# qinzheng93/GeoTransformer

Measured on NVIDIA H100. Metric: point-cloud pairs/sec (3DMatch-shape synth), higher is better.
Workload: dtype f32

## Files before the change

geotransformer_b200/_lib.py:

```python
import ctypes
import os
import threading

import torch

_HERE = os.path.dirname(os.path.abspath(__file__))
LIB_PATH = os.path.join(_HERE, 'libgeob200.so')
_lib = None

c_void_p, c_int64, c_int32, c_float, c_double, c_size_t, c_int = (
    ctypes.c_void_p, ctypes.c_int64, ctypes.c_int32, ctypes.c_float, ctypes.c_double, ctypes.c_size_t, ctypes.c_int)

SIGNATURES = {}


def _sig(name, restype, *argtypes):
    SIGNATURES[name] = (restype, list(argtypes))


P, I64, I32, F, D, SZ = c_void_p, c_int64, c_int32, c_float, c_double, c_size_t
_sig('geob200_last_error', ctypes.c_char_p)
_sig('geob200_launch_count', ctypes.c_uint64)
_sig('geob200_grid_subsample_workspace_bytes', SZ, I64, I64)
_sig('geob200_grid_subsample', c_int, P, I64, P, I64, F, P, P, P, SZ, P)
_sig('geob200_radius_search_workspace_bytes', SZ, I64, I64, I64)
_sig('geob200_radius_search', c_int, P, I64, P, I64, P, P, I64, F, I64, P, P, P, P, SZ, P)

_sig('geob200_neighbor_histogram', c_int, P, I64, I64, I64, I64, P, P)
_sig('geob200_kpconv_workspace_bytes', SZ, I64)
_sig('geob200_kpconv', c_int, P, P, P, P, I64, I64, I64, P, I64, P, P, I64, I64, F, P, P, SZ, P)
_sig('geob200_kpconv_tc_workspace_bytes', SZ, I64, I64, I64)
_sig('geob200_kpconv_tc', c_int, P, P, P, P, I64, I64, I64, P, I64, P, P, I64, I64, F, P, P, SZ, P)
_sig('geob200_set_linear_mode', None, c_int)
_sig('geob200_linear', c_int, P, I64, P, P, P, I64, I64, I64, I64, c_int, P)
_sig('geob200_split_tf32', c_int, P, I64, I64, I64, P, P)
_sig('geob200_linear_batched', c_int, P, I64, I64, P, I64, I64, P, I64, P, I64, I64, I64, I64, I64, I64, c_int, P)
_sig('geob200_group_norm_workspace_bytes', SZ, I64)
_sig('geob200_group_norm', c_int, P, I64, I64, I64, P, P, F, P, c_int, F, P, P, SZ, P)
_sig('geob200_fused_group_norm_workspace_bytes', SZ, I64, I64, I64)
_sig('geob200_linear_group_norm', c_int, P, I64, P, P, I64, I64, I64, I64, P, P, F, P, c_int, F, P, P, P, SZ, P)
_sig('geob200_kpconv_group_norm', c_int, P, P, P, P, I64, I64, I64, P, I64, P, P, I64, I64, F, I64, P, P, F, c_int, F, P, P, P, SZ,
     P, SZ, P)
_sig('geob200_group_norm_batched', c_int, P, I64, I64, I64, P, P, F, P, c_int, F, P, P, SZ, P, I64, P)
_sig('geob200_linear_group_norm_batched', c_int, P, I64, P, P, I64, I64, I64, I64, P, P, F, P, c_int, F, P, P, P, SZ, P, I64, P)
_sig('geob200_maxpool', c_int, P, P, I64, I64, I64, I64, P, P)
_sig('geob200_upsample_concat', c_int, P, P, I64, I64, P, I64, I64, I64, P, P)
_sig('geob200_kpconv_backward_workspace_bytes', SZ, I64, I64, I64, I64, I64)
_sig('geob200_kpconv_backward', c_int, P, P, P, P, I64, I64, I64, P, I64, P, I64, I64, F, P, P, P, P, P, SZ, P)
_sig('geob200_linear_backward_workspace_bytes', SZ, I64, I64, I64, c_int)
_sig('geob200_linear_backward', c_int, P, I64, P, P, I64, I64, I64, P, P, P, P, P, SZ, P)
_sig('geob200_group_norm_backward_batched_workspace_bytes', SZ, I64, I64, I64, I64)
_sig('geob200_group_norm_backward_batched', c_int, P, P, I64, I64, I64, P, F, c_int, F, P, P, P, P, P, P, SZ, P, I64, P)
_sig('geob200_maxpool_backward_batched_workspace_bytes', SZ, I64, I64, I64, I64)
_sig('geob200_maxpool_backward_batched', c_int, P, P, I64, I64, I64, I64, P, I64, P, P, P, P, SZ, P)
_sig('geob200_upsample_concat_backward_workspace_bytes', SZ, I64, I64)
_sig('geob200_upsample_concat_backward', c_int, P, I64, I64, I64, I64, I64, P, P, P, P, SZ, P)
_sig('geob200_point_to_node_partition_batched', c_int, P, P, I64, P, P, I64, P, P, P, P, P, P)
_sig('geob200_gather_rows', c_int, P, I64, I64, P, I64, P, P)
_sig('geob200_knn_partition', c_int, P, I64, P, I64, I64, P, P, P)
_sig('geob200_pairwise_distance', c_int, P, I64, P, I64, I64, c_int, P, P)
_sig('geob200_point_to_node_indices', c_int, P, I64, P, I64, P, P, P)
_sig('geob200_apply_transform', c_int, P, I64, P, P, P)
_sig('geob200_gse_indices_batched', c_int, P, I64, P, F, F, I64, P, P, P)
_sig('geob200_gse_embed_workspace_bytes', SZ, I64, I64)
_sig('geob200_gse_table_bytes', SZ, I64, I64, F, F)
_sig('geob200_gse_table_build', c_int, P, P, P, P, P, I64, I64, F, F, P, SZ, P)
_sig('geob200_gse_embed_table', c_int, P, P, I64, I64, P, SZ, I64, F, F, P, P, P, P, P, P, P)
_sig('geob200_gse_embed_pairs', c_int, P, P, I64, I64, P, P, P, P, P, P, P, P, c_int, P, SZ, P)
_sig('geob200_attention_workspace_bytes', SZ, I64, I64, I64)
_sig('geob200_attention', c_int, P, I64, P, I64, P, I64, P, P, P, I64, I64, I64, I64, P, I64, P, SZ, P)
_sig('geob200_set_attention_tma', c_int, c_int)
_sig('geob200_head_bias', c_int, P, I64, P, I64, I64, I64, P, P)
_sig('geob200_add_layernorm', c_int, P, P, P, P, I64, I64, F, P, P)
_sig('geob200_l2_normalize', c_int, P, I64, I64, P, P)
_sig('geob200_add_layernorm_backward_workspace_bytes', SZ, I64, I64)
_sig('geob200_add_layernorm_backward', c_int, P, P, P, I64, I64, F, P, P, P, P, P, SZ, P)
_sig('geob200_l2_normalize_backward', c_int, P, I64, I64, P, P, P)
_sig('geob200_head_project_backward_workspace_bytes', SZ, I64, I64, I64)
_sig('geob200_head_project_backward', c_int, P, I64, P, P, I64, I64, I64, P, P, P, I64, P, P, P, SZ, P)
_sig('geob200_attention_backward_batched_workspace_bytes', SZ, P, I64, I64)
_sig('geob200_attention_backward_batched', c_int, P, P, I64, I64, I64, I64, I64, I64, I64, I64, I64, I64, P, SZ, P)
_sig('geob200_gse_embed_backward_workspace_bytes', SZ, I64, I64)
_sig('geob200_gse_embed_backward', c_int, P, P, I64, I64, I64, P, SZ, I64, F, F, P, P, P, P, P, P, P, P, P, SZ, P)
_sig('geob200_sinkhorn', c_int, P, P, P, P, I64, I64, I64, F, P, P)
_sig('geob200_sinkhorn_backward_workspace_bytes', SZ, I64, I64, I64)
_sig('geob200_sinkhorn_backward', c_int, P, P, P, P, I64, I64, I64, F, P, P, P, P, SZ, P)
_sig('geob200_superpoint_matching_batched_workspace_bytes', SZ, I64, I64, I64)
_sig('geob200_superpoint_matching_batched', c_int, P, P, I64, P, P, I64, P, I64, c_int, P, P, P, P, SZ, P)
_sig('geob200_gather_patches_batched', c_int, P, I64, I64, P, P, P, P, I64, P, P, P, P, P)
_sig('geob200_patch_scores_batched', c_int, P, P, I64, I64, P, P, P, I64, I64, P, P)
_sig('geob200_patch_scores_backward_batched_workspace_bytes', SZ, I64, I64, I64, I64)
_sig('geob200_patch_scores_backward_batched', c_int, P, P, I64, I64, P, P, P, I64, I64, P, P, P, P, SZ, P)
_sig('geob200_lgr_batched_workspace_bytes', SZ, I64, I64, I64, I64)
_sig('geob200_local_global_registration_batched', c_int, P, P, P, P, P, I64, I64, I64, I64, I64, F, c_int, F, I64, I64, P, P, P, P,
     P, P, I64, P, P, P, P, SZ, P)
_sig('geob200_weighted_procrustes', c_int, P, P, P, I64, I64, F, F, P, P)

_sig('geob200_node_correspondences_batched_workspace_bytes', SZ, I64, I64, I64)
_sig('geob200_node_correspondences_batched', c_int, P, P, P, P, P, P, P, P, I64, P, I64, P, F, P, P, P, P, SZ, P)
_sig('geob200_evaluate_counts', c_int, P, P, I64, P, F, P, P, I64, P, P, P, I64, P, F, P, P, P, I64, c_int, F, F, F, P, P)
_sig('geob200_evaluate_batched', c_int, P, P, P, F, P, P, I64, P, P, P, I64, P, F, P, P, I64, P, I64, P, P, c_int, F, F, F, P, I64,
     P)
_sig('geob200_coarse_matching_loss_batched_workspace_bytes', SZ, I64, I64)
_sig('geob200_coarse_matching_loss_batched', c_int, P, P, I64, I64, P, P, P, P, F, F, F, F, F, F, P, I64, P, SZ, P)
_sig('geob200_fine_matching_loss_batched_workspace_bytes', SZ, I64, I64)
_sig('geob200_fine_matching_loss_batched', c_int, P, P, P, P, P, P, I64, I64, I64, P, D, P, P, I64, P, SZ, P)
_sig('geob200_coarse_matching_loss_backward_batched_workspace_bytes', SZ, I64, I64, I64)
_sig('geob200_coarse_matching_loss_backward_batched', c_int, P, P, I64, I64, P, P, P, P, F, F, F, F, F, F, P, I64, P, P, P, P, SZ, P)
_sig('geob200_fine_matching_loss_backward_batched_workspace_bytes', SZ, I64, I64)
_sig('geob200_fine_matching_loss_backward_batched', c_int, P, P, P, P, P, I64, I64, I64, P, D, P, I64, P, P, P, SZ, P)
_sig('geob200_ransac_correspondences_batched_workspace_bytes', SZ, I64, I64)
_sig('geob200_ransac_correspondences_batched', c_int, P, P, I64, I64, P, F, I64, I64, ctypes.c_uint64, I64, P, P, P, P, P, P, P, P, P, P,
     SZ, P)
_sig('geob200_feature_nn_batched_workspace_bytes', SZ, I64, I64, I64)
_sig('geob200_feature_nn_batched', c_int, P, P, I64, I64, I64, I64, P, P, P, P, P, P, P, SZ, P)
_sig('geob200_feature_corr_indices', c_int, P, P, P, P, I64, I64, I32, P, P, P, P, P)
_sig('geob200_ransac_features_batched_workspace_bytes', SZ, I64, I64, I64, I64, I64)
_sig('geob200_ransac_features_batched', c_int, P, P, P, P, I64, I64, I64, I64, P, P, F, I64, I64, I64, ctypes.c_uint64, I64, P, P, P, P, P,
     P, P, P, P, P, P, P, P, P, SZ, P)
_sig('geob200_correspondence_metrics_batched_workspace_bytes', SZ, I64, I64)
_sig('geob200_correspondence_metrics_batched', c_int, P, P, I64, I64, P, P, I64, F, P, I64, P, SZ, P)
_sig('geob200_corr_order_batched', c_int, P, I64, I64, P, I64, P, P)
_sig('geob200_corr_select_batched', c_int, P, P, P, I64, I64, P, P, I64, I64, P, P, P, P, P)
_sig('geob200_sparse_correspondence_eval_batched_workspace_bytes', SZ, I64, I64, I64)
_sig('geob200_sparse_correspondence_eval_batched', c_int, P, P, I64, P, P, I64, P, I64, I64, I64, P, P, SZ, P)
_sig('geob200_registration_error_batched', c_int, P, I64, P, I64, P, P, I64, c_int, D, D, P, P)
_sig('geob200_weighted_procrustes_counts', c_int, P, P, P, I64, I64, P, F, F, P, P)

_sig('geob200_linear_profile_enable', c_int, c_int)
_sig('geob200_set_split_k', c_int, c_int)
_sig('geob200_set_linear_persistent', c_int, c_int)
_sig('geob200_linear_profile_read', I64, I64, P, P)
_sig('geob200_backbone_workspace_bytes', SZ, P, P)
_sig('geob200_backbone_forward_batched', c_int, P, P, P, P, P, P, P, P, P, P, P, P, SZ, P, SZ, P, I64, P, P)
_sig('geob200_cloud_max_count', c_int, P, I64, I64, I64, I64, P, P, P)
_sig('geob200_transformer_batched_workspace_bytes', SZ, I64, P, I64, I64, I64)
_sig('geob200_transformer_forward_batched', c_int, P, I64, I64, I64, P, I64, P, P, P, P, SZ, P)
_sig('geob200_attention_batched_workspace_bytes', SZ, P, I64, I64)
_sig('geob200_attention_batched', c_int, P, I64, I64, I64, I64, I64, I64, I64, P, SZ, P)
_sig('geob200_attention_batched_keeps_probs', c_int, P, I64, I64, I64)
_sig('geob200_superpoint_targets_batched_workspace_bytes', SZ, I64)
_sig('geob200_superpoint_targets_batched', c_int, P, P, P, I64, P, F, I64, ctypes.c_uint64, ctypes.c_uint64, I64, P, P, P, P, SZ, P)
_sig('geob200_nonfinite_check', c_int, P, P, I64, I64, P, P)
_sig('geob200_batch_loss_weights', c_int, P, I64, I64, P, P, P, P, P)
_sig('geob200_kpconv_group_norm_batched', c_int, P, P, P, P, I64, I64, I64, P, I64, P, P, I64, I64, F, I64, P, P, F, c_int, F, P, P, P,
     SZ, P, SZ, P, I64, P)
_sig('geob200_maxpool_batched', c_int, P, P, I64, I64, I64, I64, P, I64, P, P, P)
_sig('geob200_augment_pairs_batched_workspace_bytes', SZ, I64)
_sig('geob200_augment_pairs_batched', c_int, P, P, I64, P, c_int, I64, D, D, D, D, D, ctypes.c_uint64, ctypes.c_uint64, I64, P, P, P, P, P,
     SZ, P)
_sig('geob200_modelnet_pairs_batched_workspace_bytes', SZ, I64)
_sig('geob200_modelnet_pairs_batched', c_int, P, P, I64, I64, D, D, D, D, ctypes.c_uint64, ctypes.c_uint64, I64, P, P, P, P, P, SZ, P)
_sig('geob200_modelnet_benchmark_pairs_batched_workspace_bytes', SZ, I64, I64)
_sig('geob200_modelnet_benchmark_pairs_batched', c_int, P, P, P, I64, I64, D, D, D, D, P, P, P, P, SZ, P)


def lib():
    global _lib
    if _lib is None:
        if not os.path.exists(LIB_PATH):
            raise RuntimeError(
                f'{LIB_PATH} not found: build it with `python -c "import __graft_entry__ as g; g.build()"` '
                '(there is no CPU fallback for the geotransformer_b200 ops)')
        handle = ctypes.CDLL(LIB_PATH)
        for name, (restype, argtypes) in SIGNATURES.items():
            fn = getattr(handle, name)
            fn.restype = restype
            fn.argtypes = argtypes
        _lib = handle
    return _lib


def check(rc, what):
    if rc != 0:
        msg = lib().geob200_last_error().decode(errors='replace')
        raise RuntimeError(f'{what} failed ({rc}): {msg}')


_tls = threading.local()


def stream_ptr():
    p = getattr(_tls, 'stream', None)
    if p is not None:
        return p
    return torch.cuda.current_stream().cuda_stream


class stream_scope:

    def __init__(self, ptr):
        self.ptr = ptr

    def __enter__(self):
        self.prev = getattr(_tls, 'stream', None)
        _tls.stream = self.ptr
        return self

    def __exit__(self, *a):
        _tls.stream = self.prev
        return False


def require_cuda(t, name, dtype=None):
    if not t.is_cuda:
        raise RuntimeError(f'{name} must be a CUDA tensor (geotransformer_b200 has no CPU path)')
    if dtype is not None and t.dtype != dtype:
        raise RuntimeError(f'{name} must be {dtype}, got {t.dtype}')
    if not t.is_contiguous():
        raise RuntimeError(f'{name} must be contiguous')


_WS = {}


def workspace(nbytes, device, tag='default'):
    key = (device.index if device.index is not None else torch.cuda.current_device(), stream_ptr(), tag)
    buf = _WS.get(key)
    if buf is None or buf.numel() < nbytes:
        buf = torch.empty(max(int(nbytes * 1.3), 1 << 20), dtype=torch.uint8, device=device)
        _WS[key] = buf
    return buf


def ptr(t):
    return None if t is None else t.data_ptr()
```

geotransformer_b200/csrc/common.cuh:

```cuda
#pragma once
#include <cuda_runtime.h>
#include <stdint.h>
#include <stdio.h>

namespace geob200 {

void set_error(const char* fmt, ...);
void count_launches(int n);
int ensure_max_smem(const void* kernel);

#define GEOB_CHECK_CUDA(expr)                                                                   \
    do {                                                                                        \
        cudaError_t _e = (expr);                                                                \
        if (_e != cudaSuccess) {                                                                \
            geob200::set_error("%s:%d CUDA error %s: %s", __FILE__, __LINE__, #expr,            \
                               cudaGetErrorString(_e));                                         \
            return -1;                                                                          \
        }                                                                                       \
    } while (0)

#define GEOB_CHECK_LAUNCH()                                                                     \
    do {                                                                                        \
        cudaError_t _e = cudaGetLastError();                                                    \
        if (_e != cudaSuccess) {                                                                \
            geob200::set_error("%s:%d kernel launch failed: %s", __FILE__, __LINE__,            \
                               cudaGetErrorString(_e));                                         \
            return -1;                                                                          \
        }                                                                                       \
    } while (0)

#define GEOB_REQUIRE(cond, ...)                                                                 \
    do {                                                                                        \
        if (!(cond)) {                                                                          \
            geob200::set_error(__VA_ARGS__);                                                    \
            return -2;                                                                          \
        }                                                                                       \
    } while (0)

static inline size_t align_up(size_t x, size_t a) { return (x + a - 1) / a * a; }

template <int CNT, int MASK>
struct Butterfly {
    template <int NV>
    static __device__ __forceinline__ void run(float (&v)[NV], int lane) {
        if constexpr (CNT > 1) {
            constexpr int HALF = CNT / 2;
            const bool upper = (lane & MASK) != 0;
#pragma unroll
            for (int i = 0; i < HALF; ++i) {
                const float send = upper ? v[i] : v[i + HALF];
                const float keep = upper ? v[i + HALF] : v[i];
                v[i] = keep + __shfl_xor_sync(0xffffffffu, send, MASK);
            }
            if constexpr (MASK > 1) Butterfly<HALF, MASK / 2>::run(v, lane);
        } else {
            v[0] += __shfl_xor_sync(0xffffffffu, v[0], MASK);
            if constexpr (MASK > 1) Butterfly<1, MASK / 2>::run(v, lane);
        }
    }
};
template <int NV>
__device__ __forceinline__ float warp_butterfly(float (&v)[NV], int lane) {
    Butterfly<NV, 16>::run(v, lane);
    return v[0];
}

struct GnFuse {
    int groups;
    int slot_width;
    double* partial;
};

constexpr int GEOB_MAX_CLOUDS = 64;
struct GnSeg {
    int n_clouds;
    int n_pairs;
    int start[GEOB_MAX_CLOUDS + 1];
};
size_t fused_group_norm_workspace_bytes_batched(int64_t n_rows, int64_t channels, int64_t groups, int64_t n_pairs);
int group_norm_impl(const float* x, int64_t n_rows, int64_t channels, int64_t groups, const float* gamma, const float* beta, float eps,
                    const float* residual, int leaky, float slope, float* y, void* workspace, size_t workspace_bytes, void* stream,
                    const GnSeg* seg);
int linear_group_norm_impl(const float* x, int64_t ldx, const float* weight, const float* bias, int64_t m, int64_t n, int64_t k,
                           int64_t groups, const float* gamma, const float* beta, float eps, const float* residual, int leaky,
                           float slope, float* pre_norm, float* y, void* workspace, size_t workspace_bytes, void* stream,
                           const GnSeg* seg, const float* w_img = nullptr);
int kpconv_group_norm_impl(const float* s_feats, const float* q_points, const float* s_points, const int64_t* neighbors,
                           int64_t n_query, int64_t n_support, int64_t n_neighbors, const float* kernel_points, int64_t n_kernel,
                           const float* weights_t, const float* bias, int64_t c_in, int64_t c_out, float sigma, int64_t groups,
                           const float* gamma, const float* beta, float eps, int leaky, float slope, float* pre_norm, float* y,
                           void* gn_workspace, size_t gn_workspace_bytes, void* workspace, size_t workspace_bytes, void* stream,
                           const GnSeg* seg, const float* w_img = nullptr);
int linear_img(const float* x, int64_t ldx, const float* weight, const float* w_img, const float* bias, float* y, int64_t ldy,
               int64_t m, int64_t n, int64_t k, int relu, void* stream);
int kpconv_tc_impl(const float* s_feats, const float* q_points, const float* s_points, const int64_t* neighbors, int64_t n_query,
                   int64_t n_support, int64_t n_neighbors, const float* kernel_points, int64_t n_kernel, const float* weights_t,
                   const float* w_img, const float* bias, int64_t c_in, int64_t c_out, float sigma, float* out, void* workspace,
                   size_t workspace_bytes, void* stream);

int maxpool_seg(const float* x, const int64_t* neighbors, int64_t n_query, int64_t n_support, int64_t n_neighbors, int64_t channels,
                float* y, const GnSeg* seg, const int* cloud_max, void* stream);

struct Segs {
    int n;
    int max;
    int start[GEOB_MAX_CLOUDS];
    int count[GEOB_MAX_CLOUDS];
};
int segs_from_counts(Segs* s, int64_t n, const int64_t* counts);
Segs segs_one(int64_t count);
Segs segs_range(const Segs& s, int first, int n);
int segs_products(Segs* s, const Segs& ref, const Segs& src);

struct Arena {
    char* base;
    size_t off;
    size_t cap;
    __host__ Arena(void* p, size_t bytes) : base(static_cast<char*>(p)), off(0), cap(bytes) {}
    template <typename T>
    __host__ T* take(size_t n) {
        off = align_up(off, 256);
        T* r = reinterpret_cast<T*>(base + off);
        off += n * sizeof(T);
        return r;
    }
    __host__ bool ok() const { return off <= cap; }
};

__device__ __forceinline__ float warp_sum(float v) {
#pragma unroll
    for (int o = 16; o > 0; o >>= 1) v += __shfl_xor_sync(0xffffffffu, v, o);
    return v;
}
__device__ __forceinline__ float warp_max(float v) {
#pragma unroll
    for (int o = 16; o > 0; o >>= 1) v = fmaxf(v, __shfl_xor_sync(0xffffffffu, v, o));
    return v;
}
__device__ __forceinline__ double warp_sum_d(double v) {
#pragma unroll
    for (int o = 16; o > 0; o >>= 1) v += __shfl_xor_sync(0xffffffffu, v, o);
    return v;
}

__device__ __forceinline__ float tf32_rn(float x) {
    uint32_t r;
    asm("cvt.rna.tf32.f32 %0, %1;" : "=r"(r) : "f"(x));
    return __uint_as_float(r);
}

static inline int num_sms() {
    static int n = 0;
    if (n == 0) {
        int dev = 0;
        cudaGetDevice(&dev);
        cudaDeviceGetAttribute(&n, cudaDevAttrMultiProcessorCount, dev);
        if (n <= 0) n = 132;
    }
    return n;
}

}
```

geotransformer_b200/csrc/kpconv.cu:

```cuda
#include "common.cuh"
#include "geob200.h"
#include "kpconv.cuh"

namespace geob200 {

constexpr int TQ = 32;
constexpr int CC = 32;

__global__ void __launch_bounds__(256) kpconv_c1_kernel(const float* __restrict__ feats, const float* __restrict__ q_pts,
                                                        const float* __restrict__ s_pts, const long long* __restrict__ nbr,
                                                        int H, const float* __restrict__ kp, const float* __restrict__ W,
                                                        const float* __restrict__ bias, float sigma, int Ns, int M, int Cout,
                                                        float* __restrict__ out) {
    __shared__ float kp_s[KP * 3];
    __shared__ float wk_s[16][KP_PAD];
    __shared__ float np_s[16];
    if (threadIdx.x < KP * 3) kp_s[threadIdx.x] = kp[threadIdx.x];
    __syncthreads();
    const int lane = threadIdx.x & 31, warp = threadIdx.x >> 5;
    const int sub = lane >> 4, sl = lane & 15;
    const int slot = warp * 2 + sub;
    const int m = blockIdx.x * 16 + slot;
    const bool live = m < M;
    float acc[KP];
// ... 495 lines not shown
            mean_rstd[2 * g + 1] = (float)(1.0 / sqrt(var + eps));
        }
    }
}

__global__ void __launch_bounds__(256) gn_tile_stats_kernel(const float* __restrict__ x, int N, int C, int slot_width,
                                                            double* __restrict__ partial) {
    extern __shared__ double sh[];
    const int slots = C / slot_width;
    for (int i = threadIdx.x; i < 2 * slots; i += blockDim.x) sh[i] = 0.0;
    __syncthreads();
    const int r0 = blockIdx.x * 128, r1 = min(N, r0 + 128);
    const int cw = C < 256 ? C : 256;
    const int rpb = 256 / cw;
    const int rr = threadIdx.x / cw;
    if (rr < rpb)
        for (int c = threadIdx.x % cw; c < C; c += cw) {
            double s = 0.0, s2 = 0.0;
            for (int r = r0 + rr; r < r1; r += rpb) {
                const double v = (double)x[(long long)r * C + c];
                s += v;
                s2 += v * v;
            }
            atomicAdd(&sh[2 * (c / slot_width)], s);
            atomicAdd(&sh[2 * (c / slot_width) + 1], s2);
        }
    __syncthreads();
    for (int i = threadIdx.x; i < 2 * slots; i += blockDim.x) partial[(long long)blockIdx.x * 2 * slots + i] = sh[i];
}

__global__ void __launch_bounds__(128) gn_seg_finalize_kernel(const double* __restrict__ partial, const float* __restrict__ x, int C,
                                                              int slots_total, int spg, int G, double eps, GnSeg seg,
                                                              float* __restrict__ mean_rstd) {
    __shared__ double red[8];
    const int lane = threadIdx.x & 31, warp = threadIdx.x >> 5;
    const int g = blockIdx.x, p = blockIdx.y;
    const int cpg = C / G;
    const double2* part = reinterpret_cast<const double2*>(partial);
    double sa = 0.0, sb = 0.0;
    long long rows = 0;
    for (int c = p; c < seg.n_clouds; c += seg.n_pairs) {
        const int r0 = seg.start[c], r1 = seg.start[c + 1];
        rows += r1 - r0;
        int t0 = (r0 + 127) / 128, t1 = r1 / 128;
        if (t1 < t0) t1 = t0;
        const int n_full = (t1 - t0) * spg;
        for (int i = threadIdx.x; i < n_full; i += 128) {
            const int t = t0 + i / spg, sl = i % spg;
            const double2 v = part[(long long)t * slots_total + (long long)g * spg + sl];
            sa += v.x;
            sb += v.y;
        }
        const int e0 = min(r1, t0 * 128);
        const int b1 = min(r1, max(e0, t1 * 128));
        const int n_edge = (e0 - r0) + (r1 - b1);
        for (int i = threadIdx.x; i < n_edge * cpg; i += 128) {
            const int ri = i / cpg, j = i % cpg;
            const int r = ri < e0 - r0 ? r0 + ri : b1 + (ri - (e0 - r0));
            const double v = (double)x[(long long)r * C + g * cpg + j];
            sa += v;
            sb += v * v;
        }
    }
#pragma unroll
    for (int o = 16; o > 0; o >>= 1) {
        sa += __shfl_xor_sync(0xffffffffu, sa, o);
        sb += __shfl_xor_sync(0xffffffffu, sb, o);
    }
    if (lane == 0) { red[2 * warp] = sa; red[2 * warp + 1] = sb; }
    __syncthreads();
    if (threadIdx.x == 0) {
        sa = (red[0] + red[2]) + (red[4] + red[6]);
        sb = (red[1] + red[3]) + (red[5] + red[7]);
        const double count = (double)cpg * (double)rows;
        const double mean = sa / count;
        double var = sb / count - mean * mean;
        if (var < 0.0) var = 0.0;
        mean_rstd[((long long)p * G + g) * 2] = (float)mean;
        mean_rstd[((long long)p * G + g) * 2 + 1] = (float)(1.0 / sqrt(var + eps));
    }
}

constexpr int GN_RPB = 32;
__global__ void __launch_bounds__(256) gn_seg_apply_kernel(const float* __restrict__ x, const float* __restrict__ mean_rstd,
                                                           const float* __restrict__ gamma, const float* __restrict__ beta,
                                                           const float* __restrict__ residual, float* __restrict__ y, int n_rows,
                                                           int C, int cpg, int G, int leaky, float slope, GnSeg seg) {
    extern __shared__ float gn_tab[];
    __shared__ int starts[GEOB_MAX_CLOUDS + 1];
    for (int i = threadIdx.x; i <= seg.n_clouds; i += blockDim.x) starts[i] = seg.start[i];
    __syncthreads();
    const int r0 = blockIdx.x * GN_RPB, r1 = min(n_rows, r0 + GN_RPB);
    int c0 = 0, hi = seg.n_clouds;
    while (hi - c0 > 1) {
        const int mid = (c0 + hi) >> 1;
        if (starts[mid] <= r0) c0 = mid; else hi = mid;
    }
    for (int i = threadIdx.x; i < 2 * C; i += blockDim.x) {
        const int t = i / C, c = i % C;
        const int cl = min(c0 + t, seg.n_clouds - 1);
        const float* mr = mean_rstd + (long long)(cl % seg.n_pairs) * 2 * G + 2 * (c / cpg);
        gn_tab[(2 * t) * C + c] = mr[0];
        gn_tab[(2 * t + 1) * C + c] = mr[1];
    }
    __syncthreads();
    const int b0 = starts[c0 + 1];
    const int b1 = (c0 + 2 <= seg.n_clouds) ? starts[c0 + 2] : n_rows;
    const int C4 = C >> 2;
    const long long base4 = (long long)r0 * C4;
    const int total4 = (r1 - r0) * C4;
    for (int i = threadIdx.x; i < total4; i += blockDim.x) {
        const int row = r0 + i / C4, c = (i % C4) * 4;
        const float4 v = reinterpret_cast<const float4*>(x)[base4 + i];
        float4 rv = make_float4(0.f, 0.f, 0.f, 0.f);
        if (residual != nullptr) rv = reinterpret_cast<const float4*>(residual)[base4 + i];
        float in[4] = {v.x, v.y, v.z, v.w}, o[4];
        const float rs[4] = {rv.x, rv.y, rv.z, rv.w};
        if (row < b1) {
            const float* ta = gn_tab + (row < b0 ? 0 : 2 * C) + c;
            const float4 gm = __ldg(reinterpret_cast<const float4*>(gamma + c)), bt = __ldg(reinterpret_cast<const float4*>(beta + c));
            const float ga[4] = {gm.x, gm.y, gm.z, gm.w}, ba[4] = {bt.x, bt.y, bt.z, bt.w};
#pragma unroll
            for (int u = 0; u < 4; ++u) o[u] = (in[u] - ta[u]) * ta[C + u] * ga[u] + ba[u] + rs[u];
        } else {
            int lo = c0, hh = seg.n_clouds;
            while (hh - lo > 1) {
                const int mid = (lo + hh) >> 1;
                if (starts[mid] <= row) lo = mid; else hh = mid;
            }
            const float* mr = mean_rstd + (long long)(lo % seg.n_pairs) * 2 * G;
#pragma unroll
            for (int u = 0; u < 4; ++u) {
                const int g = (c + u) / cpg;
                o[u] = (in[u] - mr[2 * g]) * mr[2 * g + 1] * gamma[c + u] + beta[c + u] + rs[u];
            }
        }
        if (leaky) {
#pragma unroll
            for (int u = 0; u < 4; ++u) o[u] = o[u] > 0.f ? o[u] : o[u] * slope;
        }
        reinterpret_cast<float4*>(y)[base4 + i] = make_float4(o[0], o[1], o[2], o[3]);
    }
}

__global__ void __launch_bounds__(256) gn_apply_kernel(const float* __restrict__ x, const float* __restrict__ mean_rstd,
                                                       const float* __restrict__ gamma, const float* __restrict__ beta,
                                                       const float* __restrict__ residual, float* __restrict__ y,
                                                       long long total4, int C, int cpg, int leaky, float slope) {
    const long long i = (long long)blockIdx.x * blockDim.x + threadIdx.x;
    if (i >= total4) return;
    const float4 v = reinterpret_cast<const float4*>(x)[i];
    const int c = (int)((i * 4) % C);
    float in[4] = {v.x, v.y, v.z, v.w}, o[4];
    float4 rv = make_float4(0.f, 0.f, 0.f, 0.f);
    if (residual != nullptr) rv = reinterpret_cast<const float4*>(residual)[i];
    const float rs[4] = {rv.x, rv.y, rv.z, rv.w};
#pragma unroll
    for (int u = 0; u < 4; ++u) {
        const int g = (c + u) / cpg;
        float t = (in[u] - mean_rstd[2 * g]) * mean_rstd[2 * g + 1] * gamma[c + u] + beta[c + u];
        t += rs[u];
        if (leaky) t = t > 0.f ? t : t * slope;
        o[u] = t;
    }
    reinterpret_cast<float4*>(y)[i] = make_float4(o[0], o[1], o[2], o[3]);
}

__device__ __forceinline__ void maxpool_row(const float* __restrict__ x, const long long* __restrict__ nb, int W, int Ns, int C,
                                            float* __restrict__ yrow, int lane) {
    constexpr int NI = 5;
    if ((C & 3) == 0 && W <= 32 * NI) {
        int idx_l[NI];
#pragma unroll
        for (int i = 0; i < NI; ++i) idx_l[i] = (lane + 32 * i < W) ? (int)min(nb[lane + 32 * i], (long long)Ns) : Ns;
        const int C4 = C >> 2;
        for (int c0 = 0; c0 < C4; c0 += 32) {
            const int c4 = c0 + lane;
            const bool active = c4 < C4;
            float4 best = make_float4(-INFINITY, -INFINITY, -INFINITY, -INFINITY);
            for (int h0 = 0; h0 < W; h0 += 4) {
                float4 v[4];
#pragma unroll
                for (int u = 0; u < 4; ++u) {
                    const int h = h0 + u;
                    int id = Ns;
#pragma unroll
                    for (int i = 0; i < NI; ++i) {
                        const int t = __shfl_sync(0xffffffffu, idx_l[i], h & 31);
                        if ((h >> 5) == i) id = t;
                    }
                    v[u] = (active && h < W && id < Ns) ? __ldg(reinterpret_cast<const float4*>(x + (long long)id * C) + c4)
                                                        : make_float4(0.f, 0.f, 0.f, 0.f);
                    if (h >= W) v[u] = best;
                }
#pragma unroll
                for (int u = 0; u < 4; ++u) {
                    best.x = fmaxf(best.x, v[u].x); best.y = fmaxf(best.y, v[u].y);
                    best.z = fmaxf(best.z, v[u].z); best.w = fmaxf(best.w, v[u].w);
                }
            }
            if (active) reinterpret_cast<float4*>(yrow)[c4] = best;
        }
        return;
    }
    for (int c = lane; c < C; c += 32) {
        float best = -INFINITY;
        for (int h = 0; h < W; ++h) {
            const long long idx = nb[h];
            const float v = (idx < Ns) ? x[idx * C + c] : 0.f;
            best = fmaxf(best, v);
        }
        yrow[c] = best;
    }
}

__global__ void __launch_bounds__(256) maxpool_seg_kernel(const float* __restrict__ x, const long long* __restrict__ nbr, int H,
                                                          int Ns, int M, int C, float* __restrict__ y, GnSeg seg,
                                                          const int* __restrict__ cloud_max) {
    __shared__ int starts[GEOB_MAX_CLOUDS + 1];
    __shared__ int width[GEOB_MAX_CLOUDS];
    for (int i = threadIdx.x; i <= seg.n_clouds; i += blockDim.x) starts[i] = seg.start[i];
    for (int i = threadIdx.x; i < seg.n_clouds; i += blockDim.x) {
        const int p = i % seg.n_pairs;
        int w = 0;
        for (int c = p; c < seg.n_clouds; c += seg.n_pairs) w = max(w, cloud_max[c]);
        width[i] = min(H, w);
    }
    __syncthreads();
    const int lane = threadIdx.x & 31;
    const int m = blockIdx.x * 8 + (threadIdx.x >> 5);
    if (m >= M) return;
    int lo = 0, hi = seg.n_clouds;
    while (hi - lo > 1) {
        const int mid = (lo + hi) >> 1;
        if (starts[mid] <= m) lo = mid; else hi = mid;
    }
    const int W = width[lo];
    maxpool_row(x, nbr + (long long)m * H, W, Ns, C, y + (long long)m * C, lane);
}

__global__ void __launch_bounds__(256) cloud_max_count_kernel(const long long* __restrict__ nbr, int H, int Ns, GnSeg seg,
                                                              int* __restrict__ cloud_max) {
    __shared__ int red[8];
    const int c = blockIdx.x;
    const int r0 = seg.start[c], r1 = seg.start[c + 1];
    int best = 0;
    for (int m = r0 + (int)threadIdx.x; m < r1; m += blockDim.x) {
        int lo = 0, hi = H;
        while (lo < hi) {
            const int mid = (lo + hi) >> 1;
            if (nbr[(long long)m * H + mid] < Ns) lo = mid + 1; else hi = mid;
        }
        best = max(best, lo);
    }
    for (int o = 16; o > 0; o >>= 1) best = max(best, __shfl_xor_sync(0xffffffffu, best, o));
    if ((threadIdx.x & 31) == 0) red[threadIdx.x >> 5] = best;
    __syncthreads();
    if (threadIdx.x == 0) {
        for (int w = 1; w < 8; ++w) best = max(best, red[w]);
        cloud_max[c] = best;
    }
}

__global__ void __launch_bounds__(256) maxpool_kernel(const float* __restrict__ x, const long long* __restrict__ nbr, int H,
                                                      int Ns, int M, int C, float* __restrict__ y) {
    const int lane = threadIdx.x & 31;
    const int m = blockIdx.x * 8 + (threadIdx.x >> 5);
    if (m >= M) return;
    if ((C & 3) == 0 && H <= 160) {
        maxpool_row(x, nbr + (long long)m * H, H, Ns, C, y + (long long)m * C, lane);
        return;
    }
    for (int c = lane; c < C; c += 32) {
        float best = -INFINITY;
        for (int h = 0; h < H; ++h) {
            const long long idx = nbr[(long long)m * H + h];
            const float v = (idx < Ns) ? x[idx * C + c] : 0.f;
            best = fmaxf(best, v);
        }
        y[(long long)m * C + c] = best;
    }
}

__global__ void __launch_bounds__(256) upsample_concat_kernel(const float* __restrict__ x, const long long* __restrict__ up,
                                                              int up_stride, int Ns, const float* __restrict__ skip, int M,
                                                              int C1, int C2, float* __restrict__ y) {
    const int lane = threadIdx.x & 31;
    const int m = blockIdx.x * 8 + (threadIdx.x >> 5);
    if (m >= M) return;
    const long long idx = up[(long long)m * up_stride];
    float* yr = y + (long long)m * (C1 + C2);
    for (int c = lane; c < C1; c += 32) yr[c] = (idx < Ns) ? x[idx * C1 + c] : 0.f;
    if (skip != nullptr)
        for (int c = lane; c < C2; c += 32) yr[C1 + c] = skip[(long long)m * C2 + c];
}

}

using namespace geob200;

namespace geob200 {
int linear_tc(const float* x, int64_t ldx, const float* w, int64_t ldw, const float* w_img, const float* bias, const float* row_scale, float* y, int64_t ldy,
              int64_t m, int64_t n, int64_t k, int relu, cudaStream_t st, const GnFuse* gn = nullptr);
static int g_linear_mode = 1;
}

extern "C" {

void geob200_set_linear_mode(int mode) { g_linear_mode = mode; }

size_t geob200_kpconv_workspace_bytes(int64_t n_support) { return (size_t)n_support + 256; }

size_t geob200_kpconv_tc_workspace_bytes(int64_t n_query, int64_t n_support, int64_t c_in) {
    return align_up((size_t)n_support, 256) + align_up((size_t)n_query * 4, 256) + (size_t)n_query * KP * (size_t)c_in * 4 + 1024;
}

int geob200_kpconv_tc(const float* s_feats, const float* q_points, const float* s_points, const int64_t* neighbors, int64_t n_query,
                      int64_t n_support, int64_t n_neighbors, const float* kernel_points, int64_t n_kernel, const float* weights_t,
                      const float* bias, int64_t c_in, int64_t c_out, float sigma, float* out, void* workspace, size_t workspace_bytes,
                      void* stream) {
    return geob200::kpconv_tc_impl(s_feats, q_points, s_points, neighbors, n_query, n_support, n_neighbors, kernel_points, n_kernel,
                                   weights_t, nullptr, bias, c_in, c_out, sigma, out, workspace, workspace_bytes, stream);
}
}

namespace geob200 {
int kpconv_tc_impl(const float* s_feats, const float* q_points, const float* s_points, const int64_t* neighbors, int64_t n_query,
                   int64_t n_support, int64_t n_neighbors, const float* kernel_points, int64_t n_kernel, const float* weights_t,
                   const float* w_img, const float* bias, int64_t c_in, int64_t c_out, float sigma, float* out, void* workspace,
                   size_t workspace_bytes, void* stream) {
    cudaStream_t st = (cudaStream_t)stream;
    GEOB_REQUIRE(n_kernel == KP, "kpconv_tc: kernel_size %lld unsupported", (long long)n_kernel);
    GEOB_REQUIRE(n_query > 0 && n_support > 0 && n_neighbors > 0, "kpconv_tc: empty input");
    GEOB_REQUIRE(c_in % 32 == 0 && c_out % 16 == 0 && c_out >= 32 && (c_out <= 128 || c_out % 128 == 0) && n_query >= 64,
                 "kpconv_tc: unsupported shape (%lld -> %lld, %lld queries)", (long long)c_in, (long long)c_out, (long long)n_query);
    GEOB_REQUIRE(workspace_bytes >= geob200_kpconv_tc_workspace_bytes(n_query, n_support, c_in), "kpconv_tc: workspace too small");
    Arena ar(workspace, workspace_bytes);
    unsigned char* pos = ar.take<unsigned char>(n_support);
    float* inv_count = ar.take<float>(n_query);
    float* wf = ar.take<float>((size_t)n_query * KP * c_in);
    row_positive_kernel<<<(unsigned)((n_support + 7) / 8), 256, 0, st>>>(s_feats, (int)n_support, (int)c_in, pos);
    launch_kpconv_gather(s_feats, pos, q_points, s_points, (const long long*)neighbors, (int)n_neighbors, kernel_points, sigma,
                         (int)n_support, (int)n_query, (int)c_in, wf, inv_count, st);
    GEOB_CHECK_LAUNCH();
    count_launches(2);
    const int rc = linear_tc(wf, KP * c_in, weights_t, KP * c_in, w_img, bias, inv_count, out, c_out, n_query, c_out, KP * c_in, 0, st);
    GEOB_REQUIRE(rc == 0, "kpconv_tc: tensor-core GEMM rejected the shape");
    return 0;
}

int linear_img(const float* x, int64_t ldx, const float* weight, const float* w_img, const float* bias, float* y, int64_t ldy,
               int64_t m, int64_t n, int64_t k, int relu, void* stream) {
    if (g_linear_mode == 1 && m > 0 && n > 0 && k > 0) {
        const int rc = linear_tc(x, ldx, weight, k, w_img, bias, nullptr, y, ldy, m, n, k, relu, (cudaStream_t)stream);
        if (rc <= 0) return rc;
    }
    return geob200_linear(x, ldx, weight, bias, y, ldy, m, n, k, relu, stream);
}
}

extern "C" {

int geob200_kpconv(const float* s_feats, const float* q_points, const float* s_points, const int64_t* neighbors,
                   int64_t n_query, int64_t n_support, int64_t n_neighbors, const float* kernel_points, int64_t n_kernel,
                   const float* weights, const float* bias, int64_t c_in, int64_t c_out, float sigma, float* out,
                   void* workspace, size_t workspace_bytes, void* stream) {
    cudaStream_t st = (cudaStream_t)stream;
    GEOB_REQUIRE(n_kernel == KP, "kpconv: kernel_size %lld unsupported (all shipped models use 15)", (long long)n_kernel);
    GEOB_REQUIRE(n_query > 0 && n_support > 0 && n_neighbors > 0, "kpconv: empty input");
    if (c_in == 1) {
        kpconv_c1_kernel<<<(unsigned)((n_query + 15) / 16), 256, 0, st>>>(s_feats, q_points, s_points, (const long long*)neighbors,
                                                                       (int)n_neighbors, kernel_points, weights, bias, sigma,
                                                                       (int)n_support, (int)n_query, (int)c_out, out);
        GEOB_CHECK_LAUNCH();
        count_launches(1);
        return 0;
    }
    GEOB_REQUIRE(c_in % 32 == 0 && c_out % 32 == 0 && c_out <= 512,
                 "kpconv: channel counts (%lld -> %lld) must be multiples of 32, c_out <= 512", (long long)c_in, (long long)c_out);
    GEOB_REQUIRE(workspace != nullptr && workspace_bytes >= geob200_kpconv_workspace_bytes(n_support), "kpconv: workspace too small");
    unsigned char* pos = (unsigned char*)workspace;
    row_positive_kernel<<<(unsigned)((n_support + 7) / 8), 256, 0, st>>>(s_feats, (int)n_support, (int)c_in, pos);
    const size_t smem = sizeof(float) * (TQ * KP * CC + 8 * 32 * KP_PAD + TQ + KP * 3 + 3) + sizeof(int) * 8 * 32;
    const unsigned qtiles = (unsigned)((n_query + TQ - 1) / TQ);
    int rc = (int)(c_out / 32);
    int split = 1;
    while (rc > 1 && split < 4 && (long long)qtiles * split < 2ll * num_sms()) { rc >>= 1; split <<= 1; }
    const dim3 grid(qtiles, (unsigned)split);
#define LAUNCH_KP(RCV)                                                                                              \
    {                                                                                                               \
        if (ensure_max_smem((const void*)kpconv_kernel<RCV>)) return -1;                                            \
        kpconv_kernel<RCV><<<grid, 256, smem, st>>>(s_feats, pos, q_points, s_points, (const long long*)neighbors,  \
                                                    (int)n_neighbors, kernel_points, weights, bias, sigma,         \
                                                    (int)n_support, (int)n_query, (int)c_in, (int)c_out, out);     \
    }
    switch (rc) {
        case 1: LAUNCH_KP(1) break;
        case 2: LAUNCH_KP(2) break;
        case 4: LAUNCH_KP(4) break;
        case 8: LAUNCH_KP(8) break;
        case 16: LAUNCH_KP(16) break;
        default: GEOB_REQUIRE(false, "kpconv: c_out %lld unsupported (32,64,128,256,512)", (long long)c_out);
    }
#undef LAUNCH_KP
    GEOB_CHECK_LAUNCH();
    count_launches(2);
    return 0;
}

int geob200_linear_batched(const float* x, int64_t ldx, int64_t stride_x, const float* weight, int64_t ldw, int64_t stride_w,
                           const float* bias, int64_t stride_b, float* y, int64_t ldy, int64_t stride_y, int64_t m, int64_t n,
                           int64_t k, int64_t batch, int relu, void* stream) {
    cudaStream_t st = (cudaStream_t)stream;
    GEOB_REQUIRE(m > 0 && n > 0 && k > 0 && batch > 0, "linear: empty problem");
    if (batch == 1 && g_linear_mode == 1) {
        const int rc = linear_tc(x, ldx, weight, ldw, nullptr, bias, nullptr, y, ldy, m, n, k, relu, st);
        if (rc <= 0) return rc;
    }
    const unsigned z = (unsigned)batch;
    const long long c64 = ((n + 63) / 64) * ((m + 63) / 64) * batch, c6432 = ((n + 31) / 32) * ((m + 63) / 64) * batch;
    if (c64 >= num_sms()) {
        dim3 grid((unsigned)((n + 63) / 64), (unsigned)((m + 63) / 64), z);
        linear_kernel<64, 64><<<grid, 256, 0, st>>>(x, (int)ldx, weight, (int)ldw, bias, y, (int)ldy, (int)m, (int)n, (int)k, relu,
                                                    stride_x, stride_w, stride_b, stride_y);
    } else if (c6432 >= num_sms()) {
        dim3 grid((unsigned)((n + 31) / 32), (unsigned)((m + 63) / 64), z);
        linear_kernel<64, 32><<<grid, 256, 0, st>>>(x, (int)ldx, weight, (int)ldw, bias, y, (int)ldy, (int)m, (int)n, (int)k, relu,
                                                    stride_x, stride_w, stride_b, stride_y);
    } else {
        dim3 grid((unsigned)((n + 31) / 32), (unsigned)((m + 31) / 32), z);
        linear_kernel<32, 32><<<grid, 256, 0, st>>>(x, (int)ldx, weight, (int)ldw, bias, y, (int)ldy, (int)m, (int)n, (int)k, relu,
                                                    stride_x, stride_w, stride_b, stride_y);
    }
    GEOB_CHECK_LAUNCH();
    count_launches(1);
    return 0;
}

int geob200_linear(const float* x, int64_t ldx, const float* weight, const float* bias, float* y, int64_t ldy, int64_t m,
                   int64_t n, int64_t k, int relu, void* stream) {
    return geob200_linear_batched(x, ldx, 0, weight, k, 0, bias, 0, y, ldy, 0, m, n, k, 1, relu, stream);
}

size_t geob200_group_norm_workspace_bytes(int64_t groups) { return (size_t)(592 * 2 * groups * 8 + 2 * groups * 4 + 256 + 1024); }

size_t geob200_fused_group_norm_workspace_bytes(int64_t n_rows, int64_t channels, int64_t groups) {
    const size_t tiles = (size_t)((n_rows + 127) / 128);
    const size_t slots = (size_t)(channels / groups >= 32 ? channels / 32 : groups);
    const size_t fused = tiles * slots * 2 * 8;
    const size_t plain = (size_t)(592 * 2 * groups * 8);
    return (fused > plain ? fused : plain) + (size_t)(2 * groups * 4) + 256 + 1024;
}

}

namespace geob200 {
size_t fused_group_norm_workspace_bytes_batched(int64_t n_rows, int64_t channels, int64_t groups, int64_t n_pairs) {
    return geob200_fused_group_norm_workspace_bytes(n_rows, channels, groups) + (size_t)(2 * groups * 4) * (size_t)(n_pairs > 1 ? n_pairs : 1) + 512;
}
struct GnWs { unsigned* ticket; float* mean_rstd; double* partial; };
static GnWs gn_carve(void* workspace, size_t bytes, int64_t groups, int64_t n_pairs = 1) {
    Arena ar(workspace, bytes);
    GnWs w;
    w.ticket = ar.take<unsigned>(64);
    w.mean_rstd = ar.take<float>(2 * groups * n_pairs);
    w.partial = ar.take<double>(1);
    return w;
}
static void launch_gn_seg_apply(const float* x, const GnWs& w, const float* gamma, const float* beta, const float* residual, float* y,
                                int64_t n_rows, int64_t channels, int64_t groups, float eps, int leaky, float slope, const GnSeg& seg,
                                cudaStream_t st) {
    const int cpg = (int)(channels / groups);
    const int slot_width = cpg < 32 ? cpg : 32;
    gn_seg_finalize_kernel<<<dim3((unsigned)groups, (unsigned)seg.n_pairs), 128, 0, st>>>(
        w.partial, x, (int)channels, (int)(channels / slot_width), cpg / slot_width, (int)groups, (double)eps, seg, w.mean_rstd);
    gn_seg_apply_kernel<<<(unsigned)((n_rows + GN_RPB - 1) / GN_RPB), 256, sizeof(float) * 4 * channels, st>>>(
        x, w.mean_rstd, gamma, beta, residual, y, (int)n_rows, (int)channels, cpg, (int)groups, leaky, slope, seg);
    count_launches(2);
}
static void launch_gn_tile_stats(const float* x, const GnWs& w, int64_t n_rows, int64_t channels, int64_t groups, cudaStream_t st) {
    const int cpg = (int)(channels / groups);
    const int slot_width = cpg < 32 ? cpg : 32;
    gn_tile_stats_kernel<<<(unsigned)((n_rows + 127) / 128), 256, sizeof(double) * 2 * (channels / slot_width), st>>>(
        x, (int)n_rows, (int)channels, slot_width, w.partial);
    count_launches(1);
}
static void launch_gn_apply(const float* x, const GnWs& w, const float* gamma, const float* beta, const float* residual, float* y,
                            int64_t n_rows, int64_t channels, int64_t groups, float eps, int leaky, float slope, cudaStream_t st) {
    const int cpg = (int)(channels / groups);
    const int slot_width = cpg < 32 ? cpg : 32;
    gn_finalize_kernel<<<1, 1024, 0, st>>>(w.partial, (int)((n_rows + 127) / 128), (int)(channels / slot_width), cpg / slot_width,
                                           (int)groups, (double)cpg * (double)n_rows, (double)eps, w.mean_rstd);
    const long long total4 = n_rows * channels / 4;
    gn_apply_kernel<<<(unsigned)((total4 + 255) / 256), 256, 0, st>>>(x, w.mean_rstd, gamma, beta, residual, y, total4, (int)channels,
                                                                     (int)(channels / groups), leaky, slope);
}
}

extern "C" {

int geob200_group_norm(const float* x, int64_t n_rows, int64_t channels, int64_t groups, const float* gamma,
                       const float* beta, float eps, const float* residual, int leaky, float slope, float* y,
                       void* workspace, size_t workspace_bytes, void* stream) {
    return geob200::group_norm_impl(x, n_rows, channels, groups, gamma, beta, eps, residual, leaky, slope, y, workspace, workspace_bytes,
                                    stream, nullptr);
}
}

namespace geob200 {
int group_norm_impl(const float* x, int64_t n_rows, int64_t channels, int64_t groups, const float* gamma, const float* beta, float eps,
                    const float* residual, int leaky, float slope, float* y, void* workspace, size_t workspace_bytes, void* stream,
                    const GnSeg* seg) {
    cudaStream_t st = (cudaStream_t)stream;
    GEOB_REQUIRE(n_rows > 0 && channels > 0 && groups > 0 && channels % groups == 0, "group_norm: bad shape");
    GEOB_REQUIRE(channels % 4 == 0, "group_norm: channels must be a multiple of 4");
    if (seg != nullptr && seg->n_pairs > 1) {
        GEOB_REQUIRE(workspace_bytes >= fused_group_norm_workspace_bytes_batched(n_rows, channels, groups, seg->n_pairs),
                     "group_norm: workspace too small (batched)");
        const GnWs w = gn_carve(workspace, workspace_bytes, groups, seg->n_pairs);
        launch_gn_tile_stats(x, w, n_rows, channels, groups, st);
        launch_gn_seg_apply(x, w, gamma, beta, residual, y, n_rows, channels, groups, eps, leaky, slope, *seg, st);
        GEOB_CHECK_LAUNCH();
        return 0;
    }
    GEOB_REQUIRE(workspace_bytes >= geob200_group_norm_workspace_bytes(groups), "group_norm: workspace too small");
    Arena ar(workspace, workspace_bytes);
    unsigned* ticket = ar.take<unsigned>(64);
    float* mean_rstd = ar.take<float>(2 * groups);
    double* partial = ar.take<double>(592 * 2 * groups);
    int nblk = (int)((n_rows + 127) / 128);
    if (nblk > 296) nblk = 296;
    if (nblk < 1) nblk = 1;
    gn_stats_kernel<<<nblk, 256, sizeof(double) * 2 * groups, st>>>(x, (int)n_rows, (int)channels, (int)groups, (double)eps,
                                                                    partial, ticket, mean_rstd);
    const long long total4 = n_rows * channels / 4;
    gn_apply_kernel<<<(unsigned)((total4 + 255) / 256), 256, 0, st>>>(x, mean_rstd, gamma, beta, residual, y, total4,
                                                                     (int)channels, (int)(channels / groups), leaky, slope);
    GEOB_CHECK_LAUNCH();
    count_launches(2);
    return 0;
}
}

extern "C" {

int geob200_maxpool(const float* x, const int64_t* neighbors, int64_t n_query, int64_t n_support, int64_t n_neighbors,
                    int64_t channels, float* y, void* stream) {
    maxpool_kernel<<<(unsigned)((n_query + 7) / 8), 256, 0, (cudaStream_t)stream>>>(x, (const long long*)neighbors, (int)n_neighbors,
                                                                                  (int)n_support, (int)n_query, (int)channels, y);
    GEOB_CHECK_LAUNCH();
    count_launches(1);
    return 0;
}

int geob200_upsample_concat(const float* x, const int64_t* up_indices, int64_t up_stride, int64_t n_support,
                            const float* skip, int64_t n_query, int64_t c1, int64_t c2, float* y, void* stream) {
    upsample_concat_kernel<<<(unsigned)((n_query + 7) / 8), 256, 0, (cudaStream_t)stream>>>(
        x, (const long long*)up_indices, (int)up_stride, (int)n_support, skip, (int)n_query, (int)c1, (int)c2, y);
    GEOB_CHECK_LAUNCH();
    count_launches(1);
    return 0;
}

int geob200_linear_group_norm(const float* x, int64_t ldx, const float* weight, const float* bias, int64_t m, int64_t n, int64_t k,
                              int64_t groups, const float* gamma, const float* beta, float eps, const float* residual, int leaky,
                              float slope, float* pre_norm, float* y, void* workspace, size_t workspace_bytes, void* stream) {
    return geob200::linear_group_norm_impl(x, ldx, weight, bias, m, n, k, groups, gamma, beta, eps, residual, leaky, slope, pre_norm, y,
                                           workspace, workspace_bytes, stream, nullptr);
}
}

namespace geob200 {
int linear_group_norm_impl(const float* x, int64_t ldx, const float* weight, const float* bias, int64_t m, int64_t n, int64_t k,
                           int64_t groups, const float* gamma, const float* beta, float eps, const float* residual, int leaky,
                           float slope, float* pre_norm, float* y, void* workspace, size_t workspace_bytes, void* stream,
                           const GnSeg* seg, const float* w_img) {
    cudaStream_t st = (cudaStream_t)stream;
    const int64_t np = (seg != nullptr && seg->n_pairs > 1) ? seg->n_pairs : 1;
    GEOB_REQUIRE(m > 0 && n > 0 && k > 0 && groups > 0 && n % groups == 0 && n % 4 == 0, "linear_group_norm: bad shape");
    GEOB_REQUIRE(workspace_bytes >= (np > 1 ? fused_group_norm_workspace_bytes_batched(m, n, groups, np)
                                            : geob200_fused_group_norm_workspace_bytes(m, n, groups)), "linear_group_norm: workspace too small");
    if (g_linear_mode == 1) {
        const GnWs w = gn_carve(workspace, workspace_bytes, groups, np);
        GnFuse gn{(int)groups, 0, w.partial};
        const int rc = linear_tc(x, ldx, weight, k, w_img, bias, nullptr, pre_norm, n, m, n, k, 0, st, &gn);
        if (rc < 0) return rc;
        if (rc == 0) {
            if (np > 1) {
                launch_gn_seg_apply(pre_norm, w, gamma, beta, residual, y, m, n, groups, eps, leaky, slope, *seg, st);
            } else {
                launch_gn_apply(pre_norm, w, gamma, beta, residual, y, m, n, groups, eps, leaky, slope, st);
                count_launches(2);
            }
            GEOB_CHECK_LAUNCH();
            return 0;
        }
    }
    int rc = linear_img(x, ldx, weight, w_img, bias, pre_norm, n, m, n, k, 0, stream);
    if (rc != 0) return rc;
    return group_norm_impl(pre_norm, m, n, groups, gamma, beta, eps, residual, leaky, slope, y, workspace, workspace_bytes, stream, seg);
}
}

extern "C" {

int geob200_kpconv_group_norm(const float* s_feats, const float* q_points, const float* s_points, const int64_t* neighbors,
                              int64_t n_query, int64_t n_support, int64_t n_neighbors, const float* kernel_points, int64_t n_kernel,
                              const float* weights_t, const float* bias, int64_t c_in, int64_t c_out, float sigma, int64_t groups,
                              const float* gamma, const float* beta, float eps, int leaky, float slope, float* pre_norm, float* y,
                              void* gn_workspace, size_t gn_workspace_bytes, void* workspace, size_t workspace_bytes, void* stream) {
    return geob200::kpconv_group_norm_impl(s_feats, q_points, s_points, neighbors, n_query, n_support, n_neighbors, kernel_points, n_kernel,
                                           weights_t, bias, c_in, c_out, sigma, groups, gamma, beta, eps, leaky, slope, pre_norm, y,
                                           gn_workspace, gn_workspace_bytes, workspace, workspace_bytes, stream, nullptr);
}
}

namespace geob200 {
int kpconv_group_norm_impl(const float* s_feats, const float* q_points, const float* s_points, const int64_t* neighbors,
                           int64_t n_query, int64_t n_support, int64_t n_neighbors, const float* kernel_points, int64_t n_kernel,
                           const float* weights_t, const float* bias, int64_t c_in, int64_t c_out, float sigma, int64_t groups,
                           const float* gamma, const float* beta, float eps, int leaky, float slope, float* pre_norm, float* y,
                           void* gn_workspace, size_t gn_workspace_bytes, void* workspace, size_t workspace_bytes, void* stream,
                           const GnSeg* seg, const float* w_img) {
    cudaStream_t st = (cudaStream_t)stream;
    const int64_t np = (seg != nullptr && seg->n_pairs > 1) ? seg->n_pairs : 1;
    GEOB_REQUIRE(n_kernel == KP, "kpconv_group_norm: kernel_size %lld unsupported", (long long)n_kernel);
    GEOB_REQUIRE(n_query > 0 && n_support > 0 && n_neighbors > 0, "kpconv_group_norm: empty input");
    GEOB_REQUIRE(c_in % 32 == 0 && c_out % 16 == 0 && c_out >= 32 && (c_out <= 128 || c_out % 128 == 0) && n_query >= 64,
                 "kpconv_group_norm: unsupported shape (%lld -> %lld, %lld queries)", (long long)c_in, (long long)c_out,
                 (long long)n_query);
    GEOB_REQUIRE(groups > 0 && c_out % groups == 0, "kpconv_group_norm: bad group count");
    GEOB_REQUIRE(gn_workspace_bytes >= (np > 1 ? fused_group_norm_workspace_bytes_batched(n_query, c_out, groups, np)
                                               : geob200_fused_group_norm_workspace_bytes(n_query, c_out, groups)),
                 "kpconv_group_norm: GroupNorm workspace too small");
    GEOB_REQUIRE(workspace_bytes >= geob200_kpconv_tc_workspace_bytes(n_query, n_support, c_in), "kpconv_group_norm: workspace too small");
    Arena ar(workspace, workspace_bytes);
    unsigned char* pos = ar.take<unsigned char>(n_support);
    float* inv_count = ar.take<float>(n_query);
    float* wf = ar.take<float>((size_t)n_query * KP * c_in);
    row_positive_kernel<<<(unsigned)((n_support + 7) / 8), 256, 0, st>>>(s_feats, (int)n_support, (int)c_in, pos);
    launch_kpconv_gather(s_feats, pos, q_points, s_points, (const long long*)neighbors, (int)n_neighbors, kernel_points, sigma,
                         (int)n_support, (int)n_query, (int)c_in, wf, inv_count, st);
    GEOB_CHECK_LAUNCH();
    count_launches(2);
    const GnWs w = gn_carve(gn_workspace, gn_workspace_bytes, groups, np);
    GnFuse gn{(int)groups, 0, w.partial};
    int rc = linear_tc(wf, KP * c_in, weights_t, KP * c_in, w_img, bias, inv_count, pre_norm, c_out, n_query, c_out, KP * c_in, 0, st, &gn);
    if (rc < 0) return rc;
    if (rc == 0) {
        if (np > 1) {
            launch_gn_seg_apply(pre_norm, w, gamma, beta, nullptr, y, n_query, c_out, groups, eps, leaky, slope, *seg, st);
        } else {
            launch_gn_apply(pre_norm, w, gamma, beta, nullptr, y, n_query, c_out, groups, eps, leaky, slope, st);
            count_launches(2);
        }
        GEOB_CHECK_LAUNCH();
        return 0;
    }
    rc = linear_tc(wf, KP * c_in, weights_t, KP * c_in, w_img, bias, inv_count, pre_norm, c_out, n_query, c_out, KP * c_in, 0, st);
    GEOB_REQUIRE(rc == 0, "kpconv_group_norm: tensor-core GEMM rejected the shape");
    return group_norm_impl(pre_norm, n_query, c_out, groups, gamma, beta, eps, nullptr, leaky, slope, y, gn_workspace, gn_workspace_bytes,
                           stream, seg);
}
}

namespace geob200 {
int make_seg(GnSeg* g, int64_t n_pairs, const int64_t* cloud_rows_h, int64_t n_rows, const char* what) {
    GEOB_REQUIRE(n_pairs >= 1 && 2 * n_pairs <= GEOB_MAX_CLOUDS && cloud_rows_h != nullptr, "%s: 1 <= pairs per batch <= %d", what,
                 GEOB_MAX_CLOUDS / 2);
    g->n_pairs = (int)n_pairs; g->n_clouds = (int)(2 * n_pairs); g->start[0] = 0;
    for (int c = 0; c < g->n_clouds; ++c) {
        GEOB_REQUIRE(cloud_rows_h[c] >= 0, "%s: negative cloud row count", what);
        g->start[c + 1] = g->start[c] + (int)cloud_rows_h[c];
    }
    GEOB_REQUIRE(g->start[g->n_clouds] == n_rows, "%s: cloud rows do not add up to n_rows", what);
    return 0;
}
}

extern "C" {

int geob200_group_norm_batched(const float* x, int64_t n_rows, int64_t channels, int64_t groups, const float* gamma, const float* beta,
                               float eps, const float* residual, int leaky, float slope, float* y, void* workspace, size_t workspace_bytes,
                               void* stream, int64_t n_pairs, const int64_t* cloud_rows_h) {
    geob200::GnSeg seg;
    if (geob200::make_seg(&seg, n_pairs, cloud_rows_h, n_rows, "group_norm")) return -2;
    return geob200::group_norm_impl(x, n_rows, channels, groups, gamma, beta, eps, residual, leaky, slope, y, workspace, workspace_bytes,
                                    stream, &seg);
}

int geob200_linear_group_norm_batched(const float* x, int64_t ldx, const float* weight, const float* bias, int64_t m, int64_t n, int64_t k,
                                      int64_t groups, const float* gamma, const float* beta, float eps, const float* residual, int leaky,
                                      float slope, float* pre_norm, float* y, void* workspace, size_t workspace_bytes, void* stream,
                                      int64_t n_pairs, const int64_t* cloud_rows_h) {
    geob200::GnSeg seg;
    if (geob200::make_seg(&seg, n_pairs, cloud_rows_h, m, "group_norm")) return -2;
    return geob200::linear_group_norm_impl(x, ldx, weight, bias, m, n, k, groups, gamma, beta, eps, residual, leaky, slope, pre_norm, y,
                                           workspace, workspace_bytes, stream, &seg);
}

int geob200_cloud_max_count(const int64_t* neighbors, int64_t n_query, int64_t n_support, int64_t n_neighbors, int64_t n_pairs,
                            const int64_t* cloud_rows_h, int32_t* cloud_max, void* stream) {
    geob200::GnSeg seg;
    if (geob200::make_seg(&seg, n_pairs, cloud_rows_h, n_query, "group_norm")) return -2;
    geob200::cloud_max_count_kernel<<<seg.n_clouds, 256, 0, (cudaStream_t)stream>>>((const long long*)neighbors, (int)n_neighbors,
                                                                                   (int)n_support, seg, cloud_max);
    GEOB_CHECK_LAUNCH();
    geob200::count_launches(1);
    return 0;
}

}

namespace geob200 {
int maxpool_seg(const float* x, const int64_t* neighbors, int64_t n_query, int64_t n_support, int64_t n_neighbors, int64_t channels,
                float* y, const GnSeg* seg, const int* cloud_max, void* stream) {
    maxpool_seg_kernel<<<(unsigned)((n_query + 7) / 8), 256, 0, (cudaStream_t)stream>>>(x, (const long long*)neighbors, (int)n_neighbors,
                                                                                      (int)n_support, (int)n_query, (int)channels, y, *seg,
                                                                                      cloud_max);
    GEOB_CHECK_LAUNCH();
    count_launches(1);
    return 0;
}
}

extern "C" {

int geob200_kpconv_group_norm_batched(const float* s_feats, const float* q_points, const float* s_points, const int64_t* neighbors,
                                      int64_t n_query, int64_t n_support, int64_t n_neighbors, const float* kernel_points, int64_t n_kernel,
                                      const float* weights_t, const float* bias, int64_t c_in, int64_t c_out, float sigma, int64_t groups,
                                      const float* gamma, const float* beta, float eps, int leaky, float slope, float* pre_norm, float* y,
                                      void* gn_workspace, size_t gn_workspace_bytes, void* workspace, size_t workspace_bytes, void* stream,
                                      int64_t n_pairs, const int64_t* cloud_rows_h) {
    geob200::GnSeg seg;
    if (geob200::make_seg(&seg, n_pairs, cloud_rows_h, n_query, "kpconv_group_norm")) return -2;
    GEOB_REQUIRE(pre_norm != nullptr && y != nullptr, "kpconv_group_norm: null output");
    return geob200::kpconv_group_norm_impl(s_feats, q_points, s_points, neighbors, n_query, n_support, n_neighbors, kernel_points, n_kernel,
                                           weights_t, bias, c_in, c_out, sigma, groups, gamma, beta, eps, leaky, slope, pre_norm, y,
                                           gn_workspace, gn_workspace_bytes, workspace, workspace_bytes, stream, &seg);
}

int geob200_maxpool_batched(const float* x, const int64_t* neighbors, int64_t n_query, int64_t n_support, int64_t n_neighbors,
                            int64_t channels, const int32_t* cloud_max, int64_t n_pairs, const int64_t* cloud_rows_h, float* y,
                            void* stream) {
    geob200::GnSeg seg;
    if (geob200::make_seg(&seg, n_pairs, cloud_rows_h, n_query, "maxpool")) return -2;
    GEOB_REQUIRE(n_query > 0 && n_support > 0 && n_neighbors > 0 && channels > 0, "maxpool: empty input");
    GEOB_REQUIRE(x != nullptr && neighbors != nullptr && cloud_max != nullptr && y != nullptr, "maxpool: null pointer");
    return geob200::maxpool_seg(x, neighbors, n_query, n_support, n_neighbors, channels, y, &seg, cloud_max, stream);
}

}
```

geotransformer_b200/csrc/linear_tc.cu:

```cuda
#include <cuda.h>

#include <cstdlib>
#include <mutex>
#include <vector>

#include "common.cuh"
#include "geob200.h"
#include "hopper.cuh"

namespace geob200 {
namespace ltc {

using namespace hop;

constexpr int BM = 128;
constexpr int KC = 32;
constexpr int TILE_A = BM * 128;
constexpr int TILE_B = 128 * 128;
constexpr int STAGE = TILE_A + 2 * TILE_B;
constexpr int NSTAGE = 4;
constexpr int PRODUCER_WARP = 8;
constexpr int NTHREADS = (PRODUCER_WARP + 4) * 32;
constexpr int SMEM = NSTAGE * STAGE + 1024 + 256 + 8 * 128 * 8 + 512;

__global__ void __launch_bounds__(256) split_tf32_kernel(const float* __restrict__ w, long long ld, long long n, long long k,
                                                         float* __restrict__ out) {
    const long long nk = n * k;
    for (long long i = (long long)blockIdx.x * blockDim.x + threadIdx.x; i < nk; i += (long long)gridDim.x * blockDim.x) {
        const long long r = i / k, c = i % k;
        const float x = w[r * ld + c];
        const float hi = tf32_rn(x);
        out[i] = hi;
        out[nk + i] = x - hi;
    }
}

template <int BNI>
__global__ void __launch_bounds__(NTHREADS, 1) linear_tc_kernel(const __grid_constant__ CUtensorMap map_x,
                                                                const __grid_constant__ CUtensorMap map_w,
                                                                const float* __restrict__ bias, const float* __restrict__ row_scale,
                                                                float* __restrict__ Y, int ldy, int M, int N, int K, int BN, int relu,
                                                                GnFuse gn, float* __restrict__ splitk_out, int chunks_per_split,
                                                                int col_tiles, int row_tiles, int num_tiles) {
    constexpr int R = BNI / 2;
    extern __shared__ unsigned char smem_raw[];
    unsigned char* smem = (unsigned char*)(((uintptr_t)smem_raw + 1023) & ~(uintptr_t)1023);
    uint64_t* bars = (uint64_t*)(smem + NSTAGE * STAGE);
    uint64_t* full = bars;
    uint64_t* empty = bars + NSTAGE;
    float2* gn_sm = (float2*)(smem + NSTAGE * STAGE + 256);
    float* bias_s = (float*)(gn_sm + 8 * 128);
    const int warp = threadIdx.x >> 5, lane = threadIdx.x & 31;
    const int nk = (K + KC - 1) / KC;
    const int tiles_per_split = col_tiles * row_tiles;

    if (threadIdx.x == 0) {
        for (int s = 0; s < NSTAGE; ++s) { mbar_init(&full[s], 1); mbar_init(&empty[s], 8); }
        asm volatile("fence.mbarrier_init.release.cluster;" ::: "memory");
        asm volatile("prefetch.tensormap [%0];" ::"l"(&map_x) : "memory");
        asm volatile("prefetch.tensormap [%0];" ::"l"(&map_w) : "memory");
    }
    __syncthreads();

    if (warp >= PRODUCER_WARP) {
        asm volatile("setmaxnreg.dec.sync.aligned.u32 40;" ::: "memory");
        if (warp == PRODUCER_WARP && lane == 0) {
            int s = 0;
            uint32_t ph = 0;
            for (int t = blockIdx.x; t < num_tiles; t += gridDim.x) {
                const int z = t / tiles_per_split, rem = t % tiles_per_split;
                const int m0 = (rem / col_tiles) * BM, n0 = (rem % col_tiles) * BN;
                const int kc0 = z * chunks_per_split, kc1 = min(nk, kc0 + chunks_per_split);
                for (int kc = kc0; kc < kc1; ++kc) {
                    mbar_wait(&empty[s], ph ^ 1u);
                    unsigned char* st = smem + s * STAGE;
                    mbar_arrive_expect_tx(&full[s], (uint32_t)(TILE_A + 2 * BN * 128));
                    tma_load_2d(st, &map_x, kc * KC, m0, &full[s]);
                    tma_load_2d(st + TILE_A, &map_w, kc * KC, n0, &full[s]);
                    tma_load_2d(st + TILE_A + TILE_B, &map_w, kc * KC, N + n0, &full[s]);
                    if (++s == NSTAGE) { s = 0; ph ^= 1u; }
                }
            }
        }
        return;
    }

    asm volatile("setmaxnreg.inc.sync.aligned.u32 232;" ::: "memory");
    const int wg = warp >> 2, wq = warp & 3;
    int s = 0;
    uint32_t ph = 0;
    for (int t = blockIdx.x; t < num_tiles; t += gridDim.x) {
        const int z = t / tiles_per_split, rem = t % tiles_per_split;
        const int ty = rem / col_tiles;
        const int m0 = ty * BM, n0 = (rem % col_tiles) * BN;
        const int kc0 = z * chunks_per_split, kc1 = min(nk, kc0 + chunks_per_split);
        asm volatile("bar.sync 1, 256;" ::: "memory");
        if (threadIdx.x < 128) bias_s[threadIdx.x] = (bias != nullptr && (int)threadIdx.x < BN) ? __ldg(bias + n0 + threadIdx.x) : 0.f;
        asm volatile("bar.sync 1, 256;" ::: "memory");

        float acc[R], cor[R];
#pragma unroll
        for (int i = 0; i < R; ++i) { acc[i] = 0.f; cor[i] = 0.f; }
        const int g = lane >> 2, tq = lane & 3;
        const int a_off = (wg * 64 + wq * 16 + g) * 128 + tq * 4;
        for (int kc = kc0; kc < kc1; ++kc) {
            mbar_wait(&full[s], ph);
            unsigned char* st = smem + s * STAGE;
            uint32_t f[2][KC / 8][4];
#pragma unroll
            for (int kk = 0; kk < KC / 8; ++kk)
#pragma unroll
                for (int e = 0; e < 4; ++e) {
                    const int j = 2 * kk + (e >> 1);
                    const float x = *reinterpret_cast<const float*>(st + a_off + (e & 1) * 8 * 128 + ((j ^ g) << 4));
                    const float hi = tf32_rn(x);
                    f[0][kk][e] = __float_as_uint(hi);
                    f[1][kk][e] = __float_as_uint(x - hi);
                }
            const uint32_t sb = smem_u32(st + TILE_A);
            const uint64_t b_hi = make_desc(sb), b_lo = make_desc(sb + TILE_B);
            wgmma_fence();
#pragma unroll
            for (int kk = 0; kk < KC / 8; ++kk) {
                const uint64_t adv = (uint64_t)(kk * 2);
                const uint32_t accum = (kc == kc0 && kk == 0) ? 0u : 1u;
                wgmma_tf32_rs<BNI>(acc, f[0][kk], b_hi + adv, accum);
                wgmma_tf32_rs<BNI>(cor, f[0][kk], b_lo + adv, accum);
                wgmma_tf32_rs<BNI>(cor, f[1][kk], b_hi + adv, 1u);
            }
            wgmma_commit();
            wgmma_wait<0>();
            __syncwarp();
            if (lane == 0) mbar_arrive(&empty[s]);
            if (++s == NSTAGE) { s = 0; ph ^= 1u; }
        }
        reg_fence(acc);
        reg_fence(cor);

        const int r0 = m0 + wg * 64 + wq * 16 + (lane >> 2);
        const int c0 = 2 * (lane & 3);
        float rs[2];
#pragma unroll
        for (int h = 0; h < 2; ++h) rs[h] = (row_scale != nullptr && r0 + 8 * h < M) ? row_scale[r0 + 8 * h] : 1.0f;
        if (splitk_out != nullptr) {
#pragma unroll
            for (int j = 0; j < BNI / 8; ++j)
#pragma unroll
                for (int h = 0; h < 2; ++h) {
                    const int m = r0 + 8 * h, col = 8 * j + c0;
                    if (m < M && col < BN)
                        *reinterpret_cast<float2*>(splitk_out + ((long long)z * M + m) * N + n0 + col) =
                            make_float2(acc[4 * j + 2 * h] + cor[4 * j + 2 * h], acc[4 * j + 2 * h + 1] + cor[4 * j + 2 * h + 1]);
                }
            continue;
        }
        const bool vec2 = ((ldy & 1) == 0) && ((reinterpret_cast<uintptr_t>(Y) & 7) == 0);
#pragma unroll
        for (int j = 0; j < BNI / 8; ++j) {
            const int col = 8 * j + c0;
            float o[4];
#pragma unroll
            for (int e = 0; e < 4; ++e) {
                float v = (acc[4 * j + e] + cor[4 * j + e]) * rs[e >> 1] + bias_s[col + (e & 1)];
                if (relu) v = fmaxf(v, 0.f);
                o[e] = v;
            }
#pragma unroll
            for (int h = 0; h < 2; ++h) {
                const int m = r0 + 8 * h;
                if (m < M && col < BN) {
                    float* yp = Y + (long long)m * ldy + n0 + col;
                    if (vec2) *reinterpret_cast<float2*>(yp) = make_float2(o[2 * h], o[2 * h + 1]);
                    else { yp[0] = o[2 * h]; yp[1] = o[2 * h + 1]; }
                }
            }
            if (gn.groups > 0) {
                const bool ok0 = r0 < M && col < BN, ok1 = r0 + 8 < M && col < BN;
                float a0 = (ok0 ? o[0] : 0.f) + (ok1 ? o[2] : 0.f), a1 = (ok0 ? o[1] : 0.f) + (ok1 ? o[3] : 0.f);
                float q0 = (ok0 ? o[0] * o[0] : 0.f) + (ok1 ? o[2] * o[2] : 0.f);
                float q1 = (ok0 ? o[1] * o[1] : 0.f) + (ok1 ? o[3] * o[3] : 0.f);
#pragma unroll
                for (int off = 4; off < 32; off <<= 1) {
                    a0 += __shfl_xor_sync(0xffffffffu, a0, off);
                    a1 += __shfl_xor_sync(0xffffffffu, a1, off);
                    q0 += __shfl_xor_sync(0xffffffffu, q0, off);
                    q1 += __shfl_xor_sync(0xffffffffu, q1, off);
                }
                if (lane < 4) {
                    gn_sm[warp * 128 + col] = make_float2(a0, q0);
                    gn_sm[warp * 128 + col + 1] = make_float2(a1, q1);
                }
            }
        }
        if (gn.groups > 0) {
            asm volatile("bar.sync 1, 256;" ::: "memory");
            const int sw = gn.slot_width, slots_tile = BN / sw, slots_total = N / sw;
            const int et = threadIdx.x;
            if (et < slots_tile) {
                double s1 = 0.0, s2 = 0.0;
                for (int w = 0; w < 8; ++w) {
                    float f1 = 0.f, f2 = 0.f;
                    for (int c = 0; c < sw; ++c) {
                        const float2 p = gn_sm[w * 128 + et * sw + c];
                        f1 += p.x;
                        f2 += p.y;
                    }
                    s1 += (double)f1;
                    s2 += (double)f2;
                }
                double* dst = gn.partial + ((long long)ty * slots_total + n0 / sw + et) * 2;
                dst[0] = s1;
                dst[1] = s2;
            }
        }
    }
}

__global__ void __launch_bounds__(256) splitk_reduce_kernel(const float* __restrict__ P, int splits, long long MN, int N,
                                                            const float* __restrict__ bias, const float* __restrict__ row_scale,
                                                            float* __restrict__ Y, int ldy, int relu) {
    const long long i4 = ((long long)blockIdx.x * blockDim.x + threadIdx.x) * 4;
    if (i4 >= MN) return;
    float4 a = *reinterpret_cast<const float4*>(P + i4);
    for (int z = 1; z < splits; ++z) {
        const float4 b = *reinterpret_cast<const float4*>(P + (long long)z * MN + i4);
        a.x += b.x; a.y += b.y; a.z += b.z; a.w += b.w;
    }
    const long long m = i4 / N;
    const int n = (int)(i4 % N);
    const float rs = row_scale != nullptr ? row_scale[m] : 1.0f;
    float o[4] = {a.x * rs, a.y * rs, a.z * rs, a.w * rs};
#pragma unroll
    for (int u = 0; u < 4; ++u) {
        if (bias != nullptr) o[u] += bias[n + u];
        if (relu) o[u] = fmaxf(o[u], 0.f);
    }
    float* y = Y + m * ldy + n;
    if ((reinterpret_cast<uintptr_t>(y) & 15) == 0) *reinterpret_cast<float4*>(y) = make_float4(o[0], o[1], o[2], o[3]);
    else { y[0] = o[0]; y[1] = o[1]; y[2] = o[2]; y[3] = o[3]; }
}

typedef CUresult (*EncodeTiledFn)(CUtensorMap*, CUtensorMapDataType, cuuint32_t, void*, const cuuint64_t*, const cuuint64_t*,
                                  const cuuint32_t*, const cuuint32_t*, CUtensorMapInterleave, CUtensorMapSwizzle,
                                  CUtensorMapL2promotion, CUtensorMapFloatOOBfill);
static EncodeTiledFn encode_fn() {
    static EncodeTiledFn fn = nullptr;
    if (fn == nullptr) {
        void* p = nullptr;
        cudaDriverEntryPointQueryResult q;
        if (cudaGetDriverEntryPoint("cuTensorMapEncodeTiled", &p, cudaEnableDefault, &q) == cudaSuccess && q == cudaDriverEntryPointSuccess)
            fn = (EncodeTiledFn)p;
    }
    return fn;
}

static int encode_map(CUtensorMap* map, const float* base, int64_t rows, int64_t cols, int64_t ld, int box_rows) {
    EncodeTiledFn fn = encode_fn();
    if (fn == nullptr) { set_error("cuTensorMapEncodeTiled entry point not available"); return -1; }
    cuuint64_t gdim[2] = {(cuuint64_t)cols, (cuuint64_t)rows};
    cuuint64_t gstride[1] = {(cuuint64_t)ld * sizeof(float)};
    cuuint32_t box[2] = {(cuuint32_t)KC, (cuuint32_t)box_rows};
    cuuint32_t estr[2] = {1, 1};
    CUresult r = fn(map, CU_TENSOR_MAP_DATA_TYPE_FLOAT32, 2, (void*)base, gdim, gstride, box, estr, CU_TENSOR_MAP_INTERLEAVE_NONE,
                    CU_TENSOR_MAP_SWIZZLE_128B, CU_TENSOR_MAP_L2_PROMOTION_L2_128B, CU_TENSOR_MAP_FLOAT_OOB_FILL_NONE);
    if (r != CUDA_SUCCESS) { set_error("cuTensorMapEncodeTiled failed with CUresult %d", (int)r); return -1; }
    return 0;
}

}

struct ProfRec { cudaEvent_t a, b; long long m, n, k; };
static std::vector<ProfRec> g_prof;
static std::mutex g_prof_mu;
static bool g_prof_on = false;
static bool g_splitk_on = true;
static bool g_persistent_on = true;

struct StreamWs { void* ptr; size_t bytes; };
static std::vector<std::pair<cudaStream_t, StreamWs>> g_split_ws, g_wimg_ws;
static std::mutex g_split_mu;
static float* stream_scratch(std::vector<std::pair<cudaStream_t, StreamWs>>& pool, cudaStream_t st, size_t bytes) {
    std::lock_guard<std::mutex> lk(g_split_mu);
    for (auto& e : pool)
        if (e.first == st) {
            if (e.second.bytes >= bytes) return (float*)e.second.ptr;
            cudaFreeAsync(e.second.ptr, st);
            e.second = {nullptr, 0};
            if (cudaMallocAsync(&e.second.ptr, bytes * 2, st) != cudaSuccess) return nullptr;
            e.second.bytes = bytes * 2;
            return (float*)e.second.ptr;
        }
    StreamWs w{nullptr, 0};
    const size_t cap = bytes * 2 > (16u << 20) ? bytes * 2 : (16u << 20);
    if (cudaMallocAsync(&w.ptr, cap, st) != cudaSuccess) return nullptr;
    w.bytes = cap;
    pool.push_back({st, w});
    return (float*)w.ptr;
}

static void launch_split_tf32(const float* w, int64_t ld, int64_t n, int64_t k, float* out, cudaStream_t st) {
    const long long nk = (long long)n * k;
    long long blocks = (nk + 255) / 256;
    if (blocks > 4LL * num_sms()) blocks = 4LL * num_sms();
    ltc::split_tf32_kernel<<<(unsigned)(blocks > 0 ? blocks : 1), 256, 0, st>>>(w, ld, n, k, out);
    count_launches(1);
}

int linear_tc(const float* x, int64_t ldx, const float* w, int64_t ldw, const float* w_img, const float* bias, const float* row_scale,
              float* y, int64_t ldy, int64_t m, int64_t n, int64_t k, int relu, cudaStream_t st, const GnFuse* gn) {
    if (m < 64 || n < 32 || (n % 16) != 0 || (k % 4) != 0 || (ldx % 4) != 0) return 1;
    if ((reinterpret_cast<uintptr_t>(x) & 15) || (reinterpret_cast<uintptr_t>(w_img) & 15)) return 1;
    if (w_img == nullptr && ((ldw % 4) != 0 || (reinterpret_cast<uintptr_t>(w) & 15))) return 1;
    if (n > 128 && (n % 128) != 0) return 1;
    const int BN = (int)(n >= 128 ? 128 : n);
    const int col_tiles = (int)(n / BN), row_tiles = (int)((m + ltc::BM - 1) / ltc::BM);
    GnFuse g{};
    if (gn != nullptr) {
        g = *gn;
        const int64_t cpg = n / g.groups;
        if (g.groups <= 0 || n % g.groups != 0 || (cpg < 32 ? (32 % cpg) != 0 : (cpg % 32) != 0 || (BN % cpg) != 0) || relu) return 1;
        g.slot_width = (int)(cpg < 32 ? cpg : 32);
    }
    const int nk = (int)((k + ltc::KC - 1) / ltc::KC);
    const int tiles = col_tiles * row_tiles;
    int splits = 1;
    if (g_splitk_on && tiles * 2 <= num_sms() && nk >= 16) {
        splits = nk / 8;
        if (splits > num_sms() / tiles) splits = num_sms() / tiles;
        if (splits > 16) splits = 16;
        if (splits < 2) splits = 1;
    }
    if (gn != nullptr && splits > 1) return 1;
    int cps = nk;
    float* part = nullptr;
    if (splits > 1) {
        cps = (nk + splits - 1) / splits;
        splits = (nk + cps - 1) / cps;
        part = stream_scratch(g_split_ws, st, (size_t)splits * (size_t)m * (size_t)n * sizeof(float));
        if (part == nullptr) { splits = 1; cps = nk; }
    }
    float* img = nullptr;
    if (w_img == nullptr) {
        img = stream_scratch(g_wimg_ws, st, (size_t)2 * (size_t)n * (size_t)k * sizeof(float));
        if (img == nullptr) { set_error("linear_tc: weight image scratch allocation failed"); return -1; }
        w_img = img;
    }
    CUtensorMap mx, mw;
    if (ltc::encode_map(&mx, x, m, k, ldx, ltc::BM)) return -1;
    if (ltc::encode_map(&mw, w_img, 2 * n, k, k, BN)) return -1;
    ProfRec rec{};
    const bool prof = g_prof_on;
    if (prof) {
        cudaEventCreate(&rec.a);
        cudaEventCreate(&rec.b);
        rec.m = m; rec.n = n; rec.k = k;
        cudaEventRecord(rec.a, st);
    }
    if (img != nullptr) launch_split_tf32(w, ldw, n, k, img, st);
    const int num_tiles = tiles * splits;
    const bool persistent = g_persistent_on && splits == 1 && tiles > num_sms();
    const unsigned grid = (unsigned)(persistent ? num_sms() : num_tiles);
    const void* kern = BN <= 32 ? (const void*)ltc::linear_tc_kernel<32> : BN <= 64 ? (const void*)ltc::linear_tc_kernel<64>
                                                                                      : (const void*)ltc::linear_tc_kernel<128>;
    if (ensure_max_smem(kern)) return -1;
#define GEOB_LTC_LAUNCH(BNI)                                                                                                  \
    ltc::linear_tc_kernel<BNI><<<grid, ltc::NTHREADS, ltc::SMEM, st>>>(mx, mw, bias, row_scale, y, (int)ldy, (int)m, (int)n, (int)k, \
                                                                       BN, relu, g, part, cps, col_tiles, row_tiles, num_tiles)
    if (BN <= 32) GEOB_LTC_LAUNCH(32);
    else if (BN <= 64) GEOB_LTC_LAUNCH(64);
    else GEOB_LTC_LAUNCH(128);
#undef GEOB_LTC_LAUNCH
    if (part != nullptr) {
        const long long mn = (long long)m * n;
        ltc::splitk_reduce_kernel<<<(unsigned)((mn / 4 + 255) / 256), 256, 0, st>>>(part, splits, mn, (int)n, bias, row_scale, y, (int)ldy, relu);
        count_launches(1);
    }
    if (prof) {
        cudaEventRecord(rec.b, st);
        std::lock_guard<std::mutex> lk(g_prof_mu);
        g_prof.push_back(rec);
    }
    GEOB_CHECK_LAUNCH();
    count_launches(1);
    return 0;
}

}

extern "C" {

int geob200_set_linear_persistent(int on) {
    geob200::g_persistent_on = on != 0;
    return 0;
}

int geob200_split_tf32(const float* w, int64_t ld, int64_t n, int64_t k, float* out, void* stream) {
    GEOB_REQUIRE(n > 0 && k > 0 && ld >= k, "split_tf32: bad shape (%lld x %lld, ld %lld)", (long long)n, (long long)k, (long long)ld);
    geob200::launch_split_tf32(w, ld, n, k, out, (cudaStream_t)stream);
    GEOB_CHECK_LAUNCH();
    return 0;
}

int geob200_set_split_k(int on) {
    geob200::g_splitk_on = on != 0;
    return 0;
}

int geob200_linear_profile_enable(int on) {
    std::lock_guard<std::mutex> lk(geob200::g_prof_mu);
    for (auto& r : geob200::g_prof) { cudaEventDestroy(r.a); cudaEventDestroy(r.b); }
    geob200::g_prof.clear();
    geob200::g_prof_on = on != 0;
    return 0;
}

int64_t geob200_linear_profile_read(int64_t capacity, int64_t* shapes, float* ms) {
    std::lock_guard<std::mutex> lk(geob200::g_prof_mu);
    int64_t n = 0;
    for (auto& r : geob200::g_prof) {
        if (n >= capacity) break;
        if (cudaEventSynchronize(r.b) != cudaSuccess) break;
        float t = 0.f;
        cudaEventElapsedTime(&t, r.a, r.b);
        shapes[3 * n] = r.m; shapes[3 * n + 1] = r.n; shapes[3 * n + 2] = r.k;
        ms[n] = t;
        ++n;
    }
    return n;
}

}
```

geotransformer_b200/csrc/native.cu:

```cuda
#include "common.cuh"
#include "geob200.h"

namespace geob200 {

struct Ctx {
    Arena ar;
    void* gn_ws;
    size_t gn_ws_bytes;
    void* stream;
    int groups;
    Ctx(void* p, size_t n) : ar(p, n) {}
    float* fl(int64_t rows, int64_t ch) { return ar.take<float>((size_t)rows * (size_t)ch); }
};

#define TRY(expr)                  \
    do {                           \
        int _rc = (expr);          \
        if (_rc != 0) return _rc;  \
    } while (0)

static int run_kpconv(Ctx& c, const geob200_kpconv_t& k, const float* s_feats, const float* q_pts, const float* s_pts,
                      const int64_t* nbr, int64_t m, int64_t ns, int64_t h, float* out) {
    const bool tc = (k.c_in % 32 == 0) && (k.c_out % 16 == 0) && k.c_out >= 32 && (k.c_out <= 128 || k.c_out % 128 == 0) && m >= 64 &&
                    k.weights_t != nullptr;
    if (tc) {
        const size_t wb = geob200_kpconv_tc_workspace_bytes(m, ns, k.c_in);
        const size_t mark = c.ar.off;
        void* ws = c.ar.take<char>(wb);
        GEOB_REQUIRE(c.ar.ok(), "native: arena too small (kpconv)");
        TRY(kpconv_tc_impl(s_feats, q_pts, s_pts, nbr, m, ns, h, k.kernel_points, 15, k.weights_t, k.weights_img, k.bias, k.c_in, k.c_out,
                           k.sigma, out, ws, wb, c.stream));
        c.ar.off = mark;
        return 0;
    }
    const size_t wb = geob200_kpconv_workspace_bytes(ns);
    const size_t mark = c.ar.off;
    void* ws = c.ar.take<char>(wb);
    GEOB_REQUIRE(c.ar.ok(), "native: arena too small (kpconv)");
    TRY(geob200_kpconv(s_feats, q_pts, s_pts, nbr, m, ns, h, k.kernel_points, 15, k.weights, k.bias, k.c_in, k.c_out, k.sigma, out, ws,
                       wb, c.stream));
    c.ar.off = mark;
    return 0;
}

static int run_kpconv_norm(Ctx& c, const geob200_kpconv_t& k, const geob200_norm_t& n, const float* s_feats, const float* q_pts,
                           const float* s_pts, const int64_t* nbr, int64_t m, int64_t ns, int64_t h, float* out, const GnSeg* seg) {
    float* y = c.fl(m, k.c_out);
    GEOB_REQUIRE(c.ar.ok(), "native: arena too small (kpconv output)");
    const bool tc = (k.c_in % 32 == 0) && (k.c_out % 16 == 0) && k.c_out >= 32 && (k.c_out <= 128 || k.c_out % 128 == 0) && m >= 64 &&
                    k.weights_t != nullptr;
    if (tc) {
        const size_t wb = geob200_kpconv_tc_workspace_bytes(m, ns, k.c_in);
        const size_t mark = c.ar.off;
        void* ws = c.ar.take<char>(wb);
        GEOB_REQUIRE(c.ar.ok(), "native: arena too small (kpconv)");
        TRY(kpconv_group_norm_impl(s_feats, q_pts, s_pts, nbr, m, ns, h, k.kernel_points, 15, k.weights_t, k.bias, k.c_in, k.c_out,
                                   k.sigma, c.groups, n.gamma, n.beta, 1e-5f, 1, 0.1f, y, out, c.gn_ws, c.gn_ws_bytes, ws, wb, c.stream, seg,
                                   k.weights_img));
        c.ar.off = mark;
        return 0;
    }
    TRY(run_kpconv(c, k, s_feats, q_pts, s_pts, nbr, m, ns, h, y));
    return group_norm_impl(y, m, k.c_out, c.groups, n.gamma, n.beta, 1e-5f, nullptr, 1, 0.1f, out, c.gn_ws, c.gn_ws_bytes, c.stream, seg);
}

static int run_unary(Ctx& c, const geob200_linear_t& l, const geob200_norm_t& n, const float* x, int64_t rows, const float* residual,
                     int leaky, float* out, const GnSeg* seg) {
    float* t = c.fl(rows, l.c_out);
    GEOB_REQUIRE(c.ar.ok(), "native: arena too small (unary)");
    TRY(linear_group_norm_impl(x, l.c_in, l.weight, l.bias, rows, l.c_out, l.c_in, c.groups, n.gamma, n.beta, 1e-5f, residual, leaky,
                               0.1f, t, out, c.gn_ws, c.gn_ws_bytes, c.stream, seg, l.weight_img));
    return 0;
}

static int run_resblock(Ctx& c, const geob200_resblock_t& b, const float* feats, int64_t ns, const float* q_pts, const float* s_pts,
                        const int64_t* nbr, int64_t m, int64_t h, float* out, const GnSeg* seg_s, const GnSeg* seg_q,
                        const int* cloud_max = nullptr) {
    const float* x = feats;
    if (b.has_unary1) {
        float* u = c.fl(ns, b.unary1.c_out);
        TRY(run_unary(c, b.unary1, b.norm1, feats, ns, nullptr, 1, u, seg_s));
        x = u;
    }
    float* yn = c.fl(m, b.conv.c_out);
    GEOB_REQUIRE(c.ar.ok(), "native: arena too small (resblock)");
    TRY(run_kpconv_norm(c, b.conv, b.norm_conv, x, q_pts, s_pts, nbr, m, ns, h, yn, seg_q));
    const float* sc = feats;
    if (b.strided) {
        float* mp = c.fl(m, b.c_in);
        GEOB_REQUIRE(c.ar.ok(), "native: arena too small (maxpool)");
        if (seg_q != nullptr && cloud_max != nullptr) {
            TRY(maxpool_seg(feats, nbr, m, ns, h, b.c_in, mp, seg_q, cloud_max, c.stream));
        } else {
            TRY(geob200_maxpool(feats, nbr, m, ns, h, b.c_in, mp, c.stream));
        }
        sc = mp;
    }
    if (b.has_shortcut) {
        float* s2 = c.fl(m, b.shortcut.c_out);
        TRY(run_unary(c, b.shortcut, b.norm_sc, sc, m, nullptr, 0, s2, seg_q));
        sc = s2;
    }
    return run_unary(c, b.unary2, b.norm2, yn, m, sc, 1, out, seg_q);
}

}

using namespace geob200;

extern "C" {

size_t geob200_backbone_workspace_bytes(const geob200_backbone_t* net, const int64_t* level_rows) {
    size_t total = 1 << 20;
    for (int l = 0; l < net->num_stages; ++l) {
        const size_t rows = (size_t)level_rows[l];
        const size_t ch = (size_t)net->init_dim << (l + 1);
        total += rows * ch * 4 * 24;
        total += geob200_kpconv_tc_workspace_bytes(level_rows[l], l > 0 ? level_rows[l - 1] : level_rows[l], (int64_t)(ch / 2)) + 4096;
    }
    return total;
}

int geob200_backbone_forward_batched(const geob200_backbone_t* net, const float* feats, const float* const* points,
                                     const int64_t* level_rows, const int64_t* const* neighbors, const int64_t* neighbor_width,
                                     const int64_t* const* subsampling, const int64_t* subsampling_width,
                                     const int64_t* const* upsampling, const int64_t* upsampling_width, float* const* out_feats,
                                     void* gn_workspace, size_t gn_workspace_bytes, void* workspace, size_t workspace_bytes, void* stream,
                                     int64_t n_pairs, const int64_t* const* cloud_rows_h, const int32_t* const* sub_cloud_max) {
    GEOB_REQUIRE(n_pairs == 1 || sub_cloud_max != nullptr, "backbone: batched execution needs the per-cloud subsampling widths");
    GEOB_REQUIRE(net->num_stages >= 2 && net->num_stages <= GEOB200_MAX_STAGES, "backbone: num_stages out of range");
    GEOB_REQUIRE(n_pairs >= 1 && 2 * n_pairs <= GEOB_MAX_CLOUDS, "backbone: 1 <= pairs per batch <= %d", GEOB_MAX_CLOUDS / 2);
    GEOB_REQUIRE(n_pairs == 1 || cloud_rows_h != nullptr, "backbone: batched execution needs the per-cloud row counts of every level");
    Ctx c(workspace, workspace_bytes);
    c.gn_ws = gn_workspace; c.gn_ws_bytes = gn_workspace_bytes; c.stream = stream; c.groups = net->groups;
    const int S = net->num_stages;
    GnSeg segs[GEOB200_MAX_STAGES];
    const GnSeg* sg[GEOB200_MAX_STAGES];
    for (int l = 0; l < S; ++l) {
        sg[l] = nullptr;
        if (n_pairs > 1) {
            GnSeg& g = segs[l];
            g.n_pairs = (int)n_pairs; g.n_clouds = (int)(2 * n_pairs); g.start[0] = 0;
            for (int cl = 0; cl < g.n_clouds; ++cl) g.start[cl + 1] = g.start[cl] + (int)cloud_rows_h[l][cl];
            GEOB_REQUIRE(g.start[g.n_clouds] == level_rows[l], "backbone: cloud rows of level %d do not add up", l);
            sg[l] = &g;
        }
    }
    const float* enc[GEOB200_MAX_STAGES];
    int64_t enc_ch[GEOB200_MAX_STAGES];
    {
        const int64_t n0 = level_rows[0];
        float* yn = c.fl(n0, net->conv1.c_out);
        GEOB_REQUIRE(c.ar.ok(), "native: arena too small (encoder1_1)");
        TRY(run_kpconv_norm(c, net->conv1, net->norm1, feats, points[0], points[0], neighbors[0], n0, n0, neighbor_width[0], yn, sg[0]));
        const geob200_resblock_t& b = net->blocks[0];
        float* o = c.fl(n0, b.unary2.c_out);
        TRY(run_resblock(c, b, yn, n0, points[0], points[0], neighbors[0], n0, neighbor_width[0], o, sg[0], sg[0]));
        enc[0] = o; enc_ch[0] = b.unary2.c_out;
    }
    int bi = 1;
    for (int lvl = 1; lvl < S; ++lvl) {
        const int64_t m = level_rows[lvl], ns = level_rows[lvl - 1];
        const geob200_resblock_t& b1 = net->blocks[bi++];
        float* o1 = c.fl(m, b1.unary2.c_out);
        TRY(run_resblock(c, b1, enc[lvl - 1], ns, points[lvl], points[lvl - 1], subsampling[lvl - 1], m, subsampling_width[lvl - 1], o1,
                         sg[lvl - 1], sg[lvl], sub_cloud_max != nullptr ? sub_cloud_max[lvl - 1] : nullptr));
        const geob200_resblock_t& b2 = net->blocks[bi++];
        float* o2 = c.fl(m, b2.unary2.c_out);
        TRY(run_resblock(c, b2, o1, m, points[lvl], points[lvl], neighbors[lvl], m, neighbor_width[lvl], o2, sg[lvl], sg[lvl]));
        const geob200_resblock_t& b3 = net->blocks[bi++];
        float* o3 = (lvl == S - 1) ? out_feats[0] : c.fl(m, b3.unary2.c_out);
        TRY(run_resblock(c, b3, o2, m, points[lvl], points[lvl], neighbors[lvl], m, neighbor_width[lvl], o3, sg[lvl], sg[lvl]));
        enc[lvl] = o3; enc_ch[lvl] = b3.unary2.c_out;
    }
    const float* latent = enc[S - 1];
    int64_t latent_ch = enc_ch[S - 1];
    int oi = 1;
    for (int lvl = S - 1; lvl >= net->finest_decoder; --lvl) {
        const int64_t m = level_rows[lvl - 1], ns = level_rows[lvl];
        const int64_t c2 = enc_ch[lvl - 1];
        float* cat = c.fl(m, latent_ch + c2);
        GEOB_REQUIRE(c.ar.ok(), "native: arena too small (decoder)");
        TRY(geob200_upsample_concat(latent, upsampling[lvl - 1], upsampling_width[lvl - 1], ns, enc[lvl - 1], m, latent_ch, c2, cat, stream));
        const geob200_linear_t& l = net->decoders[S - 1 - lvl];
        float* o = out_feats[oi++];
        if (lvl == net->finest_decoder) {
            TRY(linear_img(cat, l.c_in, l.weight, l.weight_img, l.bias, o, l.c_out, m, l.c_out, l.c_in, 0, stream));
        } else {
            TRY(run_unary(c, l, net->decoder_norms[S - 1 - lvl], cat, m, nullptr, 1, o, sg[lvl - 1]));
        }
        latent = o; latent_ch = l.c_out;
    }
    GEOB_REQUIRE(c.ar.ok(), "native: arena too small");
    return 0;
}


static int run_tail(Ctx& c, const geob200_tlayer_t& L, const float* hidden, const float* inp, int64_t rows, int64_t ch, float* out) {
    float* h = c.fl(rows, ch);
    float* x = c.fl(rows, ch);
    float* y1 = c.fl(rows, 2 * ch);
    float* y2 = c.fl(rows, ch);
    GEOB_REQUIRE(c.ar.ok(), "native: arena too small (transformer tail)");
    TRY(linear_img(hidden, ch, L.att_linear.weight, L.att_linear.weight_img, L.att_linear.bias, h, ch, rows, ch, ch, 0, c.stream));
    TRY(geob200_add_layernorm(h, inp, L.att_norm.gamma, L.att_norm.beta, rows, ch, 1e-5f, x, c.stream));
    TRY(linear_img(x, ch, L.expand.weight, L.expand.weight_img, L.expand.bias, y1, 2 * ch, rows, 2 * ch, ch, 1, c.stream));
    TRY(linear_img(y1, 2 * ch, L.squeeze.weight, L.squeeze.weight_img, L.squeeze.bias, y2, ch, rows, ch, 2 * ch, 0, c.stream));
    TRY(geob200_add_layernorm(x, y2, L.out_norm.gamma, L.out_norm.beta, rows, ch, 1e-5f, out, c.stream));
    return 0;
}

size_t geob200_transformer_batched_workspace_bytes(int64_t n_pairs, const int64_t* cloud_rows_h, int64_t channels, int64_t heads,
                                                   int64_t num_layers) {
    size_t n = 0, att = 0;
    for (int64_t c = 0; c < 2 * n_pairs; ++c) {
        n += (size_t)cloud_rows_h[c];
        const size_t other = (size_t)cloud_rows_h[(c + n_pairs) % (2 * n_pairs)];
        const size_t m = (size_t)cloud_rows_h[c] > other ? (size_t)cloud_rows_h[c] : other;
        att += align_up((size_t)cloud_rows_h[c] * m * (size_t)heads * 4, 256);
    }
    return (n * (size_t)channels * 4 * (3 + 1 + (size_t)heads + 12)) * (size_t)(num_layers + 1) + att + (2 << 20);
}

int geob200_transformer_forward_batched(const geob200_tlayer_t* layers, int64_t num_layers, int64_t channels, int64_t heads,
                                        const float* x_in, int64_t n_pairs, const int64_t* cloud_rows_h, const float* const* embeddings,
                                        float* out, void* workspace, size_t workspace_bytes, void* stream) {
    GEOB_REQUIRE(n_pairs >= 1 && 2 * n_pairs <= GEOB_MAX_CLOUDS, "transformer: 1 <= pairs per batch <= %d", GEOB_MAX_CLOUDS / 2);
    Ctx c(workspace, workspace_bytes);
    c.stream = stream;
    const int64_t C = channels, H = heads, B = n_pairs, NC = 2 * n_pairs;
    int64_t off[GEOB_MAX_CLOUDS + 1];
    off[0] = 0;
    for (int64_t i = 0; i < NC; ++i) off[i + 1] = off[i] + cloud_rows_h[i];
    const int64_t n = off[NC], R = off[B];
    const float* x = x_in;
    geob200_att_item_t items[GEOB_MAX_CLOUDS];
    size_t att_ws_bytes = 0;
    {
        for (int64_t i = 0; i < NC; ++i) { items[i].n_query = cloud_rows_h[i]; items[i].n_key = cloud_rows_h[i]; }
        att_ws_bytes = geob200_attention_batched_workspace_bytes(items, NC, H);
        for (int64_t p = 0; p < B; ++p) { items[p].n_query = cloud_rows_h[p]; items[p].n_key = cloud_rows_h[B + p]; }
        const size_t cross = geob200_attention_batched_workspace_bytes(items, B, H);
        if (cross > att_ws_bytes) att_ws_bytes = cross;
    }
    void* att_ws = c.fl((int64_t)(att_ws_bytes / 4 + 1), 1);
    for (int64_t i = 0; i < num_layers; ++i) {
        const geob200_tlayer_t& L = layers[i];
        float* y = (i == num_layers - 1) ? out : c.fl(n, C);
        if (L.is_self) {
            float* qkv = c.fl(n, 3 * C);
            float* qp = c.fl(n, H * C);
            float* qb = c.fl(n, H);
            float* hidden = c.fl(n, C);
            GEOB_REQUIRE(c.ar.ok(), "native: arena too small (self layer)");
            TRY(linear_img(x, C, L.w_qkv, L.w_qkv_img, L.b_qkv, qkv, 3 * C, n, 3 * C, C, 0, stream));
            const int64_t d = C / H;
            TRY(geob200_linear_batched(qkv, 3 * C, d, L.wp_t, C, d, nullptr, 0, qp, H * C, C, n, C, d, H, 0, stream));
            TRY(geob200_head_bias(qkv, 3 * C, L.bp, n, C, H, qb, stream));
            for (int64_t cl = 0; cl < NC; ++cl) {
                const int64_t o = off[cl];
                items[cl] = geob200_att_item_t{qkv + o * 3 * C, qkv + o * 3 * C + C, qkv + o * 3 * C + 2 * C, qp + o * H * C, qb + o * H,
                                               embeddings[cl], hidden + o * C, cloud_rows_h[cl], cloud_rows_h[cl]};
            }
            TRY(geob200_attention_batched(items, NC, 3 * C, 3 * C, 3 * C, C, C, H, att_ws, att_ws_bytes, stream));
            TRY(run_tail(c, L, hidden, x, n, C, y));
        } else {
            const int64_t Sn = n - R;
            float* q0 = c.fl(R, C);
            float* kv1 = c.fl(Sn, 2 * C);
            float* hid0 = c.fl(R, C);
            float* q1 = c.fl(Sn, C);
            float* kv0 = c.fl(R, 2 * C);
            float* hid1 = c.fl(Sn, C);
            GEOB_REQUIRE(c.ar.ok(), "native: arena too small (cross layer)");
            TRY(linear_img(x, C, L.w_q, L.w_q_img, L.b_q, q0, C, R, C, C, 0, stream));
            TRY(linear_img(x + R * C, C, L.w_kv, L.w_kv_img, L.b_kv, kv1, 2 * C, Sn, 2 * C, C, 0, stream));
            for (int64_t p = 0; p < B; ++p) {
                const int64_t ro = off[p], so = off[B + p] - R;
                items[p] = geob200_att_item_t{q0 + ro * C, kv1 + so * 2 * C, kv1 + so * 2 * C + C, nullptr, nullptr, nullptr, hid0 + ro * C,
                                              cloud_rows_h[p], cloud_rows_h[B + p]};
            }
            TRY(geob200_attention_batched(items, B, C, 2 * C, 2 * C, C, C, H, att_ws, att_ws_bytes, stream));
            TRY(run_tail(c, L, hid0, x, R, C, y));
            TRY(linear_img(x + R * C, C, L.w_q, L.w_q_img, L.b_q, q1, C, Sn, C, C, 0, stream));
            TRY(linear_img(y, C, L.w_kv, L.w_kv_img, L.b_kv, kv0, 2 * C, R, 2 * C, C, 0, stream));
            for (int64_t p = 0; p < B; ++p) {
                const int64_t ro = off[p], so = off[B + p] - R;
                items[p] = geob200_att_item_t{q1 + so * C, kv0 + ro * 2 * C, kv0 + ro * 2 * C + C, nullptr, nullptr, nullptr, hid1 + so * C,
                                              cloud_rows_h[B + p], cloud_rows_h[p]};
            }
            TRY(geob200_attention_batched(items, B, C, 2 * C, 2 * C, C, C, H, att_ws, att_ws_bytes, stream));
            TRY(run_tail(c, L, hid1, x + R * C, Sn, C, y + R * C));
        }
        x = y;
    }
    return 0;
}

}
```

geotransformer_b200/functional.py:

```python
import ctypes
import math

import torch

from . import _lib as L

_f32, _i64, _u8, _i32 = torch.float32, torch.int64, torch.uint8, torch.int32

GSE_MODE = int(__import__('os').environ.get('GEOB200_GSE_MODE', '5'))
GSE_TABLE_INV_STEP = int(__import__('os').environ.get('GEOB200_GSE_TABLE_INV_STEP', '256'))
GSE_TABLE_D_MAX = float(__import__('os').environ.get('GEOB200_GSE_TABLE_D_MAX', '96'))

EVENTS = None


class _timed:
    def __init__(self, name):
        self.name = name

    def __enter__(self):
        if EVENTS is not None:
            self.s = torch.cuda.Event(enable_timing=True)
            self.e = torch.cuda.Event(enable_timing=True)
            self.s.record()
        return self

    def __exit__(self, *a):
        if EVENTS is not None:
            self.e.record()
            EVENTS.setdefault(self.name, []).append((self.s, self.e))
        return False


def _f(t, name):
    L.require_cuda(t, name, _f32)
    return t


def _detach(t):
    return t.detach() if t is not None and t.requires_grad else t


def _needs_grad(*ts):
    return torch.is_grad_enabled() and any(t is not None and t.requires_grad for t in ts)


_GN_WS = {}


def _gn_workspace(device, groups, rows=0, channels=0, n_pairs=1):
    key = (device.index, L.stream_ptr(), groups)
    lib = L.lib()
    need = lib.geob200_fused_group_norm_workspace_bytes(rows, channels, groups) if rows else lib.geob200_group_norm_workspace_bytes(groups)
    need += 8 * groups * max(int(n_pairs), 1) + 1024
    ws = _GN_WS.get(key)
    if ws is None or ws.numel() < need:
        ws = torch.zeros(max(int(need * 1.5), 1 << 20), dtype=_u8, device=device)
        _GN_WS[key] = ws
    return ws



KPCONV_MODE = 'tc'


def kpconv(s_feats, q_points, s_points, neighbor_indices, kernel_points, weights, bias, sigma, weights_t=None):
    if _needs_grad(s_feats, weights, bias):
        return _KPConv.apply(s_feats, weights, bias, q_points, s_points, neighbor_indices, kernel_points, float(sigma), weights_t)
    return _kpconv(s_feats, q_points, s_points, neighbor_indices, kernel_points, weights, bias, sigma, weights_t)


def _kpconv(s_feats, q_points, s_points, neighbor_indices, kernel_points, weights, bias, sigma, weights_t=None):
    s_feats, weights, bias = _detach(s_feats), _detach(weights), _detach(bias)
    _f(s_feats, 's_feats'); _f(q_points, 'q_points'); _f(s_points, 's_points')
    L.require_cuda(neighbor_indices, 'neighbor_indices', _i64)
    m, h = neighbor_indices.shape
    ns = s_points.shape[0]
    k, cin, cout = weights.shape
    out = torch.empty((m, cout), dtype=_f32, device=s_feats.device)
    lib = L.lib()
    if (KPCONV_MODE == 'tc' and cin % 32 == 0 and cout % 16 == 0 and cout >= 32 and (cout <= 128 or cout % 128 == 0) and m >= 64):
        if weights_t is None:
            weights_t = weights.reshape(k * cin, cout).t().contiguous()
        ws = L.workspace(lib.geob200_kpconv_tc_workspace_bytes(m, ns, cin), s_feats.device, 'kpconv_tc')
        L.check(lib.geob200_kpconv_tc(s_feats.data_ptr(), q_points.data_ptr(), s_points.data_ptr(), neighbor_indices.data_ptr(), m, ns,
                                      h, kernel_points.data_ptr(), k, weights_t.data_ptr(), L.ptr(bias), cin, cout, float(sigma),
                                      out.data_ptr(), ws.data_ptr(), ws.numel(), L.stream_ptr()), 'kpconv_tc')
        return out
    ws = L.workspace(lib.geob200_kpconv_workspace_bytes(ns), s_feats.device, 'kpconv')
    L.check(lib.geob200_kpconv(s_feats.data_ptr(), q_points.data_ptr(), s_points.data_ptr(),
                               neighbor_indices.data_ptr(), m, ns, h, kernel_points.data_ptr(), k,
                               weights.data_ptr(), L.ptr(bias), cin, cout, float(sigma), out.data_ptr(),
                               ws.data_ptr(), ws.numel(), L.stream_ptr()), 'kpconv')
    return out


def kpconv_backward(s_feats, q_points, s_points, neighbor_indices, kernel_points, weights, sigma, grad_out, need_feats=True,
                    need_weights=True, need_bias=True):
    for t, name in ((s_feats, 's_feats'), (q_points, 'q_points'), (s_points, 's_points'), (kernel_points, 'kernel_points'),
                    (weights, 'weights'), (grad_out, 'grad_out')):
        _f(_detach(t), name)
    L.require_cuda(neighbor_indices, 'neighbor_indices', _i64)
    s_feats, weights = _detach(s_feats), _detach(weights)
    m, h = neighbor_indices.shape
    ns = s_points.shape[0]
    k, cin, cout = weights.shape
    if tuple(grad_out.shape) != (m, cout) or tuple(s_feats.shape) != (ns, cin):
        raise RuntimeError(f'kpconv_backward: grad_out must be ({m}, {cout}) and s_feats ({ns}, {cin})')
    dev = s_feats.device
    gf = torch.empty((ns, cin), dtype=_f32, device=dev) if need_feats else None
    gw = torch.empty((k, cin, cout), dtype=_f32, device=dev) if need_weights else None
    gb = torch.empty((cout,), dtype=_f32, device=dev) if need_bias else None
    lib = L.lib()
    ws = L.workspace(lib.geob200_kpconv_backward_workspace_bytes(m, ns, h, cin, cout), dev, 'kpconv_backward')
    L.check(lib.geob200_kpconv_backward(s_feats.data_ptr(), q_points.data_ptr(), s_points.data_ptr(), neighbor_indices.data_ptr(), m, ns, h,
                                        kernel_points.data_ptr(), k, weights.data_ptr(), cin, cout, float(sigma), grad_out.data_ptr(),
                                        L.ptr(gf), L.ptr(gw), L.ptr(gb), ws.data_ptr(), ws.numel(), L.stream_ptr()), 'kpconv_backward')
    return gf, gw, gb


class _KPConv(torch.autograd.Function):
    @staticmethod
    def forward(ctx, s_feats, weights, bias, q_points, s_points, neighbor_indices, kernel_points, sigma, weights_t):
        ctx.save_for_backward(s_feats, weights, q_points, s_points, neighbor_indices, kernel_points)
        ctx.sigma = sigma
        return _kpconv(s_feats, q_points, s_points, neighbor_indices, kernel_points, weights, bias, sigma, weights_t)

    @staticmethod
    def backward(ctx, grad):
        s_feats, weights, q, s, nbr, kp = ctx.saved_tensors
        nf, nw, nb = ctx.needs_input_grad[:3]
        gf, gw, gb = kpconv_backward(s_feats, q, s, nbr, kp, weights, ctx.sigma, grad.contiguous(), nf, nw, nb)
        return gf, gw, gb, None, None, None, None, None, None


def linear(x, weight, bias=None, relu=False, out=None):
    if _needs_grad(x, weight, bias):
        y = _Linear.apply(x, weight, bias, bool(relu))
        return y if out is None else out.copy_(y)
    return _linear(x, weight, bias, relu, out)


def _linear(x, weight, bias=None, relu=False, out=None):
    x, weight, bias = _detach(x), _detach(weight), _detach(bias)
    if not x.is_cuda or x.dtype != _f32 or x.stride(1) != 1:
        raise RuntimeError('linear: x must be a float32 CUDA tensor with unit inner stride')
    L.require_cuda(weight, 'weight', _f32)
    m, k = x.shape
    n = weight.shape[0]
    if out is None:
        out = torch.empty((m, n), dtype=_f32, device=x.device)
    L.check(L.lib().geob200_linear(x.data_ptr(), x.stride(0), weight.data_ptr(), L.ptr(bias), out.data_ptr(),
                                   out.stride(0), m, n, k, int(relu), L.stream_ptr()), 'linear')
    return out


def linear_backward(x, weight, grad_y, need_x=True, need_weight=True, need_bias=True, relu_y=None):
    x, weight = _detach(x), _detach(weight)
    if not x.is_cuda or x.dtype != _f32 or x.stride(1) != 1:
        raise RuntimeError('linear_backward: x must be a float32 CUDA tensor with unit inner stride')
    L.require_cuda(weight, 'weight', _f32); _f(grad_y, 'grad_y')
    m, k = x.shape
    n = weight.shape[0]
    if tuple(grad_y.shape) != (m, n) or weight.shape[1] != k:
        raise RuntimeError(f'linear_backward: grad_y must be ({m}, {n}) and weight ({n}, {k})')
    if relu_y is not None:
        _f(relu_y, 'relu_y')
        if tuple(relu_y.shape) != (m, n):
            raise RuntimeError(f'linear_backward: relu_y must be ({m}, {n})')
    dev = x.device
    wt = weight.t().contiguous() if need_x else None
    gx = torch.empty((m, k), dtype=_f32, device=dev) if need_x else None
    gw = torch.empty((n, k), dtype=_f32, device=dev) if need_weight else None
    gb = torch.empty((n,), dtype=_f32, device=dev) if need_bias else None
    lib = L.lib()
    ws = L.workspace(lib.geob200_linear_backward_workspace_bytes(m, n, k, int(relu_y is not None)), dev, 'linear_backward')
    L.check(lib.geob200_linear_backward(x.data_ptr(), x.stride(0), L.ptr(wt), L.ptr(_detach(relu_y)), m, n, k, grad_y.data_ptr(), L.ptr(gx),
                                        L.ptr(gw), L.ptr(gb), ws.data_ptr(), ws.numel(), L.stream_ptr()), 'linear_backward')
    return gx, gw, gb


class _Linear(torch.autograd.Function):
    @staticmethod
    def forward(ctx, x, weight, bias, relu):
        y = _linear(x, weight, bias, relu)
        ctx.save_for_backward(x, weight, y if relu else None)
        return y

    @staticmethod
    def backward(ctx, grad):
        x, weight, y = ctx.saved_tensors
        return (*linear_backward(x, weight, grad.contiguous(), *ctx.needs_input_grad[:3], relu_y=y), None)


def split_tf32(weight):
    weight = _detach(weight)
    if not weight.is_cuda or weight.dtype != _f32 or weight.dim() != 2 or weight.stride(1) != 1:
        raise RuntimeError('split_tf32: weight must be a 2-D float32 CUDA tensor with unit inner stride')
    n, k = weight.shape
    out = torch.empty((2 * n, k), dtype=_f32, device=weight.device)
    L.check(L.lib().geob200_split_tf32(weight.data_ptr(), weight.stride(0), n, k, out.data_ptr(), L.stream_ptr()), 'split_tf32')
    return out


def group_norm(x, weight, bias, groups, eps=1e-5, negative_slope=None, residual=None, cloud_rows=None):
    if _needs_grad(x, weight, bias, residual):
        return _GroupNorm.apply(x, weight, bias, residual, int(groups), float(eps), negative_slope, cloud_rows)
    if cloud_rows is not None:
        return group_norm_batched(x, weight, bias, groups, cloud_rows, eps, negative_slope, _detach(residual))
    return _group_norm(x, weight, bias, groups, eps, negative_slope, residual)


def group_norm_backward_batched(x, y, weight, groups, cloud_rows, grad_y, eps=1e-5, negative_slope=None, need_residual=False,
                                need_weight=True, need_bias=True):
    x, y, weight = _detach(x), _detach(y), _detach(weight)
    _f(x, 'x'); _f(weight, 'weight'); _f(grad_y, 'grad_y')
    leaky = negative_slope is not None
    if leaky:
        _f(y, 'y')
    n, c = x.shape
    if tuple(grad_y.shape) != (n, c) or (leaky and tuple(y.shape) != (n, c)):
        raise RuntimeError(f'group_norm_backward_batched: grad_y and y must be ({n}, {c})')
    dev = x.device
    np_ = len(cloud_rows) // 2
    gx = torch.empty_like(x)
    gw = torch.empty((c,), dtype=_f32, device=dev) if need_weight else None
    gb = torch.empty((c,), dtype=_f32, device=dev) if need_bias else None
    gr = torch.empty_like(x) if need_residual else None
    lib = L.lib()
    ws = L.workspace(lib.geob200_group_norm_backward_batched_workspace_bytes(n, c, groups, np_), dev, 'group_norm_backward')
    L.check(lib.geob200_group_norm_backward_batched(x.data_ptr(), L.ptr(y) if leaky else None, n, c, groups, weight.data_ptr(), float(eps),
                                                    int(leaky), float(negative_slope or 0.0), grad_y.data_ptr(), gx.data_ptr(), L.ptr(gw),
                                                    L.ptr(gb), L.ptr(gr), ws.data_ptr(), ws.numel(), L.stream_ptr(), np_,
                                                    _host_i64(cloud_rows)), 'group_norm_backward_batched')
    return gx, gw, gb, gr


class _GroupNorm(torch.autograd.Function):
    @staticmethod
    def forward(ctx, x, weight, bias, residual, groups, eps, negative_slope, cloud_rows):
        if cloud_rows is None:
            y = _group_norm(x, weight, bias, groups, eps, negative_slope, residual)
        else:
            y = group_norm_batched(x, weight, bias, groups, cloud_rows, eps, negative_slope, _detach(residual))
        ctx.save_for_backward(x, y, weight)
        ctx.args = (groups, eps, negative_slope, _seg_rows(cloud_rows, x.shape[0]))
        return y

    @staticmethod
    def backward(ctx, grad):
        x, y, weight = ctx.saved_tensors
        groups, eps, slope, rows = ctx.args
        need = ctx.needs_input_grad
        gx, gw, gb, gr = group_norm_backward_batched(x, y, weight, groups, rows, grad.contiguous(), eps, slope, need[3], need[1], need[2])
        return gx if need[0] else None, gw, gb, gr, None, None, None, None


def _seg_rows(cloud_rows, n_rows):
    return [n_rows, 0] if cloud_rows is None else [int(r) for r in cloud_rows]


def _group_norm(x, weight, bias, groups, eps=1e-5, negative_slope=None, residual=None):
    x, weight, bias, residual = _detach(x), _detach(weight), _detach(bias), _detach(residual)
    _f(x, 'x')
    n, c = x.shape
    ws = _gn_workspace(x.device, groups)
    y = torch.empty_like(x)
    L.check(L.lib().geob200_group_norm(x.data_ptr(), n, c, groups, weight.data_ptr(), bias.data_ptr(), float(eps),
                                       L.ptr(residual), int(negative_slope is not None),
                                       float(negative_slope or 0.0), y.data_ptr(), ws.data_ptr(), ws.numel(),
                                       L.stream_ptr()), 'group_norm')
    return y


def linear_group_norm(x, weight, bias, gn_weight, gn_bias, groups, eps=1e-5, negative_slope=None, residual=None, cloud_rows=None):
    if _needs_grad(x, weight, bias, gn_weight, gn_bias, residual):
        return _LinearGroupNorm.apply(x, weight, bias, gn_weight, gn_bias, residual, int(groups), float(eps), negative_slope, cloud_rows)
    if cloud_rows is not None:
        return linear_group_norm_batched(x, weight, bias, gn_weight, gn_bias, groups, cloud_rows, eps, negative_slope, _detach(residual))
    return _linear_group_norm(x, weight, bias, gn_weight, gn_bias, groups, eps, negative_slope, residual)


class _LinearGroupNorm(torch.autograd.Function):
    @staticmethod
    def forward(ctx, x, weight, bias, gn_weight, gn_bias, residual, groups, eps, negative_slope, cloud_rows):
        pre = torch.empty((x.shape[0], weight.shape[0]), dtype=_f32, device=x.device)
        if cloud_rows is None:
            y = _linear_group_norm(x, weight, bias, gn_weight, gn_bias, groups, eps, negative_slope, residual, pre=pre)
        else:
            y = linear_group_norm_batched(x, weight, bias, gn_weight, gn_bias, groups, cloud_rows, eps, negative_slope, _detach(residual),
                                          pre=pre)
        ctx.save_for_backward(x, weight, gn_weight, pre, y)
        ctx.args = (groups, eps, negative_slope, _seg_rows(cloud_rows, pre.shape[0]))
        return y

    @staticmethod
    def backward(ctx, grad):
        x, weight, gn_weight, pre, y = ctx.saved_tensors
        groups, eps, slope, rows = ctx.args
        need = ctx.needs_input_grad
        gpre, ggw, ggb, gr = group_norm_backward_batched(pre, y, gn_weight, groups, rows, grad.contiguous(), eps, slope, need[5], need[3],
                                                         need[4])
        gx, gw, gb = linear_backward(x, weight, gpre, need[0], need[1], need[2]) if any(need[:3]) else (None, None, None)
        return gx, gw, gb, ggw, ggb, gr, None, None, None, None


def _linear_group_norm(x, weight, bias, gn_weight, gn_bias, groups, eps=1e-5, negative_slope=None, residual=None, pre=None):
    x, weight, bias, gn_weight, gn_bias = _detach(x), _detach(weight), _detach(bias), _detach(gn_weight), _detach(gn_bias)
    residual = _detach(residual)
    if not x.is_cuda or x.dtype != _f32 or x.stride(1) != 1:
        raise RuntimeError('linear_group_norm: x must be a float32 CUDA tensor with unit inner stride')
    L.require_cuda(weight, 'weight', _f32)
    m, k = x.shape
    n = weight.shape[0]
    if pre is None:
        pre = scratch((m, n), x.device, 'pre_norm')
    y = torch.empty((m, n), dtype=_f32, device=x.device)
    ws = _gn_workspace(x.device, groups, m, n)
    L.check(L.lib().geob200_linear_group_norm(x.data_ptr(), x.stride(0), weight.data_ptr(), L.ptr(bias), m, n, k, groups,
                                              gn_weight.data_ptr(), gn_bias.data_ptr(), float(eps), L.ptr(residual),
                                              int(negative_slope is not None), float(negative_slope or 0.0), pre.data_ptr(),
                                              y.data_ptr(), ws.data_ptr(), ws.numel(), L.stream_ptr()), 'linear_group_norm')
    return y


def kpconv_group_norm(s_feats, q_points, s_points, neighbor_indices, kernel_points, weights, bias, sigma, gn_weight, gn_bias, groups,
                      eps=1e-5, negative_slope=0.1, weights_t=None, cloud_rows=None):
    m, h = neighbor_indices.shape
    k, cin, cout = weights.shape
    if not (KPCONV_MODE == 'tc' and cin % 32 == 0 and cout % 16 == 0 and cout >= 32 and (cout <= 128 or cout % 128 == 0) and m >= 64):
        x = kpconv(s_feats, q_points, s_points, neighbor_indices, kernel_points, weights, bias, sigma, weights_t=weights_t)
        return group_norm(x, gn_weight, gn_bias, groups, eps, negative_slope=negative_slope, cloud_rows=cloud_rows)
    if _needs_grad(s_feats, weights, bias, gn_weight, gn_bias):
        return _KPConvGroupNorm.apply(s_feats, weights, bias, gn_weight, gn_bias, q_points, s_points, neighbor_indices, kernel_points,
                                      float(sigma), int(groups), float(eps), negative_slope, weights_t, cloud_rows)
    return _kpconv_group_norm(s_feats, q_points, s_points, neighbor_indices, kernel_points, weights, bias, sigma, gn_weight, gn_bias,
                              groups, eps, negative_slope, weights_t, cloud_rows=cloud_rows)


class _KPConvGroupNorm(torch.autograd.Function):
    @staticmethod
    def forward(ctx, s_feats, weights, bias, gn_weight, gn_bias, q_points, s_points, neighbor_indices, kernel_points, sigma, groups, eps,
                negative_slope, weights_t, cloud_rows):
        pre = torch.empty((neighbor_indices.shape[0], weights.shape[2]), dtype=_f32, device=s_feats.device)
        y = _kpconv_group_norm(s_feats, q_points, s_points, neighbor_indices, kernel_points, weights, bias, sigma, gn_weight, gn_bias,
                               groups, eps, negative_slope, weights_t, pre=pre, cloud_rows=cloud_rows)
        ctx.save_for_backward(s_feats, weights, gn_weight, q_points, s_points, neighbor_indices, kernel_points, pre, y)
        ctx.args = (sigma, groups, eps, negative_slope, _seg_rows(cloud_rows, pre.shape[0]))
        return y

    @staticmethod
    def backward(ctx, grad):
        s_feats, weights, gn_weight, q, s, nbr, kp, pre, y = ctx.saved_tensors
        sigma, groups, eps, slope, rows = ctx.args
        need = ctx.needs_input_grad
        gpre, ggw, ggb, _ = group_norm_backward_batched(pre, y, gn_weight, groups, rows, grad.contiguous(), eps, slope, False, need[3],
                                                        need[4])
        gf, gw, gb = kpconv_backward(s_feats, q, s, nbr, kp, weights, sigma, gpre, need[0], need[1], need[2])
        return gf, gw, gb, ggw, ggb, None, None, None, None, None, None, None, None, None, None


def _kpconv_group_norm(s_feats, q_points, s_points, neighbor_indices, kernel_points, weights, bias, sigma, gn_weight, gn_bias, groups,
                       eps=1e-5, negative_slope=0.1, weights_t=None, pre=None, cloud_rows=None):
    m, h = neighbor_indices.shape
    k, cin, cout = weights.shape
    s_feats, weights, bias, gn_weight, gn_bias = _detach(s_feats), _detach(weights), _detach(bias), _detach(gn_weight), _detach(gn_bias)
    _f(s_feats, 's_feats'); _f(q_points, 'q_points'); _f(s_points, 's_points')
    L.require_cuda(neighbor_indices, 'neighbor_indices', _i64)
    ns = s_points.shape[0]
    dev = s_feats.device
    if weights_t is None:
        weights_t = weights.reshape(k * cin, cout).t().contiguous()
    lib = L.lib()
    if pre is None:
        pre = scratch((m, cout), dev, 'pre_norm')
    y = torch.empty((m, cout), dtype=_f32, device=dev)
    ws = L.workspace(lib.geob200_kpconv_tc_workspace_bytes(m, ns, cin), dev, 'kpconv_tc')
    if cloud_rows is not None:
        gws = _gn_workspace(dev, groups, m, cout, n_pairs=len(cloud_rows) // 2)
        L.check(lib.geob200_kpconv_group_norm_batched(
            s_feats.data_ptr(), q_points.data_ptr(), s_points.data_ptr(), neighbor_indices.data_ptr(), m, ns, h, kernel_points.data_ptr(), k,
            weights_t.data_ptr(), L.ptr(bias), cin, cout, float(sigma), groups, gn_weight.data_ptr(), gn_bias.data_ptr(), float(eps),
            int(negative_slope is not None), float(negative_slope or 0.0), pre.data_ptr(), y.data_ptr(), gws.data_ptr(), gws.numel(),
            ws.data_ptr(), ws.numel(), L.stream_ptr(), len(cloud_rows) // 2, _host_i64(cloud_rows)), 'kpconv_group_norm_batched')
        return y
    gws = _gn_workspace(dev, groups, m, cout)
    L.check(lib.geob200_kpconv_group_norm(s_feats.data_ptr(), q_points.data_ptr(), s_points.data_ptr(), neighbor_indices.data_ptr(),
                                          m, ns, h, kernel_points.data_ptr(), k, weights_t.data_ptr(), L.ptr(bias), cin, cout,
                                          float(sigma), groups, gn_weight.data_ptr(), gn_bias.data_ptr(), float(eps),
                                          int(negative_slope is not None), float(negative_slope or 0.0), pre.data_ptr(),
                                          y.data_ptr(), gws.data_ptr(), gws.numel(), ws.data_ptr(), ws.numel(), L.stream_ptr()),
            'kpconv_group_norm')
    return y


def _host_i64(values):
    values = [int(v) for v in values]
    return (ctypes.c_int64 * len(values))(*values)


def group_norm_batched(x, weight, bias, groups, cloud_rows, eps=1e-5, negative_slope=None, residual=None):
    x, weight, bias = _detach(x), _detach(weight), _detach(bias)
    _f(x, 'x')
    n, c = x.shape
    np_ = len(cloud_rows) // 2
    ws = _gn_workspace(x.device, groups, n, c, n_pairs=np_)
    y = torch.empty_like(x)
    L.check(L.lib().geob200_group_norm_batched(x.data_ptr(), n, c, groups, weight.data_ptr(), bias.data_ptr(), float(eps), L.ptr(residual),
                                               int(negative_slope is not None), float(negative_slope or 0.0), y.data_ptr(), ws.data_ptr(),
                                               ws.numel(), L.stream_ptr(), np_, _host_i64(cloud_rows)), 'group_norm_batched')
    return y


def linear_group_norm_batched(x, weight, bias, gn_weight, gn_bias, groups, cloud_rows, eps=1e-5, negative_slope=None, residual=None,
                              pre=None):
    x, weight, bias, gn_weight, gn_bias = _detach(x), _detach(weight), _detach(bias), _detach(gn_weight), _detach(gn_bias)
    m, k = x.shape
    n = weight.shape[0]
    np_ = len(cloud_rows) // 2
    if pre is None:
        pre = scratch((m, n), x.device, 'pre_norm')
    y = torch.empty((m, n), dtype=_f32, device=x.device)
    ws = _gn_workspace(x.device, groups, m, n, n_pairs=np_)
    L.check(L.lib().geob200_linear_group_norm_batched(x.data_ptr(), x.stride(0), weight.data_ptr(), L.ptr(bias), m, n, k, groups,
                                                      gn_weight.data_ptr(), gn_bias.data_ptr(), float(eps), L.ptr(residual),
                                                      int(negative_slope is not None), float(negative_slope or 0.0), pre.data_ptr(),
                                                      y.data_ptr(), ws.data_ptr(), ws.numel(), L.stream_ptr(), np_, _host_i64(cloud_rows)),
            'linear_group_norm_batched')
    return y


def maxpool(x, neighbor_indices, cloud_rows=None, cloud_max=None):
    if (cloud_rows is None) != (cloud_max is None):
        raise RuntimeError('maxpool: cloud_rows and cloud_max come together')
    if _needs_grad(x):
        return _Maxpool.apply(x, neighbor_indices, cloud_rows, cloud_max)
    return _maxpool(x, neighbor_indices, cloud_rows, cloud_max)


def _maxpool(x, neighbor_indices, cloud_rows=None, cloud_max=None):
    x = _detach(x)
    _f(x, 'x'); L.require_cuda(neighbor_indices, 'neighbor_indices', _i64)
    m, h = neighbor_indices.shape
    y = torch.empty((m, x.shape[1]), dtype=_f32, device=x.device)
    if cloud_rows is not None:
        L.require_cuda(cloud_max, 'cloud_max', _i32)
        if cloud_max.numel() != len(cloud_rows):
            raise RuntimeError('maxpool: cloud_max needs one entry per cloud')
        L.check(L.lib().geob200_maxpool_batched(x.data_ptr(), neighbor_indices.data_ptr(), m, x.shape[0], h, x.shape[1], cloud_max.data_ptr(),
                                                len(cloud_rows) // 2, _host_i64(cloud_rows), y.data_ptr(), L.stream_ptr()), 'maxpool_batched')
        return y
    L.check(L.lib().geob200_maxpool(x.data_ptr(), neighbor_indices.data_ptr(), m, x.shape[0], h, x.shape[1],
                                    y.data_ptr(), L.stream_ptr()), 'maxpool')
    return y


def cloud_max_count(neighbor_indices, n_support, cloud_rows):
    L.require_cuda(neighbor_indices, 'neighbor_indices', _i64)
    out = torch.empty((len(cloud_rows),), dtype=_i32, device=neighbor_indices.device)
    L.check(L.lib().geob200_cloud_max_count(neighbor_indices.data_ptr(), neighbor_indices.shape[0], int(n_support), neighbor_indices.shape[1],
                                            len(cloud_rows) // 2, _host_i64(cloud_rows), out.data_ptr(), L.stream_ptr()), 'cloud_max_count')
    return out


def maxpool_backward_batched(x, neighbor_indices, cloud_rows, grad_y, cloud_max=None):
    x = _detach(x)
    _f(x, 'x'); _f(grad_y, 'grad_y'); L.require_cuda(neighbor_indices, 'neighbor_indices', _i64)
    if cloud_max is not None:
        L.require_cuda(cloud_max, 'cloud_max', _i32)
        if cloud_max.numel() != len(cloud_rows):
            raise RuntimeError('maxpool_backward_batched: cloud_max needs one entry per cloud')
    m, h = neighbor_indices.shape
    ns, c = x.shape
    if tuple(grad_y.shape) != (m, c):
        raise RuntimeError(f'maxpool_backward_batched: grad_y must be ({m}, {c})')
    gx = torch.empty_like(x)
    lib = L.lib()
    ws = L.workspace(lib.geob200_maxpool_backward_batched_workspace_bytes(m, ns, h, c), x.device, 'maxpool_backward')
    L.check(lib.geob200_maxpool_backward_batched(x.data_ptr(), neighbor_indices.data_ptr(), m, ns, h, c, L.ptr(cloud_max), len(cloud_rows) // 2,
                                                 _host_i64(cloud_rows), grad_y.data_ptr(), gx.data_ptr(), ws.data_ptr(), ws.numel(),
                                                 L.stream_ptr()), 'maxpool_backward_batched')
    return gx


class _Maxpool(torch.autograd.Function):
    @staticmethod
    def forward(ctx, x, neighbor_indices, cloud_rows, cloud_max):
        ctx.save_for_backward(x, neighbor_indices, cloud_max)
        ctx.rows = _seg_rows(cloud_rows, neighbor_indices.shape[0])
        return _maxpool(x, neighbor_indices, cloud_rows, cloud_max)

    @staticmethod
    def backward(ctx, grad):
        x, nbr, cloud_max = ctx.saved_tensors
        return maxpool_backward_batched(x, nbr, ctx.rows, grad.contiguous(), cloud_max), None, None, None


def upsample_concat(x, upsample_indices, skip=None):
    if _needs_grad(x, skip):
        return _UpsampleConcat.apply(x, skip, upsample_indices)
    return _upsample_concat(x, upsample_indices, skip)


def upsample_concat_backward(upsample_indices, n_support, c1, grad_y, need_skip=True):
    _f(grad_y, 'grad_y')
# ... 1788 lines not shown
```

include/geob200.h:

```cpp
#ifndef GEOB200_H
#define GEOB200_H

#include <stddef.h>
#include <stdint.h>

#ifdef __cplusplus
extern "C" {
#endif

const char* geob200_last_error(void);
uint64_t geob200_launch_count(void);


size_t geob200_grid_subsample_workspace_bytes(int64_t n_points, int64_t batch);
int geob200_grid_subsample(const float* points, int64_t n_points, const int64_t* lengths_h, int64_t batch, float voxel,
                           float* s_points, int64_t* s_lengths, void* workspace, size_t workspace_bytes, void* stream);

size_t geob200_radius_search_workspace_bytes(int64_t n_query, int64_t n_support, int64_t batch);
int geob200_radius_search(const float* q_points, int64_t n_query, const float* s_points, int64_t n_support,
                          const int64_t* q_lengths_h, const int64_t* s_lengths_h, int64_t batch, float radius,
                          int64_t width, int64_t* out, int32_t* counts, int32_t* max_count, void* workspace,
                          size_t workspace_bytes, void* stream);

int geob200_neighbor_histogram(const int64_t* neighbors, int64_t n_rows, int64_t width, int64_t n_support, int64_t hist_n,
                               int32_t* hist, void* stream);


size_t geob200_kpconv_workspace_bytes(int64_t n_support);
int geob200_kpconv(const float* s_feats, const float* q_points, const float* s_points, const int64_t* neighbors,
                   int64_t n_query, int64_t n_support, int64_t n_neighbors, const float* kernel_points, int64_t n_kernel,
                   const float* weights, const float* bias, int64_t c_in, int64_t c_out, float sigma, float* out,
                   void* workspace, size_t workspace_bytes, void* stream);

size_t geob200_kpconv_tc_workspace_bytes(int64_t n_query, int64_t n_support, int64_t c_in);
int geob200_kpconv_tc(const float* s_feats, const float* q_points, const float* s_points, const int64_t* neighbors, int64_t n_query,
                      int64_t n_support, int64_t n_neighbors, const float* kernel_points, int64_t n_kernel, const float* weights_t,
                      const float* bias, int64_t c_in, int64_t c_out, float sigma, float* out, void* workspace, size_t workspace_bytes,
                      void* stream);

int geob200_split_tf32(const float* w, int64_t ld, int64_t n, int64_t k, float* out, void* stream);

void geob200_set_linear_mode(int mode);
int geob200_linear(const float* x, int64_t ldx, const float* weight, const float* bias, float* y, int64_t ldy, int64_t m,
                   int64_t n, int64_t k, int relu, void* stream);
int geob200_linear_batched(const float* x, int64_t ldx, int64_t stride_x, const float* weight, int64_t ldw, int64_t stride_w,
                           const float* bias, int64_t stride_b, float* y, int64_t ldy, int64_t stride_y, int64_t m, int64_t n,
                           int64_t k, int64_t batch, int relu, void* stream);

size_t geob200_group_norm_workspace_bytes(int64_t groups);
int geob200_group_norm(const float* x, int64_t n_rows, int64_t channels, int64_t groups, const float* gamma,
                       const float* beta, float eps, const float* residual, int leaky, float slope, float* y,
                       void* workspace, size_t workspace_bytes, void* stream);

size_t geob200_fused_group_norm_workspace_bytes(int64_t n_rows, int64_t channels, int64_t groups);
int geob200_linear_group_norm(const float* x, int64_t ldx, const float* weight, const float* bias, int64_t m, int64_t n, int64_t k,
                              int64_t groups, const float* gamma, const float* beta, float eps, const float* residual, int leaky,
                              float slope, float* pre_norm, float* y, void* workspace, size_t workspace_bytes, void* stream);
int geob200_kpconv_group_norm(const float* s_feats, const float* q_points, const float* s_points, const int64_t* neighbors,
                              int64_t n_query, int64_t n_support, int64_t n_neighbors, const float* kernel_points, int64_t n_kernel,
                              const float* weights_t, const float* bias, int64_t c_in, int64_t c_out, float sigma, int64_t groups,
                              const float* gamma, const float* beta, float eps, int leaky, float slope, float* pre_norm, float* y,
                              void* gn_workspace, size_t gn_workspace_bytes, void* workspace, size_t workspace_bytes, void* stream);

int geob200_group_norm_batched(const float* x, int64_t n_rows, int64_t channels, int64_t groups, const float* gamma, const float* beta,
                               float eps, const float* residual, int leaky, float slope, float* y, void* workspace, size_t workspace_bytes,
                               void* stream, int64_t n_pairs, const int64_t* cloud_rows_h);
int geob200_linear_group_norm_batched(const float* x, int64_t ldx, const float* weight, const float* bias, int64_t m, int64_t n, int64_t k,
                                      int64_t groups, const float* gamma, const float* beta, float eps, const float* residual, int leaky,
                                      float slope, float* pre_norm, float* y, void* workspace, size_t workspace_bytes, void* stream,
                                      int64_t n_pairs, const int64_t* cloud_rows_h);
int geob200_kpconv_group_norm_batched(const float* s_feats, const float* q_points, const float* s_points, const int64_t* neighbors,
                                      int64_t n_query, int64_t n_support, int64_t n_neighbors, const float* kernel_points, int64_t n_kernel,
                                      const float* weights_t, const float* bias, int64_t c_in, int64_t c_out, float sigma, int64_t groups,
                                      const float* gamma, const float* beta, float eps, int leaky, float slope, float* pre_norm, float* y,
                                      void* gn_workspace, size_t gn_workspace_bytes, void* workspace, size_t workspace_bytes, void* stream,
                                      int64_t n_pairs, const int64_t* cloud_rows_h);

int geob200_maxpool(const float* x, const int64_t* neighbors, int64_t n_query, int64_t n_support, int64_t n_neighbors,
                    int64_t channels, float* y, void* stream);
int geob200_maxpool_batched(const float* x, const int64_t* neighbors, int64_t n_query, int64_t n_support, int64_t n_neighbors,
                            int64_t channels, const int32_t* cloud_max, int64_t n_pairs, const int64_t* cloud_rows_h, float* y,
                            void* stream);

int geob200_cloud_max_count(const int64_t* neighbors, int64_t n_query, int64_t n_support, int64_t n_neighbors, int64_t n_pairs,
                            const int64_t* cloud_rows_h, int32_t* cloud_max, void* stream);

int geob200_upsample_concat(const float* x, const int64_t* up_indices, int64_t up_stride, int64_t n_support,
                            const float* skip, int64_t n_query, int64_t c1, int64_t c2, float* y, void* stream);


size_t geob200_kpconv_backward_workspace_bytes(int64_t n_query, int64_t n_support, int64_t n_neighbors, int64_t c_in, int64_t c_out);
int geob200_kpconv_backward(const float* s_feats, const float* q_points, const float* s_points, const int64_t* neighbors, int64_t n_query,
                            int64_t n_support, int64_t n_neighbors, const float* kernel_points, int64_t n_kernel, const float* weights,
                            int64_t c_in, int64_t c_out, float sigma, const float* grad_out, float* grad_feats, float* grad_weights,
                            float* grad_bias, void* workspace, size_t workspace_bytes, void* stream);

size_t geob200_linear_backward_workspace_bytes(int64_t m, int64_t n, int64_t k, int relu);
int geob200_linear_backward(const float* x, int64_t ldx, const float* weight_t, const float* relu_y, int64_t m, int64_t n, int64_t k,
                            const float* grad_y, float* grad_x, float* grad_weight, float* grad_bias, void* workspace, size_t workspace_bytes,
                            void* stream);

size_t geob200_group_norm_backward_batched_workspace_bytes(int64_t n_rows, int64_t channels, int64_t groups, int64_t n_pairs);
int geob200_group_norm_backward_batched(const float* x, const float* y, int64_t n_rows, int64_t channels, int64_t groups, const float* gamma,
                                        float eps, int leaky, float slope, const float* grad_y, float* grad_x, float* grad_gamma,
                                        float* grad_beta, float* grad_residual, void* workspace, size_t workspace_bytes, void* stream,
                                        int64_t n_pairs, const int64_t* cloud_rows_h);

size_t geob200_maxpool_backward_batched_workspace_bytes(int64_t n_query, int64_t n_support, int64_t n_neighbors, int64_t channels);
int geob200_maxpool_backward_batched(const float* x, const int64_t* neighbors, int64_t n_query, int64_t n_support, int64_t n_neighbors,
                                     int64_t channels, const int32_t* cloud_max, int64_t n_pairs, const int64_t* cloud_rows_h,
                                     const float* grad_y, float* grad_x, void* workspace, size_t workspace_bytes, void* stream);

size_t geob200_upsample_concat_backward_workspace_bytes(int64_t n_query, int64_t n_support);
int geob200_upsample_concat_backward(const int64_t* up_indices, int64_t up_stride, int64_t n_query, int64_t n_support, int64_t c1, int64_t c2,
                                     const float* grad_y, float* grad_x, float* grad_skip, void* workspace, size_t workspace_bytes,
                                     void* stream);


int geob200_point_to_node_partition_batched(const float* points, const float* nodes, int64_t n_clouds, const int64_t* cloud_points,
                                            const int64_t* cloud_nodes, int64_t point_limit, int64_t* point_to_node, uint8_t* node_masks,
                                            int32_t* node_sizes, int64_t* node_knn_indices, uint8_t* node_knn_masks, void* stream);

int geob200_knn_partition(const float* points, int64_t n_points, const float* nodes, int64_t n_nodes, int64_t k,
                          int64_t* knn_indices, float* knn_sq_distances, void* stream);
int geob200_pairwise_distance(const float* x, int64_t n, const float* y, int64_t m, int64_t channels, int normalized, float* out,
                              void* stream);
int geob200_point_to_node_indices(const float* points, int64_t n_points, const float* nodes, int64_t n_nodes, int64_t* indices,
                                  int32_t* node_sizes, void* stream);
int geob200_apply_transform(const float* points, int64_t n_points, const float* transform, float* out, void* stream);

int geob200_gather_rows(const float* table, int64_t n_rows, int64_t channels, const int64_t* indices, int64_t n_indices,
                        float* out, void* stream);


int geob200_gse_indices_batched(const float* points, int64_t n_clouds, const int64_t* cloud_rows_h, float sigma_d, float factor_a,
                                int64_t angle_k, float* d_indices, float* a_indices, void* stream);

size_t geob200_gse_embed_workspace_bytes(int64_t n, int64_t channels);
int geob200_gse_embed_pairs(const float* d_indices, const float* a_indices, int64_t n_rows, int64_t channels, const float* div_term,
                            const float* wd_t, const float* wa_t, const float* wd, const float* wa, const float* bd, const float* ba,
                            float* embeddings, int mode, void* workspace, size_t workspace_bytes, void* stream);

size_t geob200_gse_table_bytes(int64_t channels, int64_t inv_step, float d_max, float a_max);
int geob200_gse_table_build(const float* div_term, const float* wd_t, const float* wa_t, const float* bd, const float* ba,
                            int64_t channels, int64_t inv_step, float d_max, float a_max, void* table, size_t table_bytes,
                            void* stream);
int geob200_gse_embed_table(const float* d_indices, const float* a_indices, int64_t n_rows, int64_t channels, const void* table,
                            size_t table_bytes, int64_t inv_step, float d_max, float a_max, const float* div_term, const float* wd,
                            const float* wa, const float* bd, const float* ba, float* embeddings, void* stream);

size_t geob200_attention_workspace_bytes(int64_t n_query, int64_t n_key, int64_t heads);
int geob200_attention(const float* q, int64_t ldq, const float* k, int64_t ldk, const float* v, int64_t ldv, const float* qp,
                      const float* qb, const float* embed, int64_t n_query, int64_t n_key, int64_t channels, int64_t heads,
                      float* out, int64_t ldo, void* workspace, size_t workspace_bytes, void* stream);
#define GEOB200_ATT_MAX_ITEMS 32
typedef struct { const float* q; const float* k; const float* v; const float* qp; const float* qb; const float* embed; float* out;
                 int64_t n_query, n_key; } geob200_att_item_t;
size_t geob200_attention_batched_workspace_bytes(const geob200_att_item_t* items_h, int64_t n_items, int64_t heads);
int geob200_attention_batched(const geob200_att_item_t* items_h, int64_t n_items, int64_t ldq, int64_t ldk, int64_t ldv, int64_t ldo,
                              int64_t channels, int64_t heads, void* workspace, size_t workspace_bytes, void* stream);
int geob200_attention_batched_keeps_probs(const geob200_att_item_t* items_h, int64_t n_items, int64_t channels, int64_t heads);
int geob200_set_attention_tma(int on);
int geob200_head_bias(const float* q, int64_t ldq, const float* bias_p, int64_t n, int64_t channels, int64_t heads, float* qb,
                      void* stream);
int geob200_add_layernorm(const float* a, const float* b, const float* gamma, const float* beta, int64_t n, int64_t channels,
                          float eps, float* y, void* stream);
int geob200_l2_normalize(const float* x, int64_t n, int64_t channels, float* y, void* stream);


size_t geob200_add_layernorm_backward_workspace_bytes(int64_t n, int64_t channels);
int geob200_add_layernorm_backward(const float* a, const float* b, const float* gamma, int64_t n, int64_t channels, float eps,
                                   const float* grad_y, float* grad_x, float* grad_gamma, float* grad_beta, void* workspace,
                                   size_t workspace_bytes, void* stream);
int geob200_l2_normalize_backward(const float* x, int64_t n, int64_t channels, const float* grad_y, float* grad_x, void* stream);
size_t geob200_head_project_backward_workspace_bytes(int64_t n, int64_t channels, int64_t heads);
int geob200_head_project_backward(const float* q, int64_t ldq, const float* wp, const float* bp, int64_t n, int64_t channels, int64_t heads,
                                  const float* grad_qp, const float* grad_qb, float* grad_q, int64_t ldgq, float* grad_wp, float* grad_bp,
                                  void* workspace, size_t workspace_bytes, void* stream);
typedef struct { const float* probs; const float* grad_out; float* grad_q; float* grad_k; float* grad_v; float* grad_qp; float* grad_qb;
                 float* grad_embed; } geob200_att_grad_item_t;
size_t geob200_attention_backward_batched_workspace_bytes(const geob200_att_item_t* items_h, int64_t n_items, int64_t heads);
int geob200_attention_backward_batched(const geob200_att_item_t* items_h, const geob200_att_grad_item_t* grads_h, int64_t n_items,
                                       int64_t ldq, int64_t ldk, int64_t ldv, int64_t ldo, int64_t ldgq, int64_t ldgk, int64_t ldgv,
                                       int64_t channels, int64_t heads, void* workspace, size_t workspace_bytes, void* stream);
size_t geob200_gse_embed_backward_workspace_bytes(int64_t n_rows, int64_t channels);
int geob200_gse_embed_backward(const float* d_indices, const float* a_indices, int64_t n_rows, int64_t angle_k, int64_t channels,
                               const void* table, size_t table_bytes, int64_t inv_step, float d_max, float a_max, const float* div_term,
                               const float* wa, const float* ba, const float* grad_embed, float* grad_wd, float* grad_bd, float* grad_wa,
                               float* grad_ba, void* workspace, size_t workspace_bytes, void* stream);


size_t geob200_superpoint_matching_batched_workspace_bytes(int64_t n_rows, int64_t n_products, int64_t n_pairs);
int geob200_superpoint_matching_batched(const float* ref_feats, const float* src_feats, int64_t channels, const uint8_t* ref_masks,
                                        const uint8_t* src_masks, int64_t n_pairs, const int64_t* cloud_nodes, int64_t num_correspondences,
                                        int dual, int64_t* corr_indices, float* corr_scores, int32_t* num_out, void* workspace,
                                        size_t workspace_bytes, void* stream);

int geob200_gather_patches_batched(const int64_t* corr_indices, int64_t n_corr, int64_t n_clouds, const int64_t* cloud_nodes,
                                   const int64_t* cloud_points, const int64_t* node_knn_indices, const uint8_t* node_knn_masks, int64_t k,
                                   const float* points, int64_t* out_indices, uint8_t* out_masks, float* out_points, void* stream);

int geob200_patch_scores_batched(const float* ref_feats, const float* src_feats, int64_t channels, int64_t n_pairs, const int64_t* cloud_points,
                                 const int64_t* ref_knn_indices, const int64_t* src_knn_indices, int64_t n_patches, int64_t k,
                                 float* scores, void* stream);

size_t geob200_patch_scores_backward_batched_workspace_bytes(int64_t n_rows, int64_t n_patches_total, int64_t k, int64_t channels);
int geob200_patch_scores_backward_batched(const float* ref_feats, const float* src_feats, int64_t channels, int64_t n_pairs,
                                          const int64_t* cloud_points, const int64_t* ref_knn_indices, const int64_t* src_knn_indices,
                                          int64_t n_patches, int64_t k, const float* grad_scores, float* grad_ref_feats,
                                          float* grad_src_feats, void* workspace, size_t workspace_bytes, void* stream);

int geob200_sinkhorn(const float* scores, const uint8_t* row_masks, const uint8_t* col_masks, const float* alpha,
                     int64_t n_patches, int64_t k, int64_t num_iterations, float inf, float* out, void* stream);

size_t geob200_sinkhorn_backward_workspace_bytes(int64_t n_patches, int64_t k, int64_t num_iterations);
int geob200_sinkhorn_backward(const float* scores, const uint8_t* row_masks, const uint8_t* col_masks, const float* alpha, int64_t n_patches,
                              int64_t k, int64_t num_iterations, float inf, const float* grad_out, float* grad_scores, float* grad_alpha,
                              void* workspace, size_t workspace_bytes, void* stream);


size_t geob200_lgr_batched_workspace_bytes(int64_t n_pairs, int64_t n_patches, int64_t k, int64_t topk);
int geob200_local_global_registration_batched(const float* ref_knn_points, const float* src_knn_points, const uint8_t* ref_knn_masks,
                                              const uint8_t* src_knn_masks, const float* log_scores, int64_t n_pairs, int64_t n_patches,
                                              int64_t k, int64_t score_ld, int64_t topk, float acceptance_radius, int mutual,
                                              float confidence_threshold, int64_t correspondence_threshold, int64_t num_refinement_steps,
                                              float* ref_corr_points, float* src_corr_points, float* corr_scores, int32_t* corr_patch,
                                              int32_t* num_corr, float* estimated_transform, int64_t transform_ld, float* patch_transforms,
                                              int32_t* patch_inliers, int32_t* best_patch, void* workspace, size_t workspace_bytes,
                                              void* stream);

int geob200_weighted_procrustes(const float* src_points, const float* ref_points, const float* weights, int64_t batch,
                                int64_t n, float weight_thresh, float eps, float* transforms, void* stream);

size_t geob200_node_correspondences_batched_workspace_bytes(int64_t n_rows, int64_t n_products, int64_t k);
int geob200_node_correspondences_batched(const float* ref_nodes, const float* src_nodes, const float* ref_knn_points,
                                         const float* src_knn_points, const uint8_t* ref_masks, const uint8_t* src_masks,
                                         const uint8_t* ref_knn_masks, const uint8_t* src_knn_masks, int64_t n_pairs, const int64_t* cloud_nodes,
                                         int64_t k, const float* transforms, float pos_radius, int64_t* corr_indices, float* corr_overlaps,
                                         int32_t* count, void* workspace, size_t workspace_bytes, void* stream);

int geob200_evaluate_counts(const int64_t* gt_node_corr_indices, const float* gt_node_corr_overlaps, int64_t n_gt, const int32_t* n_gt_dev,
                            float acceptance_overlap, const int64_t* ref_node_corr_indices, const int64_t* src_node_corr_indices,
                            int64_t n_node_corr, const int32_t* n_node_corr_dev, const float* ref_corr_points, const float* src_corr_points,
                            int64_t n_corr, const int32_t* n_corr_dev, float acceptance_radius, const float* gt_transform,
                            const float* est_transform, const float* src_points, int64_t n_src_points, int mode, float rmse_threshold,
                            float rre_threshold, float rte_threshold, float* metrics, void* stream);
int geob200_evaluate_batched(const int64_t* gt_node_corr_indices, const float* gt_node_corr_overlaps, const int32_t* n_gt_dev,
                             float acceptance_overlap, const int64_t* ref_node_corr_indices, const int64_t* src_node_corr_indices,
                             int64_t n_node_corr, const int32_t* n_node_corr_dev, const float* ref_corr_points, const float* src_corr_points,
                             int64_t n_corr, const int32_t* n_corr_dev, float acceptance_radius, const float* gt_transforms,
                             const float* est_transforms, int64_t transform_ld, const float* points, int64_t n_pairs, const int64_t* cloud_nodes,
                             const int64_t* cloud_points, int mode, float rmse_threshold, float rre_threshold, float rte_threshold,
                             float* metrics, int64_t metrics_ld, void* stream);

size_t geob200_coarse_matching_loss_batched_workspace_bytes(int64_t n_rows, int64_t n_products);
int geob200_coarse_matching_loss_batched(const float* ref_feats, const float* src_feats, int64_t channels, int64_t n_pairs,
                                         const int64_t* cloud_nodes, const int64_t* gt_node_corr_indices, const float* gt_node_corr_overlaps,
                                         const int32_t* gt_count, float positive_margin, float negative_margin, float positive_optimal,
                                         float negative_optimal, float log_scale, float positive_overlap, float* out, int64_t out_ld,
                                         void* workspace, size_t workspace_bytes, void* stream);
size_t geob200_fine_matching_loss_batched_workspace_bytes(int64_t n_pairs, int64_t n_patches);
int geob200_fine_matching_loss_batched(const float* ref_knn_points, const float* src_knn_points, const uint8_t* ref_knn_masks,
                                       const uint8_t* src_knn_masks, const float* matching_scores, const float* transforms, int64_t n_pairs,
                                       int64_t n_patches, int64_t k, const int32_t* patch_count, double positive_radius,
                                       const float* loss_weights, float* out, int64_t out_ld, void* workspace, size_t workspace_bytes,
                                       void* stream);

size_t geob200_coarse_matching_loss_backward_batched_workspace_bytes(int64_t n_rows, int64_t n_products, int64_t n_pairs);
int geob200_coarse_matching_loss_backward_batched(const float* ref_feats, const float* src_feats, int64_t channels, int64_t n_pairs,
                                                  const int64_t* cloud_nodes, const int64_t* gt_node_corr_indices,
                                                  const float* gt_node_corr_overlaps, const int32_t* gt_count, float positive_margin,
                                                  float negative_margin, float positive_optimal, float negative_optimal, float log_scale,
                                                  float positive_overlap, const float* grad_rows, int64_t grad_ld, const float* loss_weights,
                                                  float* grad_ref_feats, float* grad_src_feats, void* workspace, size_t workspace_bytes,
                                                  void* stream);
size_t geob200_fine_matching_loss_backward_batched_workspace_bytes(int64_t n_pairs, int64_t n_patches);
int geob200_fine_matching_loss_backward_batched(const float* ref_knn_points, const float* src_knn_points, const uint8_t* ref_knn_masks,
                                                const uint8_t* src_knn_masks, const float* transforms, int64_t n_pairs, int64_t n_patches,
                                                int64_t k, const int32_t* patch_count, double positive_radius, const float* grad_rows,
                                                int64_t grad_ld, const float* loss_weights, float* grad_scores, void* workspace,
                                                size_t workspace_bytes, void* stream);

size_t geob200_ransac_correspondences_batched_workspace_bytes(int64_t n_pairs, int64_t num_iterations);
int geob200_ransac_correspondences_batched(const float* ref_corr_points, const float* src_corr_points, int64_t n_pairs, int64_t capacity,
                                           const int32_t* num_corr, float distance_threshold, int64_t ransac_n, int64_t num_iterations,
                                           uint64_t seed, int64_t pair_base, float* transforms, float* fitness, float* inlier_rmse,
                                           int32_t* inlier_count,
                                           int32_t* best_iteration, float* hyp_transforms, int32_t* hyp_inliers, float* hyp_rmse,
                                           int32_t* hyp_samples, void* workspace, size_t workspace_bytes, void* stream);

size_t geob200_correspondence_metrics_batched_workspace_bytes(int64_t n_pairs, int64_t capacity);
int geob200_correspondence_metrics_batched(const float* ref_corr_points, const float* src_corr_points, int64_t n_pairs, int64_t capacity,
                                           const int32_t* num_corr, const float* transforms, int64_t transform_ld, float positive_radius,
                                           float* out, int64_t out_ld, void* workspace, size_t workspace_bytes, void* stream);

size_t geob200_feature_nn_batched_workspace_bytes(int64_t n_pairs, int64_t cap_query, int64_t cap_support);
int geob200_feature_nn_batched(const float* query, const float* support, int64_t n_pairs, int64_t cap_query, int64_t cap_support,
                               int64_t channels, const int32_t* n_query, const int32_t* n_support, int64_t* query_index,
                               double* query_dist, int64_t* support_index, double* support_dist, void* workspace, size_t workspace_bytes,
                               void* stream);
int geob200_feature_corr_indices(const int64_t* ref_nn, const double* ref_dist, const int64_t* src_nn, const double* src_dist,
                                 int64_t n_ref, int64_t n_src, int32_t mode, int64_t* ref_corr, int64_t* src_corr, float* feat_dist,
                                 int32_t* count, void* stream);
size_t geob200_ransac_features_batched_workspace_bytes(int64_t n_pairs, int64_t cap_src, int64_t cap_ref, int64_t num_iterations,
                                                       int64_t val_iterations);
int geob200_ransac_features_batched(const float* src_points, const float* ref_points, const float* src_feats, const float* ref_feats,
                                    int64_t n_pairs, int64_t cap_src, int64_t cap_ref, int64_t channels, const int32_t* n_src,
                                    const int32_t* n_ref, float distance_threshold, int64_t ransac_n, int64_t num_iterations,
                                    int64_t val_iterations, uint64_t seed, int64_t pair_base, float* transforms, float* fitness,
                                    float* inlier_rmse, int32_t* inlier_count, int32_t* best_iteration, int32_t* num_validated,
                                    int64_t* rec_matches, int32_t* rec_samples, int32_t* rec_pass, int32_t* rec_val_ids,
                                    float* rec_transforms, int32_t* rec_inliers, float* rec_rmse, void* workspace, size_t workspace_bytes,
                                    void* stream);

int geob200_corr_order_batched(const float* scores, int64_t n_pairs, int64_t capacity, const int32_t* num_corr, int64_t kmax, int32_t* order,
                               void* stream);
int geob200_corr_select_batched(const float* ref_corr_points, const float* src_corr_points, const float* corr_scores, int64_t n_pairs,
                                int64_t capacity, const int32_t* num_corr, const int32_t* order, int64_t kmax, int64_t k,
                                float* ref_out, float* src_out, float* scores_out, int32_t* count_out, void* stream);
size_t geob200_sparse_correspondence_eval_batched_workspace_bytes(int64_t n_pairs, int64_t m_cap, int64_t n_cap);
int geob200_sparse_correspondence_eval_batched(const int64_t* ref_node_corr_indices, const int64_t* src_node_corr_indices, int64_t pred_cap,
                                               const int32_t* pred_count, const int64_t* gt_node_corr_indices, int64_t gt_cap,
                                               const int32_t* gt_count, int64_t n_pairs, int64_t m_cap, int64_t n_cap, double* out,
                                               void* workspace, size_t workspace_bytes, void* stream);
int geob200_registration_error_batched(const float* gt_transforms, int64_t gt_ld, const float* est_transforms, int64_t est_ld,
                                       const float* covariances, const int32_t* has_covariance, int64_t n_pairs, int mode,
                                       double threshold0, double threshold1, double* out, void* stream);
int geob200_weighted_procrustes_counts(const float* src_points, const float* ref_points, const float* weights, int64_t batch,
                                       int64_t capacity, const int32_t* counts, float weight_thresh, float eps, float* transforms,
                                       void* stream);

int geob200_linear_profile_enable(int on);
int geob200_set_split_k(int on);
int geob200_set_linear_persistent(int on);
int64_t geob200_linear_profile_read(int64_t capacity, int64_t* shapes, float* ms);

#define GEOB200_MAX_STAGES 6
typedef struct { const float* weight; const float* bias; int64_t c_in, c_out; const float* weight_img; } geob200_linear_t;
typedef struct { const float* gamma; const float* beta; } geob200_norm_t;
typedef struct { const float* weights; const float* weights_t; const float* bias; const float* kernel_points;
                 int64_t c_in, c_out; float sigma; const float* weights_img; } geob200_kpconv_t;
typedef struct {
    int32_t has_unary1, has_shortcut, strided, reserved;
    int64_t c_in;
    geob200_linear_t unary1; geob200_norm_t norm1;
    geob200_kpconv_t conv;   geob200_norm_t norm_conv;
    geob200_linear_t unary2; geob200_norm_t norm2;
    geob200_linear_t shortcut; geob200_norm_t norm_sc;
} geob200_resblock_t;
typedef struct {
    int32_t num_stages, finest_decoder, groups, init_dim;
    geob200_kpconv_t conv1; geob200_norm_t norm1;
    geob200_resblock_t blocks[1 + 3 * (GEOB200_MAX_STAGES - 1)];
    geob200_linear_t decoders[GEOB200_MAX_STAGES];
    geob200_norm_t decoder_norms[GEOB200_MAX_STAGES];
} geob200_backbone_t;
size_t geob200_backbone_workspace_bytes(const geob200_backbone_t* net, const int64_t* level_rows);
int geob200_backbone_forward_batched(const geob200_backbone_t* net, const float* feats, const float* const* points,
                                     const int64_t* level_rows, const int64_t* const* neighbors, const int64_t* neighbor_width,
                                     const int64_t* const* subsampling, const int64_t* subsampling_width,
                                     const int64_t* const* upsampling, const int64_t* upsampling_width, float* const* out_feats,
                                     void* gn_workspace, size_t gn_workspace_bytes, void* workspace, size_t workspace_bytes, void* stream,
                                     int64_t n_pairs, const int64_t* const* cloud_rows_h, const int32_t* const* sub_cloud_max);

typedef struct {
    int32_t is_self, reserved;
    const float* w_qkv; const float* b_qkv; const float* w_q; const float* b_q; const float* w_kv; const float* b_kv;
    const float* wp_t; const float* bp;
    geob200_linear_t att_linear; geob200_norm_t att_norm;
    geob200_linear_t expand; geob200_linear_t squeeze; geob200_norm_t out_norm;
    const float* w_qkv_img; const float* w_q_img; const float* w_kv_img;
} geob200_tlayer_t;
size_t geob200_transformer_batched_workspace_bytes(int64_t n_pairs, const int64_t* cloud_rows_h, int64_t channels, int64_t heads,
                                                   int64_t num_layers);
int geob200_transformer_forward_batched(const geob200_tlayer_t* layers, int64_t num_layers, int64_t channels, int64_t heads,
                                        const float* x, int64_t n_pairs, const int64_t* cloud_rows_h, const float* const* embeddings_h,
                                        float* out, void* workspace, size_t workspace_bytes, void* stream);

size_t geob200_superpoint_targets_batched_workspace_bytes(int64_t n_gt_rows);
int geob200_superpoint_targets_batched(const int64_t* gt_indices, const float* gt_overlaps, const int32_t* gt_count, int64_t n_pairs,
                                       const int64_t* cloud_nodes, float overlap_threshold, int64_t num_targets, uint64_t seed,
                                       uint64_t iteration, int64_t pair_base, int64_t* corr_indices, float* corr_scores, int32_t* num_out,
                                       void* workspace, size_t workspace_bytes, void* stream);

int geob200_nonfinite_check(const float* const* ptrs, const int64_t* numels, int64_t n_tensors, int64_t max_numel, float* found_inf,
                            void* stream);

int geob200_batch_loss_weights(const float* loss_rows, int64_t ld_rows, int64_t n_pairs, float* weights, float* mean_row, float* n_valid,
                               float* found_inf, void* stream);

#define GEOB200_AUGMENT_3DMATCH 0
#define GEOB200_AUGMENT_KITTI 1
#define GEOB200_AUGMENT_TAG_BASE 0xA6000000u

size_t geob200_augment_pairs_batched_workspace_bytes(int64_t n_rows);
int geob200_augment_pairs_batched(const float* points, const int64_t* lengths_h, int64_t n_pairs, const float* transforms, int mode,
                                  int64_t point_limit, double noise, double rotation_factor, double min_scale, double max_scale,
                                  double shift, uint64_t seed, uint64_t iteration, int64_t pair_base, float* out_points, int32_t* origin,
                                  float* out_transforms, double* record, void* workspace, size_t workspace_bytes, void* stream);

size_t geob200_modelnet_pairs_batched_workspace_bytes(int64_t n_rows);
int geob200_modelnet_pairs_batched(const float* shapes, const int64_t* lengths_h, int64_t n_pairs, int64_t num_points, double keep_ratio,
                                   double rotation_magnitude, double translation_magnitude, double noise_magnitude, uint64_t seed,
                                   uint64_t iteration, int64_t pair_base, float* out_points, int32_t* origin, float* out_transforms,
                                   double* record, void* workspace, size_t workspace_bytes, void* stream);

size_t geob200_modelnet_benchmark_pairs_batched_workspace_bytes(int64_t n_pairs, int64_t num_points);
int geob200_modelnet_benchmark_pairs_batched(const float* shapes, const int64_t* lengths_h, const int64_t* indices_h, int64_t n_pairs,
                                             int64_t num_points, double keep_ratio, double rotation_magnitude, double translation_magnitude,
                                             double noise_magnitude, float* out_points, int32_t* origin, float* out_transforms,
                                             void* workspace, size_t workspace_bytes, void* stream);

#ifdef __cplusplus
}
#endif
#endif
```

Baseline: 435.1.

## Split decoder linear across the upsample-concat to run the latent GEMM at coarse resolution

The decoder no longer upsamples and concatenates the latent with the skip features before a single linear. It now multiplies the latent part by its slice of the weight at the coarse level (fewer rows), then gathers those partial products through the upsample index table inside the fine-level GEMM epilogue while computing the skip part. An extra producer warp prefetches the gathered accumulator rows into L2 using bulk prefetch. This removes the concat buffer write and the redundant GEMM work on duplicated rows, at the cost of a second launch, a gather in the epilogue, and extra kernel template variants.

```diff
diff --git a/geotransformer_b200/_lib.py b/geotransformer_b200/_lib.py
--- a/geotransformer_b200/_lib.py
+++ b/geotransformer_b200/_lib.py
@@ -45,6 +45,10 @@
 _sig('geob200_linear_group_norm_batched', c_int, P, I64, P, P, I64, I64, I64, I64, P, P, F, P, c_int, F, P, P, P, SZ, P, I64, P)
 _sig('geob200_maxpool', c_int, P, P, I64, I64, I64, I64, P, P)
 _sig('geob200_upsample_concat', c_int, P, P, I64, I64, P, I64, I64, I64, P, P)
+_sig('geob200_linear_partial_out', c_int, P, I64, P, I64, I64, I64, I64, P, P)
+_sig('geob200_linear_partial_in', c_int, P, I64, P, P, P, P, I64, I64, P, I64, I64, I64, I64, I64, c_int, P)
+_sig('geob200_linear_group_norm_partial_in_batched', c_int, P, I64, P, P, P, P, I64, I64, I64, I64, I64, I64, I64, P, P, F, P, c_int, F,
+     P, P, P, SZ, P, I64, P)
 _sig('geob200_kpconv_backward_workspace_bytes', SZ, I64, I64, I64, I64, I64)
 _sig('geob200_kpconv_backward', c_int, P, P, P, P, I64, I64, I64, P, I64, P, I64, I64, F, P, P, P, P, P, SZ, P)
 _sig('geob200_linear_backward_workspace_bytes', SZ, I64, I64, I64, c_int)
@@ -130,6 +134,7 @@
 _sig('geob200_linear_profile_enable', c_int, c_int)
 _sig('geob200_set_split_k', c_int, c_int)
 _sig('geob200_set_linear_persistent', c_int, c_int)
+_sig('geob200_set_decoder_split', c_int, c_int)
 _sig('geob200_linear_profile_read', I64, I64, P, P)
 _sig('geob200_backbone_workspace_bytes', SZ, P, P)
 _sig('geob200_backbone_forward_batched', c_int, P, P, P, P, P, P, P, P, P, P, P, P, SZ, P, SZ, P, I64, P, P)
diff --git a/geotransformer_b200/csrc/common.cuh b/geotransformer_b200/csrc/common.cuh
--- a/geotransformer_b200/csrc/common.cuh
+++ b/geotransformer_b200/csrc/common.cuh
@@ -93,6 +93,17 @@
                            const GnSeg* seg, const float* w_img = nullptr);
 int linear_img(const float* x, int64_t ldx, const float* weight, const float* w_img, const float* bias, float* y, int64_t ldy,
                int64_t m, int64_t n, int64_t k, int relu, void* stream);
+bool decoder_split_applies(int64_t m, int64_t n, int64_t k, int64_t k1, const float* w_img);
+int linear_partial_out_impl(const float* x, int64_t ldx, const float* w_img, int64_t m, int64_t n, int64_t k, int64_t k1, float* acc,
+                            void* stream);
+int linear_partial_in_impl(const float* skip, int64_t ldx, const float* w_img, const float* bias, const float* acc, const int64_t* up,
+                           int64_t up_stride, int64_t n_support, float* y, int64_t ldy, int64_t m, int64_t n, int64_t k, int64_t k1, int relu,
+                           void* stream);
+int linear_group_norm_partial_in_impl(const float* skip, int64_t ldx, const float* w_img, const float* bias, const float* acc,
+                                      const int64_t* up, int64_t up_stride, int64_t n_support, int64_t m, int64_t n, int64_t k, int64_t k1,
+                                      int64_t groups, const float* gamma, const float* beta, float eps, const float* residual, int leaky,
+                                      float slope, float* pre_norm, float* y, void* workspace, size_t workspace_bytes, void* stream,
+                                      const GnSeg* seg);
 int kpconv_tc_impl(const float* s_feats, const float* q_points, const float* s_points, const int64_t* neighbors, int64_t n_query,
                    int64_t n_support, int64_t n_neighbors, const float* kernel_points, int64_t n_kernel, const float* weights_t,
                    const float* w_img, const float* bias, int64_t c_in, int64_t c_out, float sigma, float* out, void* workspace,
diff --git a/geotransformer_b200/csrc/kpconv.cu b/geotransformer_b200/csrc/kpconv.cu
--- a/geotransformer_b200/csrc/kpconv.cu
+++ b/geotransformer_b200/csrc/kpconv.cu
@@ -821,6 +821,11 @@
 namespace geob200 {
 int linear_tc(const float* x, int64_t ldx, const float* w, int64_t ldw, const float* w_img, const float* bias, const float* row_scale, float* y, int64_t ldy,
               int64_t m, int64_t n, int64_t k, int relu, cudaStream_t st, const GnFuse* gn = nullptr);
+int linear_tc_partial(const float* x, int64_t ldx, const float* w_img, int64_t k, int64_t k1, const float* bias, float* y, int64_t ldy,
+                      int64_t m, int64_t n, int relu, float* acc_out, const float* acc_in, const int64_t* up, int64_t up_stride,
+                      int64_t n_support, cudaStream_t st, const GnFuse* gn);
+bool linear_tc_sequential(int64_t m, int64_t n, int64_t k);
+bool decoder_split_enabled();
 static int g_linear_mode = 1;
 }
 
@@ -1184,6 +1189,83 @@
 }
 
 namespace geob200 {
+bool decoder_split_applies(int64_t m, int64_t n, int64_t k, int64_t k1, const float* w_img) {
+    return decoder_split_enabled() && g_linear_mode == 1 && w_img != nullptr && k1 > 0 && k1 < k && k1 % 32 == 0 && (k - k1) % 4 == 0 &&
+           linear_tc_sequential(m, n, k);
+}
+
+#define TRY_ARGS(expr)             \
+    do {                           \
+        int _rc = (expr);          \
+        if (_rc != 0) return _rc;  \
+    } while (0)
+
+static int partial_args(const float* x, int64_t ldx, const float* w_img, const float* acc, int64_t m, int64_t n, int64_t k, int64_t k1,
+                        bool out_mode, const char* what) {
+    GEOB_REQUIRE(x != nullptr && w_img != nullptr && acc != nullptr, "%s: null input", what);
+    GEOB_REQUIRE(m >= 1 && n >= 32 && n % 16 == 0 && (n <= 128 || n % 128 == 0), "%s: unsupported shape (%lld x %lld)", what, (long long)m,
+                 (long long)n);
+    GEOB_REQUIRE(k1 > 0 && k1 < k && k1 % 32 == 0 && k % 4 == 0, "%s: k1 = %lld must be a multiple of 32 in (0, k = %lld), k a multiple of 4",
+                 what, (long long)k1, (long long)k);
+    const int64_t kp = out_mode ? k1 : k - k1;
+    GEOB_REQUIRE(ldx >= kp && ldx % 4 == 0, "%s: ldx %lld must be >= %lld and a multiple of 4", what, (long long)ldx, (long long)kp);
+    GEOB_REQUIRE(((reinterpret_cast<uintptr_t>(x) | reinterpret_cast<uintptr_t>(w_img) | reinterpret_cast<uintptr_t>(acc)) & 15) == 0,
+                 "%s: x, w_img and the accumulator image must be 16-byte aligned", what);
+    return 0;
+}
+
+int linear_partial_out_impl(const float* x, int64_t ldx, const float* w_img, int64_t m, int64_t n, int64_t k, int64_t k1, float* acc,
+                            void* stream) {
+    TRY_ARGS(partial_args(x, ldx, w_img, acc, m, n, k, k1, true, "linear_partial_out"));
+    const int rc = linear_tc_partial(x, ldx, w_img, k, k1, nullptr, nullptr, 0, m, n, 0, acc, nullptr, nullptr, 0, 0, (cudaStream_t)stream,
+                                     nullptr);
+    GEOB_REQUIRE(rc <= 0, "linear_partial_out: shape not handled by the tensor-core GEMM");
+    return rc;
+}
+
+int linear_partial_in_impl(const float* skip, int64_t ldx, const float* w_img, const float* bias, const float* acc, const int64_t* up,
+                           int64_t up_stride, int64_t n_support, float* y, int64_t ldy, int64_t m, int64_t n, int64_t k, int64_t k1, int relu,
+                           void* stream) {
+    TRY_ARGS(partial_args(skip, ldx, w_img, acc, m, n, k, k1, false, "linear_partial_in"));
+    GEOB_REQUIRE(up != nullptr && y != nullptr && up_stride >= 1 && n_support >= 1 && ldy >= n, "linear_partial_in: bad output / index table");
+    const int rc = linear_tc_partial(skip, ldx, w_img, k, k1, bias, y, ldy, m, n, relu, nullptr, acc, up, up_stride, n_support,
+                                     (cudaStream_t)stream, nullptr);
+    GEOB_REQUIRE(rc <= 0, "linear_partial_in: shape not handled by the tensor-core GEMM");
+    return rc;
+}
+
+int linear_group_norm_partial_in_impl(const float* skip, int64_t ldx, const float* w_img, const float* bias, const float* acc,
+                                      const int64_t* up, int64_t up_stride, int64_t n_support, int64_t m, int64_t n, int64_t k, int64_t k1,
+                                      int64_t groups, const float* gamma, const float* beta, float eps, const float* residual, int leaky,
+                                      float slope, float* pre_norm, float* y, void* workspace, size_t workspace_bytes, void* stream,
+                                      const GnSeg* seg) {
+    cudaStream_t st = (cudaStream_t)stream;
+    const int64_t np = (seg != nullptr && seg->n_pairs > 1) ? seg->n_pairs : 1;
+    TRY_ARGS(partial_args(skip, ldx, w_img, acc, m, n, k, k1, false, "linear_partial_in"));
+    GEOB_REQUIRE(up != nullptr && pre_norm != nullptr && y != nullptr && gamma != nullptr && beta != nullptr && up_stride >= 1 &&
+                 n_support >= 1, "linear_group_norm_partial_in: null input or bad index table");
+    GEOB_REQUIRE(groups > 0 && n % groups == 0, "linear_group_norm_partial_in: bad group count");
+    GEOB_REQUIRE(workspace != nullptr && workspace_bytes >= (np > 1 ? fused_group_norm_workspace_bytes_batched(m, n, groups, np)
+                                                                     : geob200_fused_group_norm_workspace_bytes(m, n, groups)),
+                 "linear_group_norm_partial_in: workspace too small");
+    const GnWs w = gn_carve(workspace, workspace_bytes, groups, np);
+    GnFuse gn{(int)groups, 0, w.partial};
+    int rc = linear_tc_partial(skip, ldx, w_img, k, k1, bias, pre_norm, n, m, n, 0, nullptr, acc, up, up_stride, n_support, st, &gn);
+    if (rc < 0) return rc;
+    if (rc == 0) {
+        if (np > 1) {
+            launch_gn_seg_apply(pre_norm, w, gamma, beta, residual, y, m, n, groups, eps, leaky, slope, *seg, st);
+        } else {
+            launch_gn_apply(pre_norm, w, gamma, beta, residual, y, m, n, groups, eps, leaky, slope, st);
+            count_launches(2);
+        }
+        GEOB_CHECK_LAUNCH();
+        return 0;
+    }
+    TRY_ARGS(linear_partial_in_impl(skip, ldx, w_img, bias, acc, up, up_stride, n_support, pre_norm, n, m, n, k, k1, 0, stream));
+    return group_norm_impl(pre_norm, m, n, groups, gamma, beta, eps, residual, leaky, slope, y, workspace, workspace_bytes, stream, seg);
+}
+
 int make_seg(GnSeg* g, int64_t n_pairs, const int64_t* cloud_rows_h, int64_t n_rows, const char* what) {
     GEOB_REQUIRE(n_pairs >= 1 && 2 * n_pairs <= GEOB_MAX_CLOUDS && cloud_rows_h != nullptr, "%s: 1 <= pairs per batch <= %d", what,
                  GEOB_MAX_CLOUDS / 2);
@@ -1216,6 +1298,32 @@
     if (geob200::make_seg(&seg, n_pairs, cloud_rows_h, m, "group_norm")) return -2;
     return geob200::linear_group_norm_impl(x, ldx, weight, bias, m, n, k, groups, gamma, beta, eps, residual, leaky, slope, pre_norm, y,
                                            workspace, workspace_bytes, stream, &seg);
+}
+
+int geob200_linear_partial_out(const float* x, int64_t ldx, const float* w_img, int64_t m, int64_t n, int64_t k, int64_t k1, float* acc,
+                               void* stream) {
+    return geob200::linear_partial_out_impl(x, ldx, w_img, m, n, k, k1, acc, stream);
+}
+
+int geob200_linear_partial_in(const float* skip, int64_t ldx, const float* w_img, const float* bias, const float* acc,
+                              const int64_t* up_indices, int64_t up_stride, int64_t n_support, float* y, int64_t ldy, int64_t m, int64_t n,
+                              int64_t k, int64_t k1, int relu, void* stream) {
+    return geob200::linear_partial_in_impl(skip, ldx, w_img, bias, acc, up_indices, up_stride, n_support, y, ldy, m, n, k, k1, relu, stream);
+}
+
+int geob200_linear_group_norm_partial_in_batched(const float* skip, int64_t ldx, const float* w_img, const float* bias, const float* acc,
+                                                 const int64_t* up_indices, int64_t up_stride, int64_t n_support, int64_t m, int64_t n,
+                                                 int64_t k, int64_t k1, int64_t groups, const float* gamma, const float* beta, float eps,
+                                                 const float* residual, int leaky, float slope, float* pre_norm, float* y, void* workspace,
+                                                 size_t workspace_bytes, void* stream, int64_t n_pairs, const int64_t* cloud_rows_h) {
+    geob200::GnSeg seg;
+    const geob200::GnSeg* sp = nullptr;
+    if (n_pairs != 1 || cloud_rows_h != nullptr) {
+        if (geob200::make_seg(&seg, n_pairs, cloud_rows_h, m, "linear_group_norm_partial_in")) return -2;
+        sp = &seg;
+    }
+    return geob200::linear_group_norm_partial_in_impl(skip, ldx, w_img, bias, acc, up_indices, up_stride, n_support, m, n, k, k1, groups, gamma,
+                                                      beta, eps, residual, leaky, slope, pre_norm, y, workspace, workspace_bytes, stream, sp);
 }
 
 int geob200_cloud_max_count(const int64_t* neighbors, int64_t n_query, int64_t n_support, int64_t n_neighbors, int64_t n_pairs,
diff --git a/geotransformer_b200/csrc/linear_tc.cu b/geotransformer_b200/csrc/linear_tc.cu
--- a/geotransformer_b200/csrc/linear_tc.cu
+++ b/geotransformer_b200/csrc/linear_tc.cu
@@ -35,13 +35,16 @@
     }
 }
 
-template <int BNI>
+enum { PLAIN = 0, PARTIAL_OUT = 1, PARTIAL_IN = 2 };
+template <int BNI, int MODE>
 __global__ void __launch_bounds__(NTHREADS, 1) linear_tc_kernel(const __grid_constant__ CUtensorMap map_x,
                                                                 const __grid_constant__ CUtensorMap map_w,
                                                                 const float* __restrict__ bias, const float* __restrict__ row_scale,
                                                                 float* __restrict__ Y, int ldy, int M, int N, int K, int BN, int relu,
                                                                 GnFuse gn, float* __restrict__ splitk_out, int chunks_per_split,
-                                                                int col_tiles, int row_tiles, int num_tiles) {
+                                                                int col_tiles, int row_tiles, int num_tiles, float* __restrict__ acc_out,
+                                                                const float* __restrict__ acc_in, const long long* __restrict__ up,
+                                                                int up_stride, int n_support) {
     constexpr int R = BNI / 2;
     extern __shared__ unsigned char smem_raw[];
     unsigned char* smem = (unsigned char*)(((uintptr_t)smem_raw + 1023) & ~(uintptr_t)1023);
@@ -50,12 +53,14 @@
     uint64_t* empty = bars + NSTAGE;
     float2* gn_sm = (float2*)(smem + NSTAGE * STAGE + 256);
     float* bias_s = (float*)(gn_sm + 8 * 128);
+    volatile int* cur_tile = (volatile int*)(smem + NSTAGE * STAGE + 128);
     const int warp = threadIdx.x >> 5, lane = threadIdx.x & 31;
     const int nk = (K + KC - 1) / KC;
     const int tiles_per_split = col_tiles * row_tiles;
 
     if (threadIdx.x == 0) {
         for (int s = 0; s < NSTAGE; ++s) { mbar_init(&full[s], 1); mbar_init(&empty[s], 8); }
+        *cur_tile = -1;
         asm volatile("fence.mbarrier_init.release.cluster;" ::: "memory");
         asm volatile("prefetch.tensormap [%0];" ::"l"(&map_x) : "memory");
         asm volatile("prefetch.tensormap [%0];" ::"l"(&map_w) : "memory");
@@ -82,6 +87,29 @@
                 }
             }
         }
+        if constexpr (MODE == PARTIAL_IN) {
+            if (warp == PRODUCER_WARP + 1) {
+                const int bytes = BN * 4;
+                auto prefetch = [&](int t) {
+                    const int rem = t % tiles_per_split;
+                    const int m0 = (rem / col_tiles) * BM, n0 = (rem % col_tiles) * BN;
+                    for (int r = lane; r < BM; r += 32) {
+                        if (m0 + r >= M) break;
+                        const unsigned long long src = (unsigned long long)up[(long long)(m0 + r) * up_stride];
+                        if (src < (unsigned long long)n_support) {
+                            const float* p = acc_in + (long long)src * 2 * N + n0;
+                            asm volatile("cp.async.bulk.prefetch.L2.global [%0], %1;" ::"l"(p), "r"(bytes) : "memory");
+                            asm volatile("cp.async.bulk.prefetch.L2.global [%0], %1;" ::"l"(p + N), "r"(bytes) : "memory");
+                        }
+                    }
+                };
+                if (blockIdx.x < num_tiles) prefetch(blockIdx.x);
+                for (int t = blockIdx.x; t + (int)gridDim.x < num_tiles; t += gridDim.x) {
+                    while (*cur_tile < t) __nanosleep(256);
+                    prefetch(t + gridDim.x);
+                }
+            }
+        }
         return;
     }
 
@@ -96,11 +124,47 @@
         const int kc0 = z * chunks_per_split, kc1 = min(nk, kc0 + chunks_per_split);
         asm volatile("bar.sync 1, 256;" ::: "memory");
         if (threadIdx.x < 128) bias_s[threadIdx.x] = (bias != nullptr && (int)threadIdx.x < BN) ? __ldg(bias + n0 + threadIdx.x) : 0.f;
+        if constexpr (MODE == PARTIAL_IN) if (threadIdx.x == 0) *cur_tile = t;
         asm volatile("bar.sync 1, 256;" ::: "memory");
 
         float acc[R], cor[R];
-#pragma unroll
-        for (int i = 0; i < R; ++i) { acc[i] = 0.f; cor[i] = 0.f; }
+        if constexpr (MODE == PARTIAL_IN) {
+            const int r0 = m0 + wg * 64 + wq * 16 + (lane >> 2), c0 = 2 * (lane & 3);
+            bool ok[2];
+            const float* row[2];
+#pragma unroll
+            for (int h = 0; h < 2; ++h) {
+                const unsigned long long src = r0 + 8 * h < M ? (unsigned long long)up[(long long)(r0 + 8 * h) * up_stride]
+                                                              : (unsigned long long)n_support;
+                ok[h] = src < (unsigned long long)n_support;
+                row[h] = acc_in + (long long)(ok[h] ? src : 0) * 2 * N + n0;
+            }
+#pragma unroll
+            for (int j = 0; j < BNI / 8; ++j) {
+                const int col = min(8 * j + c0, BN - 2);
+#pragma unroll
+                for (int h = 0; h < 2; ++h) {
+                    const float2 a = __ldg(reinterpret_cast<const float2*>(row[h] + col));
+                    const float2 c = __ldg(reinterpret_cast<const float2*>(row[h] + N + col));
+                    acc[4 * j + 2 * h] = a.x; acc[4 * j + 2 * h + 1] = a.y;
+                    cor[4 * j + 2 * h] = c.x; cor[4 * j + 2 * h + 1] = c.y;
+                }
+            }
+#pragma unroll
+            for (int j = 0; j < BNI / 8; ++j)
+#pragma unroll
+                for (int h = 0; h < 2; ++h) {
+                    const bool keep = ok[h] && 8 * j + c0 < BN;
+#pragma unroll
+                    for (int i = 0; i < 2; ++i) {
+                        acc[4 * j + 2 * h + i] = keep ? acc[4 * j + 2 * h + i] : 0.f;
+                        cor[4 * j + 2 * h + i] = keep ? cor[4 * j + 2 * h + i] : 0.f;
+                    }
+                }
+        } else {
+#pragma unroll
+            for (int i = 0; i < R; ++i) { acc[i] = 0.f; cor[i] = 0.f; }
+        }
         const int g = lane >> 2, tq = lane & 3;
         const int a_off = (wg * 64 + wq * 16 + g) * 128 + tq * 4;
         for (int kc = kc0; kc < kc1; ++kc) {
@@ -123,7 +187,7 @@
 #pragma unroll
             for (int kk = 0; kk < KC / 8; ++kk) {
                 const uint64_t adv = (uint64_t)(kk * 2);
-                const uint32_t accum = (kc == kc0 && kk == 0) ? 0u : 1u;
+                const uint32_t accum = (MODE != PARTIAL_IN && kc == kc0 && kk == 0) ? 0u : 1u;
                 wgmma_tf32_rs<BNI>(acc, f[0][kk], b_hi + adv, accum);
                 wgmma_tf32_rs<BNI>(cor, f[0][kk], b_lo + adv, accum);
                 wgmma_tf32_rs<BNI>(cor, f[1][kk], b_hi + adv, 1u);
@@ -142,6 +206,20 @@
         float rs[2];
 #pragma unroll
         for (int h = 0; h < 2; ++h) rs[h] = (row_scale != nullptr && r0 + 8 * h < M) ? row_scale[r0 + 8 * h] : 1.0f;
+        if constexpr (MODE == PARTIAL_OUT) {
+#pragma unroll
+            for (int j = 0; j < BNI / 8; ++j)
+#pragma unroll
+                for (int h = 0; h < 2; ++h) {
+                    const int m = r0 + 8 * h, col = 8 * j + c0;
+                    if (m < M && col < BN) {
+                        float* dst = acc_out + (long long)m * 2 * N + n0 + col;
+                        *reinterpret_cast<float2*>(dst) = make_float2(acc[4 * j + 2 * h], acc[4 * j + 2 * h + 1]);
+                        *reinterpret_cast<float2*>(dst + N) = make_float2(cor[4 * j + 2 * h], cor[4 * j + 2 * h + 1]);
+                    }
+                }
+            continue;
+        }
         if (splitk_out != nullptr) {
 #pragma unroll
             for (int j = 0; j < BNI / 8; ++j)
@@ -275,6 +353,18 @@
 static bool g_prof_on = false;
 static bool g_splitk_on = true;
 static bool g_persistent_on = true;
+static bool g_decoder_split_on = true;
+
+static int splitk_splits(int tiles, int nk) {
+    int splits = 1;
+    if (g_splitk_on && tiles * 2 <= num_sms() && nk >= 16) {
+        splits = nk / 8;
+        if (splits > num_sms() / tiles) splits = num_sms() / tiles;
+        if (splits > 16) splits = 16;
+        if (splits < 2) splits = 1;
+    }
+    return splits;
+}
 
 struct StreamWs { void* ptr; size_t bytes; };
 static std::vector<std::pair<cudaStream_t, StreamWs>> g_split_ws, g_wimg_ws;
@@ -323,13 +413,7 @@
     }
     const int nk = (int)((k + ltc::KC - 1) / ltc::KC);
     const int tiles = col_tiles * row_tiles;
-    int splits = 1;
-    if (g_splitk_on && tiles * 2 <= num_sms() && nk >= 16) {
-        splits = nk / 8;
-        if (splits > num_sms() / tiles) splits = num_sms() / tiles;
-        if (splits > 16) splits = 16;
-        if (splits < 2) splits = 1;
-    }
+    int splits = splitk_splits(tiles, nk);
     if (gn != nullptr && splits > 1) return 1;
     int cps = nk;
     float* part = nullptr;
@@ -360,12 +444,14 @@
     const int num_tiles = tiles * splits;
     const bool persistent = g_persistent_on && splits == 1 && tiles > num_sms();
     const unsigned grid = (unsigned)(persistent ? num_sms() : num_tiles);
-    const void* kern = BN <= 32 ? (const void*)ltc::linear_tc_kernel<32> : BN <= 64 ? (const void*)ltc::linear_tc_kernel<64>
-                                                                                      : (const void*)ltc::linear_tc_kernel<128>;
+    const void* kern = BN <= 32 ? (const void*)ltc::linear_tc_kernel<32, ltc::PLAIN>
+                       : BN <= 64 ? (const void*)ltc::linear_tc_kernel<64, ltc::PLAIN>
+                                  : (const void*)ltc::linear_tc_kernel<128, ltc::PLAIN>;
     if (ensure_max_smem(kern)) return -1;
 #define GEOB_LTC_LAUNCH(BNI)                                                                                                  \
-    ltc::linear_tc_kernel<BNI><<<grid, ltc::NTHREADS, ltc::SMEM, st>>>(mx, mw, bias, row_scale, y, (int)ldy, (int)m, (int)n, (int)k, \
-                                                                       BN, relu, g, part, cps, col_tiles, row_tiles, num_tiles)
+    ltc::linear_tc_kernel<BNI, ltc::PLAIN><<<grid, ltc::NTHREADS, ltc::SMEM, st>>>(                                           \
+        mx, mw, bias, row_scale, y, (int)ldy, (int)m, (int)n, (int)k, BN, relu, g, part, cps, col_tiles, row_tiles, num_tiles,   \
+        nullptr, nullptr, nullptr, 0, 0)
     if (BN <= 32) GEOB_LTC_LAUNCH(32);
     else if (BN <= 64) GEOB_LTC_LAUNCH(64);
     else GEOB_LTC_LAUNCH(128);
@@ -385,9 +471,85 @@
     return 0;
 }
 
+bool linear_tc_sequential(int64_t m, int64_t n, int64_t k) {
+    if (m < 64 || n < 32 || (n % 16) != 0 || (k % 4) != 0) return false;
+    if (n > 128 && (n % 128) != 0) return false;
+    const int BN = (int)(n >= 128 ? 128 : n);
+    const int tiles = (int)(n / BN) * (int)((m + ltc::BM - 1) / ltc::BM);
+    return splitk_splits(tiles, (int)((k + ltc::KC - 1) / ltc::KC)) == 1;
+}
+
+bool decoder_split_enabled() { return g_decoder_split_on; }
+
+int linear_tc_partial(const float* x, int64_t ldx, const float* w_img, int64_t k, int64_t k1, const float* bias, float* y, int64_t ldy,
+                      int64_t m, int64_t n, int relu, float* acc_out, const float* acc_in, const int64_t* up, int64_t up_stride,
+                      int64_t n_support, cudaStream_t st, const GnFuse* gn) {
+    const bool out_mode = acc_out != nullptr;
+    const int64_t kp = out_mode ? k1 : k - k1;
+    if (m < 1 || n < 32 || (n % 16) != 0 || (k % 4) != 0 || (k1 % ltc::KC) != 0 || k1 <= 0 || k1 >= k || (ldx % 4) != 0) return 1;
+    if (w_img == nullptr || (reinterpret_cast<uintptr_t>(x) & 15) || (reinterpret_cast<uintptr_t>(w_img) & 15)) return 1;
+    if (reinterpret_cast<uintptr_t>(out_mode ? (const float*)acc_out : acc_in) & 15) return 1;
+    if (n > 128 && (n % 128) != 0) return 1;
+    const int BN = (int)(n >= 128 ? 128 : n);
+    const int col_tiles = (int)(n / BN), row_tiles = (int)((m + ltc::BM - 1) / ltc::BM);
+    GnFuse g{};
+    if (gn != nullptr) {
+        if (out_mode) return 1;
+        g = *gn;
+        const int64_t cpg = n / g.groups;
+        if (g.groups <= 0 || n % g.groups != 0 || (cpg < 32 ? (32 % cpg) != 0 : (cpg % 32) != 0 || (BN % cpg) != 0) || relu) return 1;
+        g.slot_width = (int)(cpg < 32 ? cpg : 32);
+    }
+    CUtensorMap mx, mw;
+    if (ltc::encode_map(&mx, x, m, kp, ldx, ltc::BM)) return -1;
+    if (ltc::encode_map(&mw, out_mode ? w_img : w_img + k1, 2 * n, kp, k, BN)) return -1;
+    ProfRec rec{};
+    const bool prof = g_prof_on;
+    if (prof) {
+        cudaEventCreate(&rec.a);
+        cudaEventCreate(&rec.b);
+        rec.m = m; rec.n = n; rec.k = kp;
+        cudaEventRecord(rec.a, st);
+    }
+    const int tiles = col_tiles * row_tiles;
+    const bool persistent = g_persistent_on && tiles > num_sms();
+    const unsigned grid = (unsigned)(persistent ? num_sms() : tiles);
+    const long long* upl = (const long long*)up;
+#define GEOB_LTC_PARTIAL(BNI, MODE)                                                                                           \
+    do {                                                                                                                      \
+        if (ensure_max_smem((const void*)ltc::linear_tc_kernel<BNI, MODE>)) return -1;                                         \
+        ltc::linear_tc_kernel<BNI, MODE><<<grid, ltc::NTHREADS, ltc::SMEM, st>>>(                                             \
+            mx, mw, bias, nullptr, y, (int)ldy, (int)m, (int)n, (int)kp, BN, relu, g, nullptr, (int)((kp + ltc::KC - 1) / ltc::KC), \
+            col_tiles, row_tiles, tiles, acc_out, acc_in, upl, (int)up_stride, (int)n_support);                               \
+    } while (0)
+    if (out_mode) {
+        if (BN <= 32) GEOB_LTC_PARTIAL(32, ltc::PARTIAL_OUT);
+        else if (BN <= 64) GEOB_LTC_PARTIAL(64, ltc::PARTIAL_OUT);
+        else GEOB_LTC_PARTIAL(128, ltc::PARTIAL_OUT);
+    } else {
+        if (BN <= 32) GEOB_LTC_PARTIAL(32, ltc::PARTIAL_IN);
+        else if (BN <= 64) GEOB_LTC_PARTIAL(64, ltc::PARTIAL_IN);
+        else GEOB_LTC_PARTIAL(128, ltc::PARTIAL_IN);
+    }
+#undef GEOB_LTC_PARTIAL
+    if (prof) {
+        cudaEventRecord(rec.b, st);
+        std::lock_guard<std::mutex> lk(g_prof_mu);
+        g_prof.push_back(rec);
+    }
+    GEOB_CHECK_LAUNCH();
+    count_launches(1);
+    return 0;
+}
+
 }
 
 extern "C" {
+
+int geob200_set_decoder_split(int on) {
+    geob200::g_decoder_split_on = on != 0;
+    return 0;
+}
 
 int geob200_set_linear_persistent(int on) {
     geob200::g_persistent_on = on != 0;
diff --git a/geotransformer_b200/csrc/native.cu b/geotransformer_b200/csrc/native.cu
--- a/geotransformer_b200/csrc/native.cu
+++ b/geotransformer_b200/csrc/native.cu
@@ -179,11 +179,29 @@
     for (int lvl = S - 1; lvl >= net->finest_decoder; --lvl) {
         const int64_t m = level_rows[lvl - 1], ns = level_rows[lvl];
         const int64_t c2 = enc_ch[lvl - 1];
+        const geob200_linear_t& l = net->decoders[S - 1 - lvl];
+        float* o = out_feats[oi++];
+        if (decoder_split_applies(m, l.c_out, l.c_in, latent_ch, l.weight_img)) {
+            float* acc = c.fl(ns, 2 * l.c_out);
+            GEOB_REQUIRE(c.ar.ok(), "native: arena too small (decoder)");
+            TRY(linear_partial_out_impl(latent, latent_ch, l.weight_img, ns, l.c_out, l.c_in, latent_ch, acc, stream));
+            if (lvl == net->finest_decoder) {
+                TRY(linear_partial_in_impl(enc[lvl - 1], c2, l.weight_img, l.bias, acc, upsampling[lvl - 1], upsampling_width[lvl - 1], ns,
+                                           o, l.c_out, m, l.c_out, l.c_in, latent_ch, 0, stream));
+            } else {
+                float* t = c.fl(m, l.c_out);
+                GEOB_REQUIRE(c.ar.ok(), "native: arena too small (decoder)");
+                const geob200_norm_t& nm = net->decoder_norms[S - 1 - lvl];
+                TRY(linear_group_norm_partial_in_impl(enc[lvl - 1], c2, l.weight_img, l.bias, acc, upsampling[lvl - 1],
+                                                      upsampling_width[lvl - 1], ns, m, l.c_out, l.c_in, latent_ch, c.groups, nm.gamma,
+                                                      nm.beta, 1e-5f, nullptr, 1, 0.1f, t, o, c.gn_ws, c.gn_ws_bytes, stream, sg[lvl - 1]));
+            }
+            latent = o; latent_ch = l.c_out;
+            continue;
+        }
         float* cat = c.fl(m, latent_ch + c2);
         GEOB_REQUIRE(c.ar.ok(), "native: arena too small (decoder)");
         TRY(geob200_upsample_concat(latent, upsampling[lvl - 1], upsampling_width[lvl - 1], ns, enc[lvl - 1], m, latent_ch, c2, cat, stream));
-        const geob200_linear_t& l = net->decoders[S - 1 - lvl];
-        float* o = out_feats[oi++];
         if (lvl == net->finest_decoder) {
             TRY(linear_img(cat, l.c_in, l.weight, l.weight_img, l.bias, o, l.c_out, m, l.c_out, l.c_in, 0, stream));
         } else {
diff --git a/geotransformer_b200/functional.py b/geotransformer_b200/functional.py
--- a/geotransformer_b200/functional.py
+++ b/geotransformer_b200/functional.py
@@ -201,6 +201,51 @@
     out = torch.empty((2 * n, k), dtype=_f32, device=weight.device)
     L.check(L.lib().geob200_split_tf32(weight.data_ptr(), weight.stride(0), n, k, out.data_ptr(), L.stream_ptr()), 'split_tf32')
     return out
+
+
+def linear_partial_out(x, w_img):
+    _f(x, 'x'); _f(w_img, 'w_img')
+    m, k1 = x.shape
+    n, k = w_img.shape[0] // 2, w_img.shape[1]
+    acc = torch.empty((m, 2 * n), dtype=_f32, device=x.device)
+    L.check(L.lib().geob200_linear_partial_out(x.data_ptr(), x.stride(0), w_img.data_ptr(), m, n, k, k1, acc.data_ptr(), L.stream_ptr()),
+            'linear_partial_out')
+    return acc
+
+
+def linear_partial_in(skip, w_img, acc, upsample_indices, n_support, bias=None, relu=False):
+    _f(skip, 'skip'); _f(w_img, 'w_img'); _f(acc, 'acc')
+    m, k2 = skip.shape
+    n, k = w_img.shape[0] // 2, w_img.shape[1]
+    y = torch.empty((m, n), dtype=_f32, device=skip.device)
+    L.check(L.lib().geob200_linear_partial_in(skip.data_ptr(), skip.stride(0), w_img.data_ptr(), L.ptr(_detach(bias)), acc.data_ptr(),
+                                              upsample_indices.data_ptr(), upsample_indices.stride(0), n_support, y.data_ptr(), n, m, n, k,
+                                              k - k2, int(relu), L.stream_ptr()), 'linear_partial_in')
+    return y
+
+
+def linear_group_norm_partial_in(skip, w_img, acc, upsample_indices, n_support, bias, gn_weight, gn_bias, groups, eps=1e-5,
+                                 negative_slope=None, residual=None, cloud_rows=None, pre=None, workspace=None):
+    _f(skip, 'skip'); _f(w_img, 'w_img'); _f(acc, 'acc')
+    m, k2 = skip.shape
+    n, k = w_img.shape[0] // 2, w_img.shape[1]
+    np_ = 1 if cloud_rows is None else len(cloud_rows) // 2
+    if pre is None:
+        pre = torch.empty((m, n), dtype=_f32, device=skip.device)
+    y = torch.empty((m, n), dtype=_f32, device=skip.device)
+    if workspace is None:
+        workspace = _gn_workspace(skip.device, groups, m, n, n_pairs=np_)
+    L.check(L.lib().geob200_linear_group_norm_partial_in_batched(
+        skip.data_ptr(), skip.stride(0), w_img.data_ptr(), L.ptr(_detach(bias)), acc.data_ptr(), upsample_indices.data_ptr(),
+        upsample_indices.stride(0), n_support, m, n, k, k - k2, groups, _detach(gn_weight).data_ptr(), _detach(gn_bias).data_ptr(),
+        float(eps), L.ptr(_detach(residual)), int(negative_slope is not None), float(negative_slope or 0.0), pre.data_ptr(), y.data_ptr(),
+        workspace.data_ptr(), workspace.numel(), L.stream_ptr(), np_, None if cloud_rows is None else _host_i64(cloud_rows)),
+        'linear_group_norm_partial_in')
+    return y
+
+
+def set_decoder_split(on):
+    L.lib().geob200_set_decoder_split(int(bool(on)))
 
 
 def group_norm(x, weight, bias, groups, eps=1e-5, negative_slope=None, residual=None, cloud_rows=None):
diff --git a/include/geob200.h b/include/geob200.h
--- a/include/geob200.h
+++ b/include/geob200.h
@@ -87,6 +87,17 @@
 
 int geob200_upsample_concat(const float* x, const int64_t* up_indices, int64_t up_stride, int64_t n_support,
                             const float* skip, int64_t n_query, int64_t c1, int64_t c2, float* y, void* stream);
+
+int geob200_linear_partial_out(const float* x, int64_t ldx, const float* w_img, int64_t m, int64_t n, int64_t k, int64_t k1, float* acc,
+                               void* stream);
+int geob200_linear_partial_in(const float* skip, int64_t ldx, const float* w_img, const float* bias, const float* acc,
+                              const int64_t* up_indices, int64_t up_stride, int64_t n_support, float* y, int64_t ldy, int64_t m, int64_t n,
+                              int64_t k, int64_t k1, int relu, void* stream);
+int geob200_linear_group_norm_partial_in_batched(const float* skip, int64_t ldx, const float* w_img, const float* bias, const float* acc,
+                                                 const int64_t* up_indices, int64_t up_stride, int64_t n_support, int64_t m, int64_t n,
+                                                 int64_t k, int64_t k1, int64_t groups, const float* gamma, const float* beta, float eps,
+                                                 const float* residual, int leaky, float slope, float* pre_norm, float* y, void* workspace,
+                                                 size_t workspace_bytes, void* stream, int64_t n_pairs, const int64_t* cloud_rows_h);
 
 
 size_t geob200_kpconv_backward_workspace_bytes(int64_t n_query, int64_t n_support, int64_t n_neighbors, int64_t c_in, int64_t c_out);
@@ -333,6 +344,7 @@
 int geob200_linear_profile_enable(int on);
 int geob200_set_split_k(int on);
 int geob200_set_linear_persistent(int on);
+int geob200_set_decoder_split(int on);
 int64_t geob200_linear_profile_read(int64_t capacity, int64_t* shapes, float* ms);
 
 #define GEOB200_MAX_STAGES 6
```

Measured after the change: 443.0 (median of 6 runs). 1.8% higher.
